# sergiud/SuiteSparse

Hardware: AMD Instinct MI355X
Metric: GFLOP/s supernodal Cholesky factor (Common->fl / t_factorize) (higher is better)
Workload: dtype f64; 1 GPU; poisson3d_200^3_geometricND_leaf4; n=8000000, nsuper=428821, parallelism=1 GPU

## Files before the change

### include/cholmod.h

```cpp
#ifndef CHOLMOD_AMD_H
#define CHOLMOD_AMD_H

#include <stddef.h>
#include <stdint.h>
#include <stdio.h>

#ifdef __cplusplus
extern "C" {
#endif

typedef int64_t SuiteSparse_long ;

#define CHOLMOD_MAIN_VERSION 3
#define CHOLMOD_SUB_VERSION 0
#define CHOLMOD_SUBSUB_VERSION 14

#ifndef TRUE
#define TRUE 1
#define FALSE 0
#endif

#define CHOLMOD_INT 0
#define CHOLMOD_INTLONG 1
#define CHOLMOD_LONG 2
// ... 206 lines not shown
double cholmod_l_norm_dense (cholmod_dense *X, int norm, cholmod_common *Common) ;
double cholmod_l_norm_sparse (cholmod_sparse *A, int norm, cholmod_common *Common) ;

cholmod_factor *cholmod_l_analyze (cholmod_sparse *A, cholmod_common *Common) ;
cholmod_factor *cholmod_l_analyze_p (cholmod_sparse *A, SuiteSparse_long *UserPerm,
    SuiteSparse_long *fset, size_t fsize, cholmod_common *Common) ;
cholmod_factor *cholmod_l_analyze_p2 (int for_whom, cholmod_sparse *A,
    SuiteSparse_long *UserPerm, SuiteSparse_long *fset, size_t fsize,
    cholmod_common *Common) ;
int cholmod_l_factorize (cholmod_sparse *A, cholmod_factor *L, cholmod_common *Common) ;
int cholmod_l_factorize_p (cholmod_sparse *A, double beta [2], SuiteSparse_long *fset,
    size_t fsize, cholmod_factor *L, cholmod_common *Common) ;
cholmod_dense *cholmod_l_solve (int sys, cholmod_factor *L, cholmod_dense *B,
    cholmod_common *Common) ;
int cholmod_l_solve2 (int sys, cholmod_factor *L, cholmod_dense *B, cholmod_sparse *Bset,
    cholmod_dense **X_Handle, cholmod_sparse **Xset_Handle, cholmod_dense **Y_Handle,
    cholmod_dense **E_Handle, cholmod_common *Common) ;
double cholmod_l_rcond (cholmod_factor *L, cholmod_common *Common) ;
int cholmod_l_change_factor (int to_xtype, int to_ll, int to_super, int to_packed, int to_monotonic,
    cholmod_factor *L, cholmod_common *Common) ;
int cholmod_l_etree (cholmod_sparse *A, SuiteSparse_long *Parent, cholmod_common *Common) ;
SuiteSparse_long cholmod_l_postorder (SuiteSparse_long *Parent, size_t n,
    SuiteSparse_long *Weight, SuiteSparse_long *Post, cholmod_common *Common) ;
int cholmod_l_rowcolcounts (cholmod_sparse *A, SuiteSparse_long *fset, size_t fsize,
    SuiteSparse_long *Parent, SuiteSparse_long *Post, SuiteSparse_long *RowCount,
    SuiteSparse_long *ColCount, SuiteSparse_long *First, SuiteSparse_long *Level,
    cholmod_common *Common) ;

int cholmod_l_super_symbolic (cholmod_sparse *A, cholmod_sparse *F,
    SuiteSparse_long *Parent, cholmod_factor *L, cholmod_common *Common) ;
int cholmod_l_super_symbolic2 (int for_whom, cholmod_sparse *A, cholmod_sparse *F,
    SuiteSparse_long *Parent, cholmod_factor *L, cholmod_common *Common) ;
int cholmod_l_super_numeric (cholmod_sparse *A, cholmod_sparse *F, double beta [2],
    cholmod_factor *L, cholmod_common *Common) ;
int cholmod_l_super_lsolve (cholmod_factor *L, cholmod_dense *X, cholmod_dense *E,
    cholmod_common *Common) ;
int cholmod_l_super_ltsolve (cholmod_factor *L, cholmod_dense *X, cholmod_dense *E,
    cholmod_common *Common) ;

int cholmod_l_gpu_memorysize (size_t *total_mem, size_t *available_mem,
    cholmod_common *Common) ;
int cholmod_l_gpu_probe (cholmod_common *Common) ;
int cholmod_l_gpu_deallocate (cholmod_common *Common) ;
void cholmod_l_gpu_end (cholmod_common *Common) ;
int cholmod_l_gpu_allocate (cholmod_common *Common) ;
int cholmod_gpu_memorysize (size_t *total_mem, size_t *available_mem, cholmod_common *Common) ;
int cholmod_gpu_probe (cholmod_common *Common) ;
int cholmod_gpu_deallocate (cholmod_common *Common) ;
void cholmod_gpu_end (cholmod_common *Common) ;
int cholmod_gpu_allocate (cholmod_common *Common) ;

int cholmod_l_factor_to_host (cholmod_factor *L, cholmod_common *Common) ;
int cholmod_l_hip_stats (cholmod_factor *L, double *stats, cholmod_common *Common) ;
int cholmod_l_hip_prepare (cholmod_factor *L, cholmod_common *Common) ;
int cholmod_l_gather_factor (cholmod_factor *L, cholmod_common *Common) ;
int cholmod_l_refactorize_resident (double beta [2], cholmod_factor *L,
    cholmod_common *Common) ;

#ifdef __cplusplus
}
#endif
#endif
```

### include/cholmod_hip.h

```cpp
#ifndef CHOLMOD_HIP_H
#define CHOLMOD_HIP_H

#include <stddef.h>
#include <stdint.h>

#ifdef __cplusplus
extern "C" {
#endif

#define CHOLMOD_HIP_OK            0
#define CHOLMOD_HIP_NOT_POSDEF    1
#define CHOLMOD_HIP_NO_DEVICE   (-1)
#define CHOLMOD_HIP_OUT_OF_MEMORY (-2)
#define CHOLMOD_HIP_TOO_LARGE   (-3)
#define CHOLMOD_HIP_INVALID     (-4)
#define CHOLMOD_HIP_GPU_PROBLEM (-5)

#define CHOLMOD_HIP_PLAN_DEFAULT   0
#define CHOLMOD_HIP_TILE128         4
#define CHOLMOD_HIP_NO_SMALL_FRONTS 16
#define CHOLMOD_HIP_NO_XCD_SWIZZLE 32
#define CHOLMOD_HIP_FIXED_OB       64
#define CHOLMOD_HIP_WIDE_OB       128
#define CHOLMOD_HIP_NO_CB_ASSIGN   2048
#define CHOLMOD_HIP_NO_FUSED_POTRF 512
#define CHOLMOD_HIP_NO_FUSED_TRSM 1024
#define CHOLMOD_HIP_NO_LEAF_PAIRS 4096
#define CHOLMOD_HIP_NO_EXCHANGE_LOOKAHEAD 256
#define CHOLMOD_HIP_CHAIN256     8192
#define CHOLMOD_HIP_PHI_TWIN    16384
#define CHOLMOD_HIP_CX_STORAGE   32768
#define CHOLMOD_HIP_PLAN_HOST_ONLY 2

typedef struct cholmod_hip_plan cholmod_hip_plan ;

int cholmod_hip_probe (void) ;

int cholmod_hip_memorysize (size_t *total_mem, size_t *available_mem) ;

int cholmod_hip_set_device (int device) ;
int cholmod_hip_device_count (int *count) ;

cholmod_hip_plan *cholmod_hip_plan_create (int64_t n, int64_t nsuper,
    const int64_t *super, const int64_t *pi, const int64_t *px,
    const int64_t *s, int flags, int *status) ;

void cholmod_hip_plan_destroy (cholmod_hip_plan *plan) ;

typedef int (*cholmod_hip_allreduce_fn) (void *dev_ptr, int64_t count_doubles,
    int group_first, int group_size, void *user) ;
cholmod_hip_plan *cholmod_hip_plan_create_dist (int64_t n, int64_t nsuper,
    const int64_t *super, const int64_t *pi, const int64_t *px,
    const int64_t *s, int flags, int rank, int world, int *status) ;
int cholmod_hip_set_allreduce (cholmod_hip_plan *plan,
    cholmod_hip_allreduce_fn fn, void *user) ;
int cholmod_hip_rccl_unique_id (void *id128) ;
int cholmod_hip_rccl_attach (cholmod_hip_plan *plan, const void *id128) ;
int cholmod_hip_rccl_detach (cholmod_hip_plan *plan) ;
int64_t cholmod_hip_debug_routing (cholmod_hip_plan *plan, int64_t cap, int64_t *pair_d, int64_t *pair_a,
    int64_t *cb_lo, int64_t *cb_hi) ;
int cholmod_hip_debug_schedule_hash (cholmod_hip_plan *plan, uint64_t *out16) ;
int cholmod_hip_progress_enable (cholmod_hip_plan *plan, int enable) ;
int cholmod_hip_progress (cholmod_hip_plan *plan, int64_t *out12) ;
int64_t cholmod_hip_get_batches (cholmod_hip_plan *plan, int64_t *batch_of, int64_t *global_arena) ;
int cholmod_hip_get_partition (cholmod_hip_plan *plan, int64_t *owner) ;
int cholmod_hip_get_groups (cholmod_hip_plan *plan, int64_t *first, int64_t *size) ;
int cholmod_hip_gather_factor (cholmod_hip_plan *plan) ;

int cholmod_hip_factorize (cholmod_hip_plan *plan, const int64_t *Sp,
    const int64_t *Si, const int64_t *Snz, const double *Sx, double beta,
    int quick_return_if_not_posdef, double *Lx_host, int64_t *minor) ;

int cholmod_hip_upload_matrix (cholmod_hip_plan *plan, const int64_t *Sp,
    const int64_t *Si, const int64_t *Snz, const double *Sx) ;
int cholmod_hip_factorize_resident (cholmod_hip_plan *plan, double beta,
    int quick_return_if_not_posdef, int64_t *minor) ;

int cholmod_hip_set_value_map (cholmod_hip_plan *plan, const int64_t *src, int64_t snz,
    int64_t nvalues) ;
int cholmod_hip_refresh_values (cholmod_hip_plan *plan, const double *values, int64_t nvalues) ;
int cholmod_hip_values_staging (cholmod_hip_plan *plan, double **host_buffer, int64_t *nvalues) ;
int cholmod_hip_values_push (cholmod_hip_plan *plan, int64_t offset, int64_t count) ;
int cholmod_hip_values_commit (cholmod_hip_plan *plan, int commit) ;
int cholmod_hip_values_gather_index (cholmod_hip_plan *plan, const int64_t **index, int64_t *chunk_len, int64_t *count) ;
int cholmod_hip_values_begin (cholmod_hip_plan *plan) ;
int cholmod_hip_values_push_chunk (cholmod_hip_plan *plan, int64_t chunk) ;

int cholmod_hip_download_factor (cholmod_hip_plan *plan, double *Lx_host) ;
int cholmod_hip_download_even_columns (cholmod_hip_plan *plan, double *out_host) ;
int cholmod_hip_upload_factor (cholmod_hip_plan *plan, const double *Lx_host) ;

int cholmod_hip_solve (cholmod_hip_plan *plan, int which, double *X,
    int64_t nrhs, int64_t ldx) ;

int cholmod_hip_get_maps (cholmod_hip_plan *plan, int64_t *sparent,
    int64_t *level, int64_t *relmap) ;

int cholmod_hip_diag_minmax (cholmod_hip_plan *plan, double *out3) ;
int cholmod_hip_factor_checks (cholmod_hip_plan *plan, double *out5) ;
int cholmod_hip_factor_checks_local (cholmod_hip_plan *plan, double *out5) ;

#define CHOLMOD_HIP_NSTATS 40
int cholmod_hip_get_stats (cholmod_hip_plan *plan, double *stats) ;
int cholmod_hip_set_profiling (cholmod_hip_plan *plan, int on) ;
int64_t cholmod_hip_get_launch_profile (cholmod_hip_plan *plan, int64_t cap, int32_t *kind,
    int32_t *grid, int32_t *aux, double *ms, double *flops, double *bytes) ;

int cholmod_hip_debug_thin_cycles (cholmod_hip_plan *plan, int64_t launch, long long *out10) ;
int64_t cholmod_hip_debug_launch_regions (cholmod_hip_plan *plan, int64_t launch, int64_t cap, int64_t *out) ;

int cholmod_hip_dense_partial_factor (double *F, int64_t nsrow, int64_t nscol,
    int flags, int64_t *info) ;

const char *cholmod_hip_version (void) ;

#ifdef __cplusplus
}
#endif
#endif
```

### suitesparse_amd/cholmod.py

```python
from __future__ import annotations

import ctypes as C
import os
import subprocess

import numpy as np

_HERE = os.path.dirname(os.path.abspath(__file__))
LIB_PATH = os.environ.get("CHOLMOD_AMD_LIB") or os.path.join(_HERE, "lib", "libcholmod_amd.so")
HOOKS_LIB_PATH = os.path.join(_HERE, "lib", "libcholmod_amd_testhooks.so")
CSRC = os.path.join(_HERE, "csrc")

CHOLMOD_MAXMETHODS = 9
CHOLMOD_HIP_NSTATS = 40

PATTERN, REAL, COMPLEX, ZOMPLEX = 0, 1, 2, 3
OK, NOT_INSTALLED, OUT_OF_MEMORY, TOO_LARGE, INVALID, GPU_PROBLEM = 0, -1, -2, -3, -4, -5
NOT_POSDEF = 1
NATURAL, GIVEN, POSTORDERED = 0, 1, 6
SIMPLICIAL, AUTO, SUPERNODAL = 0, 1, 2
SYS_A, SYS_LDLt, SYS_LD, SYS_DLt, SYS_L, SYS_Lt, SYS_D, SYS_P, SYS_Pt = range(9)
HIP_PLAN_HOST_ONLY = 2
HIP_WIDE_OB, HIP_NO_FUSED_POTRF, HIP_NO_FUSED_TRSM, HIP_PHI_TWIN = 128, 512, 1024, 16384
HIP_INVALID = -4


class Method(C.Structure):
    _fields_ = [("lnz", C.c_double), ("fl", C.c_double), ("ordering", C.c_int)]


ERRFUNC = C.CFUNCTYPE(None, C.c_int, C.c_char_p, C.c_int, C.c_char_p)
ALLREDUCE_FN = C.CFUNCTYPE(C.c_int, C.c_void_p, C.c_int64, C.c_int, C.c_int, C.c_void_p)


class Common(C.Structure):
    _fields_ = [
        ("supernodal", C.c_int), ("supernodal_switch", C.c_double),
        ("final_asis", C.c_int), ("final_super", C.c_int), ("final_ll", C.c_int),
        ("final_pack", C.c_int), ("final_monotonic", C.c_int), ("final_resymbol", C.c_int),
        ("zrelax", C.c_double * 3), ("nrelax", C.c_size_t * 3),
        ("prefer_upper", C.c_int), ("quick_return_if_not_posdef", C.c_int),
        ("print", C.c_int), ("nmethods", C.c_int), ("current", C.c_int), ("selected", C.c_int),
        ("method", Method * (CHOLMOD_MAXMETHODS + 1)),
        ("postorder", C.c_int), ("try_catch", C.c_int),
        ("error_handler", ERRFUNC),
        ("itype", C.c_int), ("dtype", C.c_int), ("status", C.c_int),
        ("fl", C.c_double), ("lnz", C.c_double), ("anz", C.c_double), ("modfl", C.c_double),
        ("malloc_count", C.c_size_t), ("memory_usage", C.c_size_t), ("memory_inuse", C.c_size_t),
        ("nrealloc_col", C.c_double), ("nrealloc_factor", C.c_double), ("ndbounds_hit", C.c_double),
        ("rowfacfl", C.c_double), ("aatfl", C.c_double),
        ("called_nd", C.c_int), ("blas_ok", C.c_int),
        ("useGPU", C.c_int), ("maxGpuMemBytes", C.c_size_t), ("maxGpuMemFraction", C.c_double),
        ("gpuMemorySize", C.c_size_t), ("gpuKernelTime", C.c_double), ("gpuFlops", C.c_int64),
        ("gpuNumKernelLaunches", C.c_int), ("devBuffSize", C.c_size_t), ("ibuffer", C.c_int),
        ("syrkStart", C.c_double),
        ("cholmod_cpu_gemm_time", C.c_double), ("cholmod_cpu_syrk_time", C.c_double),
        ("cholmod_cpu_trsm_time", C.c_double), ("cholmod_cpu_potrf_time", C.c_double),
        ("cholmod_gpu_gemm_time", C.c_double), ("cholmod_gpu_syrk_time", C.c_double),
        ("cholmod_gpu_trsm_time", C.c_double), ("cholmod_gpu_potrf_time", C.c_double),
        ("cholmod_assemble_time", C.c_double), ("cholmod_assemble_time2", C.c_double),
        ("cholmod_cpu_gemm_calls", C.c_size_t), ("cholmod_cpu_syrk_calls", C.c_size_t),
        ("cholmod_cpu_trsm_calls", C.c_size_t), ("cholmod_cpu_potrf_calls", C.c_size_t),
        ("cholmod_gpu_gemm_calls", C.c_size_t), ("cholmod_gpu_syrk_calls", C.c_size_t),
        ("cholmod_gpu_trsm_calls", C.c_size_t), ("cholmod_gpu_potrf_calls", C.c_size_t),
        ("hip_factor_on_device", C.c_int), ("hip_flags", C.c_int), ("hip_profile", C.c_int),
        ("hip_rank", C.c_int), ("hip_world", C.c_int),
        ("hip_allreduce", C.c_void_p), ("hip_allreduce_user", C.c_void_p),
# ... 10 lines not shown


class Triplet(C.Structure):
    _fields_ = [("nrow", C.c_size_t), ("ncol", C.c_size_t), ("nzmax", C.c_size_t), ("nnz", C.c_size_t),
                ("i", C.c_void_p), ("j", C.c_void_p), ("x", C.c_void_p), ("z", C.c_void_p),
                ("stype", C.c_int), ("itype", C.c_int), ("xtype", C.c_int), ("dtype", C.c_int)]


class Dense(C.Structure):
    _fields_ = [("nrow", C.c_size_t), ("ncol", C.c_size_t), ("nzmax", C.c_size_t),
                ("d", C.c_size_t), ("x", C.c_void_p), ("z", C.c_void_p),
                ("xtype", C.c_int), ("dtype", C.c_int)]


class Factor(C.Structure):
    _fields_ = [("n", C.c_size_t), ("minor", C.c_size_t),
                ("Perm", C.c_void_p), ("ColCount", C.c_void_p), ("IPerm", C.c_void_p),
                ("nzmax", C.c_size_t),
                ("p", C.c_void_p), ("i", C.c_void_p), ("x", C.c_void_p), ("z", C.c_void_p),
                ("nz", C.c_void_p), ("next", C.c_void_p), ("prev", C.c_void_p),
                ("nsuper", C.c_size_t), ("ssize", C.c_size_t), ("xsize", C.c_size_t),
                ("maxcsize", C.c_size_t), ("maxesize", C.c_size_t),
                ("super", C.c_void_p), ("pi", C.c_void_p), ("px", C.c_void_p), ("s", C.c_void_p),
                ("ordering", C.c_int), ("is_ll", C.c_int), ("is_super", C.c_int),
                ("is_monotonic", C.c_int), ("itype", C.c_int), ("xtype", C.c_int),
                ("dtype", C.c_int), ("useGPU", C.c_int),
                ("hip_plan", C.c_void_p), ("hip_on_device", C.c_int), ("hip_host_valid", C.c_int),
                ("cx_twin", C.c_void_p), ("hip_apat_hash", C.c_uint64), ("hip_apat_nnz", C.c_size_t),
                ("hip_apat_valid", C.c_int), ("hip_apat_hash2", C.c_uint64), ("hip_is_twin", C.c_int),
                ("bset_work", C.c_void_p), ("hip_plan_ahead", C.c_int)]


API_SYMBOLS = [
    "cholmod_l_start", "cholmod_l_finish", "cholmod_l_defaults", "cholmod_l_error",
    "cholmod_l_malloc", "cholmod_l_calloc", "cholmod_l_free",
    "cholmod_l_allocate_sparse", "cholmod_l_free_sparse", "cholmod_l_copy_sparse",
    "cholmod_l_nnz", "cholmod_l_ptranspose", "cholmod_l_transpose",
    "cholmod_l_allocate_triplet", "cholmod_l_free_triplet", "cholmod_l_triplet_to_sparse",
    "cholmod_l_allocate_dense", "cholmod_l_zeros", "cholmod_l_ones", "cholmod_l_copy_dense",
    "cholmod_l_free_dense", "cholmod_l_free_factor",
    "cholmod_l_read_sparse", "cholmod_l_read_triplet", "cholmod_l_read_dense", "cholmod_l_read_matrix", "cholmod_l_check_factor", "cholmod_l_check_sparse",
    "cholmod_gpu_memorysize", "cholmod_gpu_probe", "cholmod_gpu_deallocate", "cholmod_gpu_end", "cholmod_gpu_allocate",
    "cholmod_l_gpu_stats", "cholmod_l_sdmult", "cholmod_l_norm_dense", "cholmod_l_norm_sparse",
    "cholmod_l_analyze", "cholmod_l_analyze_p", "cholmod_l_analyze_p2",
    "cholmod_l_factorize", "cholmod_l_factorize_p", "cholmod_l_solve", "cholmod_l_solve2",
    "cholmod_l_rcond", "cholmod_l_change_factor", "cholmod_l_realloc",
    "SuiteSparse_start", "SuiteSparse_finish", "SuiteSparse_malloc", "SuiteSparse_calloc", "SuiteSparse_realloc", "SuiteSparse_free",
    "cholmod_l_etree", "cholmod_l_postorder", "cholmod_l_rowcolcounts",
    "cholmod_l_super_symbolic", "cholmod_l_super_symbolic2", "cholmod_l_super_numeric",
    "cholmod_l_super_lsolve", "cholmod_l_super_ltsolve",
    "cholmod_l_gpu_memorysize", "cholmod_l_gpu_probe", "cholmod_l_gpu_deallocate",
    "cholmod_l_gpu_end", "cholmod_l_gpu_allocate",
    "cholmod_l_factor_to_host", "cholmod_l_hip_stats", "cholmod_l_refactorize_resident",
    "cholmod_l_gather_factor", "cholmod_l_hip_prepare",
]
HIP_SYMBOLS = [
    "cholmod_hip_probe", "cholmod_hip_memorysize", "cholmod_hip_set_device", "cholmod_hip_device_count",
    "cholmod_hip_plan_create", "cholmod_hip_plan_destroy", "cholmod_hip_factorize",
    "cholmod_hip_plan_create_dist", "cholmod_hip_set_allreduce", "cholmod_hip_get_partition",
    "cholmod_hip_get_groups", "cholmod_hip_get_batches", "cholmod_hip_progress_enable", "cholmod_hip_progress", "cholmod_hip_debug_schedule_hash", "cholmod_hip_diag_minmax", "cholmod_hip_values_staging", "cholmod_hip_values_push", "cholmod_hip_values_commit", "cholmod_hip_values_gather_index", "cholmod_hip_values_begin", "cholmod_hip_values_push_chunk", "cholmod_hip_debug_routing",
    "cholmod_hip_gather_factor",
    "cholmod_hip_upload_matrix", "cholmod_hip_factorize_resident",
    "cholmod_hip_set_value_map", "cholmod_hip_refresh_values",
    "cholmod_hip_download_factor", "cholmod_hip_download_even_columns", "cholmod_hip_upload_factor", "cholmod_hip_solve",
    "cholmod_hip_get_maps", "cholmod_hip_get_stats", "cholmod_hip_set_profiling",
    
    
    "cholmod_hip_dense_partial_factor", "cholmod_hip_factor_checks", "cholmod_hip_factor_checks_local", "cholmod_hip_get_launch_profile", "cholmod_hip_debug_thin_cycles", "cholmod_hip_debug_launch_regions",
    "cholmod_hip_rccl_unique_id", "cholmod_hip_rccl_attach", "cholmod_hip_rccl_detach",
    "cholmod_hip_version",
]

PROBES_PATH = os.path.join(_HERE, "lib", "libcholmod_amd_probes.so")
PROBE_SYMBOLS = [
    "cholmod_hip_bench_update_kernel", "cholmod_hip_bench_update_pair", "cholmod_hip_bench_mfma_peak", "cholmod_hip_bench_mfma_peak2",
    "cholmod_hip_bench_mixed", "cholmod_hip_debug_potrf_cycles", "cholmod_hip_debug_panel_cycles",
    "cholmod_hip_debug_latency", "cholmod_hip_bench_mfma_ceiling", "cholmod_hip_probe_cu_mask", "cholmod_hip_probe_overlap", "cholmod_hip_debug_update_diff", "cholmod_hip_debug_diag_cycles", "cholmod_hip_bench_handoff",
]

_probes = None


def build(force: bool = False) -> str:
    if force:
        subprocess.check_call(["make", "-C", CSRC, "-s", "clean"])
    subprocess.check_call(["make", "-C", CSRC, "-s", "-j3"])
    return LIB_PATH


_libs = {}


def lib(hooks=None):
    if hooks is None:
        hooks = os.environ.get("SSAMD_TEST_HOOKS_LIB") == "1"
    path = HOOKS_LIB_PATH if hooks else LIB_PATH
    if path in _libs:
        return _libs[path]
    if not os.path.exists(path):
        raise RuntimeError(
            f"{path} is missing: build it with `python -c 'import __graft_entry__ as g; "
            "g.build()'` (hipcc --offload-arch=gfx950).  There is no fallback path.")
    L = C.CDLL(path)
    vp, i64, dbl, sz = C.c_void_p, C.c_int64, C.c_double, C.c_size_t
    cm = C.POINTER(Common)
    sp, dn, fc = C.POINTER(Sparse), C.POINTER(Dense), C.POINTER(Factor)

    def sig(name, res, args):
        f = getattr(L, name)
        f.restype = res
        f.argtypes = args

# ... 3 lines not shown
    sig("cholmod_l_allocate_sparse", sp, [sz, sz, sz, C.c_int, C.c_int, C.c_int, C.c_int, cm])
    sig("cholmod_l_free_sparse", C.c_int, [C.POINTER(sp), cm])
    sig("cholmod_l_copy_sparse", sp, [sp, cm])
    sig("cholmod_l_nnz", i64, [sp, cm])
    sig("cholmod_l_ptranspose", sp, [sp, C.c_int, vp, vp, sz, cm])
    sig("cholmod_l_transpose", sp, [sp, C.c_int, cm])
    sig("cholmod_l_allocate_dense", dn, [sz, sz, sz, C.c_int, cm])
    sig("cholmod_l_zeros", dn, [sz, sz, C.c_int, cm])
    sig("cholmod_l_ones", dn, [sz, sz, C.c_int, cm])
    sig("cholmod_l_copy_dense", dn, [dn, cm])
    sig("cholmod_l_free_dense", C.c_int, [C.POINTER(dn), cm])
    sig("cholmod_l_free_factor", C.c_int, [C.POINTER(fc), cm])
    sig("cholmod_l_check_factor", C.c_int, [fc, cm])
    sig("cholmod_l_check_sparse", C.c_int, [sp, cm])
    sig("cholmod_l_gpu_stats", C.c_int, [cm])
    sig("cholmod_l_sdmult", C.c_int, [sp, C.c_int, C.POINTER(dbl * 2), C.POINTER(dbl * 2), dn, dn, cm])
    sig("cholmod_l_norm_dense", dbl, [dn, C.c_int, cm])
    sig("cholmod_l_norm_sparse", dbl, [sp, C.c_int, cm])
    sig("cholmod_l_analyze", fc, [sp, cm])
    sig("cholmod_l_analyze_p", fc, [sp, vp, vp, sz, cm])
    sig("cholmod_l_analyze_p2", fc, [C.c_int, sp, vp, vp, sz, cm])
    sig("cholmod_l_factorize", C.c_int, [sp, fc, cm])
    sig("cholmod_l_factorize_p", C.c_int, [sp, C.POINTER(dbl * 2), vp, sz, fc, cm])
    sig("cholmod_l_solve", dn, [C.c_int, fc, dn, cm])
    sig("cholmod_l_solve2", C.c_int, [C.c_int, fc, dn, sp, C.POINTER(dn), C.POINTER(sp), C.POINTER(dn), C.POINTER(dn), cm])
    sig("cholmod_l_rcond", dbl, [fc, cm])
    sig("cholmod_l_change_factor", C.c_int, [C.c_int, C.c_int, C.c_int, C.c_int, C.c_int, fc, cm])
    sig("cholmod_l_etree", C.c_int, [sp, vp, cm])
    sig("cholmod_l_postorder", i64, [vp, sz, vp, vp, cm])
    sig("cholmod_l_rowcolcounts", C.c_int, [sp, vp, sz, vp, vp, vp, vp, vp, vp, cm])
    sig("cholmod_l_super_symbolic", C.c_int, [sp, sp, vp, fc, cm])
    sig("cholmod_l_super_numeric", C.c_int, [sp, sp, C.POINTER(dbl * 2), fc, cm])
    sig("cholmod_l_super_lsolve", C.c_int, [fc, dn, dn, cm])
    sig("cholmod_l_super_ltsolve", C.c_int, [fc, dn, dn, cm])
    sig("cholmod_l_gpu_memorysize", C.c_int, [C.POINTER(sz), C.POINTER(sz), cm])
    sig("cholmod_l_gpu_probe", C.c_int, [cm])
    sig("cholmod_l_gpu_allocate", C.c_int, [cm])
    sig("cholmod_l_gpu_deallocate", C.c_int, [cm])
    sig("cholmod_l_factor_to_host", C.c_int, [fc, cm])
    sig("cholmod_l_hip_stats", C.c_int, [fc, C.POINTER(dbl * CHOLMOD_HIP_NSTATS), cm])
    sig("cholmod_l_refactorize_resident", C.c_int, [C.POINTER(dbl * 2), fc, cm])
    sig("cholmod_l_read_sparse", sp, [vp, cm])
    sig("cholmod_l_read_dense", dn, [vp, cm])
    sig("cholmod_l_read_triplet", vp, [vp, cm])
    sig("cholmod_l_free_triplet", C.c_int, [C.POINTER(vp), cm])
    sig("cholmod_l_read_matrix", vp, [vp, C.c_int, C.POINTER(C.c_int), cm])
    sig("cholmod_hip_probe", C.c_int, [])
    sig("cholmod_hip_set_device", C.c_int, [C.c_int])
    sig("cholmod_hip_memorysize", C.c_int, [C.POINTER(sz), C.POINTER(sz)])
    sig("cholmod_hip_plan_create", vp, [i64, i64, vp, vp, vp, vp, C.c_int, C.POINTER(C.c_int)])
    sig("cholmod_hip_plan_destroy", None, [vp])
    sig("cholmod_hip_plan_create_dist", vp, [i64, i64, vp, vp, vp, vp, C.c_int, C.c_int, C.c_int,
                                             C.POINTER(C.c_int)])
    sig("cholmod_hip_set_allreduce", C.c_int, [vp, ALLREDUCE_FN, vp])
    sig("cholmod_hip_get_partition", C.c_int, [vp, vp])
    sig("cholmod_hip_get_groups", C.c_int, [vp, vp, vp])
    sig("cholmod_hip_get_batches", i64, [vp, vp, vp])
    sig("cholmod_hip_progress_enable", C.c_int, [vp, C.c_int])
    sig("cholmod_hip_progress", C.c_int, [vp, vp])
    sig("cholmod_hip_debug_schedule_hash", C.c_int, [vp, vp])
    sig("cholmod_hip_debug_routing", C.c_int64, [vp, C.c_int64, vp, vp, vp, vp])
    sig("cholmod_hip_gather_factor", C.c_int, [vp])
    sig("cholmod_l_gather_factor", C.c_int, [fc, cm])
    sig("cholmod_l_hip_prepare", C.c_int, [fc, cm])
    sig("cholmod_hip_factorize", C.c_int, [vp, vp, vp, vp, vp, dbl, C.c_int, vp, C.POINTER(i64)])
    sig("cholmod_hip_upload_matrix", C.c_int, [vp, vp, vp, vp, vp])
    sig("cholmod_hip_factorize_resident", C.c_int, [vp, dbl, C.c_int, C.POINTER(i64)])
    sig("cholmod_hip_download_factor", C.c_int, [vp, vp])
    sig("cholmod_hip_upload_factor", C.c_int, [vp, vp])
    sig("cholmod_hip_solve", C.c_int, [vp, C.c_int, vp, i64, i64])
    sig("cholmod_hip_get_maps", C.c_int, [vp, vp, vp, vp])
    sig("cholmod_hip_get_stats", C.c_int, [vp, vp])
    sig("cholmod_hip_set_profiling", C.c_int, [vp, C.c_int])
    sig("cholmod_hip_dense_partial_factor", C.c_int, [vp, i64, i64, C.c_int, C.POINTER(i64)])
    sig("cholmod_hip_factor_checks", C.c_int, [vp, vp])
    sig("cholmod_hip_factor_checks_local", C.c_int, [vp, vp])
    sig("cholmod_hip_get_launch_profile", i64, [vp, i64, vp, vp, vp, vp, vp, vp])
    sig("cholmod_hip_debug_thin_cycles", C.c_int, [vp, i64, vp])
    sig("cholmod_hip_debug_launch_regions", i64, [vp, i64, i64, vp])
    sig("cholmod_hip_rccl_unique_id", C.c_int, [vp])
    sig("cholmod_hip_rccl_attach", C.c_int, [vp, vp])
    sig("cholmod_hip_rccl_detach", C.c_int, [vp])
    sig("cholmod_hip_version", C.c_char_p, [])
    _libs[path] = L
    return L


def probes():
    global _probes
    if _probes is not None:
        return _probes
    if not os.path.exists(PROBES_PATH):
        raise RuntimeError(f"{PROBES_PATH} is missing: build it with __graft_entry__.build()")
    L = C.CDLL(PROBES_PATH)
    vp, i64, dbl = C.c_void_p, C.c_int64, C.c_double
    for name, res, args in (
            ("cholmod_hip_bench_update_kernel", dbl, [i64, i64, i64, C.c_int, C.c_int]),
            ("cholmod_hip_bench_update_pair", dbl, [i64, i64, i64, i64, i64, C.c_int, C.c_int]),
            ("cholmod_hip_bench_mfma_peak", dbl, [C.c_int, C.c_int]),
            ("cholmod_hip_bench_mfma_peak2", dbl, [C.c_int, C.c_int, C.c_int, C.c_int]),
            ("cholmod_hip_bench_mixed", dbl, [C.c_int, C.c_int, C.c_int]),
            ("cholmod_hip_bench_mfma_ceiling", dbl, [C.c_int, C.c_int, C.c_int, C.c_int, vp]),
            ("cholmod_hip_probe_cu_mask", dbl, [vp, C.c_int, C.c_int, C.c_int, vp]),
            ("cholmod_hip_probe_overlap", C.c_int, [vp, vp, C.c_int, i64, i64, C.c_int, C.c_int, C.c_int, vp]),
            ("cholmod_hip_debug_update_diff", dbl, [i64, i64, i64, C.c_int, C.c_int, C.c_int]),
            ("cholmod_hip_debug_diag_cycles", C.c_int, [vp, C.c_int, C.c_int]),
# ... 230 lines not shown
```

### suitesparse_amd/csrc/hip/descriptors.hip.h

```cpp
#pragma once
#include <hip/hip_runtime.h>
#include <stdint.h>

typedef long long i64;
typedef int i32;

namespace sship {


struct FrontD {
    i64 psx;
    i64 psi;
    i64 cb;
    i64 rel;
    i32 k1;
    i32 nscol, nsrow, ncb;
    i32 parent;
    i32 child_begin, child_end;
    i32 assemble;
    i32 cbp;
    i32 own_w, own_g, own_r;
    i32 cbd;
    i32 cb_lo, cb_hi;
};
__host__ __device__ __forceinline__ bool col_owned (const FrontD &f, int c) { return f.own_w == 0 || ((c / f.own_w) % f.own_g) == f.own_r ; }
__host__ __device__ __forceinline__ int col_local (const FrontD &f, int c) { return f.own_w == 0 ? c : ((c / f.own_w) / f.own_g) * f.own_w + c % f.own_w ; }
__host__ __device__ __forceinline__ int owned_before (const FrontD &f, int c)
{
    if (f.own_w == 0) return c ;
    const int t = c / f.own_w ;
    const int full = t > f.own_r ? (t - f.own_r + f.own_g - 1) / f.own_g : 0 ;
    return full * f.own_w + ((t % f.own_g) == f.own_r ? c % f.own_w : 0) ;
}

struct ChildD { i64 cb; i64 rel; i32 ncb; i32 cbp; };
struct EaGroup { i32 front; i32 blk_start; i32 c_lo; i32 c_hi;
                 i64 pbase; };
#define EA_NO_PBASE INT64_MIN
struct ZeroGroup { i64 off; i64 len; i32 blk_start; i32 pad; };
struct PfGroup { i64 off; i32 lda; i32 nb; i32 front; i32 col0; };
struct TrGroup { i64 l_off; i64 b_off; i32 lda; i32 m; i32 nb; i32 front;
                 i32 col0; i32 blk_start; };
struct DgGroup { i64 off; i32 lda; i32 w; i32 front; i32 col0; i32 slot; i32 pad; };
struct RsGroup { i64 l_off; i64 b_off; i32 lda; i32 m; i32 w; i32 front; i32 col0; i32 blk_start; i32 slot; i32 pad; };
struct GemmGroup {
    i64 a_off, b_off, c_off;
    i32 lda, ldc;
    i32 m, n, k;
    i32 tri;
    i32 c_in_cb;
    i32 tile_start;
    i32 mt, nt;
    i32 front;
    i32 tile_mul, tile_add;
    i32 ntiles;
    i32 nblk;
    i32 swz;
    i32 assign;
    i32 pf_next, pf_col0;
    i32 tile_cnt;
};

__host__ __device__ __forceinline__ int tri_col (int j, int m) { return j * m - ((j * (j + 1)) >> 1) ; }

struct RelPair { i32 d ; i32 a ; i64 off ; } ;
#define ZERO_CHUNK 8192
#define ZERO_COLS 8
#ifndef EA_TW
#define EA_TW 8
#endif
#define UPD3_LX_PAD 64
#define PF_NB 64
#define PF2_LD 64
#define TRM_ROWS 64
#define SM_MAX 136
#define TF_PW 16
struct XchgD {
    i64 slab ;
    i32 lda ;
    i32 w ;
    i32 mb ;
    i32 R ;
    i32 g, r ;
    i32 fo ;
    i32 mf ;
    i32 Rf ;
} ;
#define WIN_ROWS 8192
struct WinD { i64 store ; i64 win ; i32 ld ; i32 c0, c1 ; i32 r0 ; i32 nrows ; i32 own_w, own_g, own_r ; i32 mode ; i32 blk_start ; } ;
#define DG_W 256
#define RS_ROWS 64
struct CfGroup { i64 l_off ; i32 lda ; i32 w ; i32 front ; i32 col0 ; i32 m1 ; i32 slot ; i32 fslot ; i32 dstart ; i32 bstart ; i32 off2 ; i32 m2 ; i32 off3 ; i32 m3 ; i32 pad ; } ;
struct SolveTask { i32 front ; i32 c0, c1 ; i32 below ; } ;
#define SOLVE_IB 64
#define SOLVE_SB 256
#define SOLVE_BIG_COLS 256
struct InvTask { i32 front ; i32 jb ; i64 w_off ; } ;
struct SolveBlk { i32 front, jb, w, wg_start, inv, slot ; } ;
#define CHK_COLS 64
struct CheckTask { i32 front ; i32 c0 ; } ;

}
```

### suitesparse_amd/csrc/hip/engine.hip

```cpp
#include "kernels.hip.h"
#include "plan.hip.h"
#include <thread>

#include <dlfcn.h>
#include <unistd.h>

namespace sship {
RcclApi *rccl_api ()
{
    static RcclApi api ;
    static bool tried = false ;
    if (tried) return api.h ? &api : nullptr ;
    tried = true ;
    const char *over = getenv ("CHOLMOD_HIP_RCCL_LIBRARY") ;
    const char *names [] = {"librccl.so.1", "librccl.so", "/opt/rocm/lib/librccl.so.1", nullptr} ;
    void *h = nullptr ;
    if (over && *over)
    {
        h = dlopen (over, RTLD_NOW | RTLD_LOCAL) ;
        if (!h) fprintf (stderr, "cholmod_hip: CHOLMOD_HIP_RCCL_LIBRARY=%s: %s\n", over, dlerror ()) ;
    }
    else for (int q = 0 ; names [q] && !h ; q++) h = dlopen (names [q], RTLD_NOW | RTLD_LOCAL) ;
    if (!h) return nullptr ;
    api.GetUniqueId = (decltype (api.GetUniqueId)) dlsym (h, "ncclGetUniqueId") ;
    api.CommInitRank = (decltype (api.CommInitRank)) dlsym (h, "ncclCommInitRank") ;
    api.CommSplit = (decltype (api.CommSplit)) dlsym (h, "ncclCommSplit") ;
    api.AllReduce = (decltype (api.AllReduce)) dlsym (h, "ncclAllReduce") ;
    api.ReduceScatter = (decltype (api.ReduceScatter)) dlsym (h, "ncclReduceScatter") ;
    api.AllGather = (decltype (api.AllGather)) dlsym (h, "ncclAllGather") ;
    api.Broadcast = (decltype (api.Broadcast)) dlsym (h, "ncclBroadcast") ;
    api.CommDestroy = (decltype (api.CommDestroy)) dlsym (h, "ncclCommDestroy") ;
    api.GetErrorString = (decltype (api.GetErrorString)) dlsym (h, "ncclGetErrorString") ;
    if (!api.GetUniqueId || !api.CommInitRank || !api.CommSplit || !api.AllReduce || !api.ReduceScatter || !api.AllGather || !api.Broadcast || !api.CommDestroy) return nullptr ;
    api.h = h ;
    return &api ;
}
}
#define COMMA ,
#define CXS_LAUNCH(K, ...) do { if (cxs) hipLaunchKernelGGL (K<true>, __VA_ARGS__) ; else hipLaunchKernelGGL (K<false>, __VA_ARGS__) ; } while (0)
#define RCCLCHK(call) do { ncclResult_t r_ = (call) ; if (r_ != ncclSuccess) { \
    fprintf (stderr, "cholmod_hip: %s failed: %s (%s:%d)\n", #call, \
        (rccl_api () && rccl_api ()->GetErrorString) ? rccl_api ()->GetErrorString (r_) : "?", __FILE__, __LINE__) ; \
    return CHOLMOD_HIP_GPU_PROBLEM ; } } while (0)


namespace {

static void free_device (cholmod_hip_plan *P)
{
    if (P->prog_dev) { (void) hipHostFree (P->prog_dev) ; P->prog_dev = nullptr ; }
    if (P->h_vals) { (void) hipHostFree (P->h_vals) ; P->h_vals = nullptr ; }
    if (P->values_ev) { (void) hipEventDestroy (P->values_ev) ; P->values_ev = nullptr ; }
    for (auto e : P->chunk_ev) (void) hipEventDestroy (e) ;
    P->chunk_ev.clear () ;
    if (P->d_vorder) { (void) hipFree (P->d_vorder) ; P->d_vorder = nullptr ; }
    if (RcclApi *R = (P->nccl_world ? rccl_api () : nullptr))
    {
        for (auto &g : P->nccl_group) (void) R->CommDestroy (g.second) ;
        (void) R->CommDestroy (P->nccl_world) ;
        P->nccl_group.clear () ; P->nccl_world = nullptr ;
    }
    if (P->ar_done) (void) hipEventDestroy (P->ar_done) ;
    void *ptrs [] = {P->d_Ls, P->d_fr, P->d_supermap, P->d_child, P->d_relmap, P->d_info,
        P->d_lvl_list, P->d_Lx, P->d_cb, P->d_zg, P->d_eg, P->d_pg, P->d_tg, P->d_tu_cnt, P->d_cdesc, P->d_smd, P->d_sp01, P->d_gg, P->d_sm,
        P->d_Sp, P->d_Si, P->d_Snz, P->d_Sx, P->d_amap, P->d_X, P->d_Y, P->d_perm, P->d_xchg, P->d_stage, P->d_ag, P->d_agf, P->d_Lx_full, P->d_fr_full, P->d_dg, P->d_rg, P->d_wg, P->d_cg, P->d_cflags, P->d_crel, P->d_relpairs, P->d_dinv, P->d_sv,
        P->d_inv_tasks, P->d_winv, P->d_solved, P->d_sv_acc, P->d_ticket, P->d_chk, P->d_chk_out, P->d_thin_tim, P->d_sb_tasks, P->d_sb_commit, P->d_first_fail, P->d_vsrc, P->d_vals} ;
    for (void *p : ptrs) if (p) (void) hipFree (p) ;
    for (auto e : P->evpool) (void) hipEventDestroy (e) ;
    for (auto e : P->sync_ev) (void) hipEventDestroy (e) ;
    if (P->stream2) (void) hipStreamDestroy (P->stream2) ;
    if (P->ev0) (void) hipEventDestroy (P->ev0) ;
    if (P->ev1) (void) hipEventDestroy (P->ev1) ;
    if (P->stream) (void) hipStreamDestroy (P->stream) ;
}

static int upload_plan (cholmod_hip_plan *P)
{
    hipError_t e ;
    const bool ptiming = getenv ("CHOLMOD_HIP_PLAN_TIMING") != nullptr ;
    auto pnow = [] () { return std::chrono::duration<double> (std::chrono::steady_clock::now ().time_since_epoch ()).count () ; } ;
    double tu0 = pnow () ;
    HIPCHK (hipStreamCreate (&P->stream)) ;
    if (const char *e = TEST_ENV ("CHOLMOD_HIP_TEST_JITTER"))
    {
        unsigned long long seed = 0 ; int mx = 2000 ;
        if (sscanf (e, "%llu:%d", &seed, &mx) >= 1 && mx > 0)
        {
            P->jitter_us = mx ;
            P->jitter_state = seed * 0x9E3779B97F4A7C15ull + (unsigned long long) (P->rank + 1) * 0xD1B54A32D192ED03ull ;
        }
    }
    { const char *e = TEST_ENV ("CHOLMOD_HIP_TEST_DROP_WAITS") ; P->test_drop_waits = e ? std::max (atoi (e), 1) : 0 ; }
    if (const char *e = TEST_ENV ("CHOLMOD_HIP_TEST_HANG_EXCHANGE")) (void) sscanf (e, "%d:%ld:%ld", &P->test_hang_rank, &P->test_hang_xchg, &P->test_hang_fact) ;
    P->upd3_wg4 = P->world > 1 || P->force_shared ;
    {
        int least = 0, greatest = 0 ;
        if (hipDeviceGetStreamPriorityRange (&least, &greatest) == hipSuccess && greatest != least)
            HIPCHK (hipStreamCreateWithPriority (&P->stream2, hipStreamDefault, greatest)) ;
        else HIPCHK (hipStreamCreate (&P->stream2)) ;
    }
    for (int q = 0 ; q < P->sch.nevents ; q++)
    {
        hipEvent_t e ;
        HIPCHK (hipEventCreateWithFlags (&e, hipEventDisableTiming)) ;
        P->sync_ev.push_back (e) ;
    }
    HIPCHK (hipEventCreate (&P->ev0)) ;
    HIPCHK (hipEventCreate (&P->ev1)) ;
    size_t freeb = 0, totalb = 0 ;
    HIPCHK (hipMemGetInfo (&freeb, &totalb)) ;
    double need = 8.0 * P->lx_local + 8.0 * P->arena + 8.0 * P->ssize + 4.0 * P->relsize
        + sizeof (GemmGroup) * (double) P->sch.gg.size () + 64.0 * P->nsuper + (double) (64 << 20) ;
    if (need > (double) freeb)
    {
        fprintf (stderr, "cholmod_hip: factor needs %.2f GB of HBM, %.2f GB free\n",
            need / 1e9, freeb / 1e9) ;
        return CHOLMOD_HIP_OUT_OF_MEMORY ;
    }
    double tu1 = pnow () ;
    P->d_Ls = dupload (P->Ls, e) ; HIPCHK (e) ;
    P->d_fr = dupload (P->fr, e) ; HIPCHK (e) ;
    P->d_supermap = dupload (P->supermap, e) ; HIPCHK (e) ;
    P->d_child = dupload (P->child, e) ; HIPCHK (e) ;
    P->d_crel = dupload (P->crel, e) ; HIPCHK (e) ;
    P->d_relpairs = dupload (P->relpairs, e) ; HIPCHK (e) ;
    {
        std::vector<ChildD> cdv (P->child.size ()) ;
        for (size_t q = 0 ; q < P->child.size () ; q++)
        {
            if (P->child [q] < 0 || (size_t) P->child [q] >= P->fr.size ()) { cdv [q] = ChildD {0, 0, 0, 1} ; continue ; }
            const FrontD &cf = P->fr [P->child [q]] ;
            cdv [q] = ChildD {cf.cb, cf.rel, cf.ncb, cf.cbp} ;
        }
        P->d_cdesc = dupload (cdv, e) ; HIPCHK (e) ;
    }
    P->d_lvl_list = dupload (P->lvl_list, e) ; HIPCHK (e) ;
    P->d_zg = dupload (P->sch.zg, e) ; HIPCHK (e) ;
    P->d_eg = dupload (P->sch.eg, e) ; HIPCHK (e) ;
    P->d_pg = dupload (P->sch.pg, e) ; HIPCHK (e) ;
    P->d_tg = dupload (P->sch.tg, e) ; HIPCHK (e) ;
    HIPCHK (hipMalloc ((void **) &P->d_tu_cnt, std::max<size_t> (P->sch.tg.size (), 1) * sizeof (i32))) ;
    P->d_gg = dupload (P->sch.gg, e) ; HIPCHK (e) ;
    P->d_dg = dupload (P->sch.dg, e) ; HIPCHK (e) ;
    P->d_rg = dupload (P->sch.rg, e) ; HIPCHK (e) ;
    P->d_wg = dupload (P->sch.wg, e) ; HIPCHK (e) ;
    P->d_cg = dupload (P->sch.cg, e) ; HIPCHK (e) ;
    HIPCHK (hipMalloc ((void **) &P->d_cflags, (4 * (size_t) P->sch.ncflags + 4) * sizeof (int))) ;
    HIPCHK (hipMalloc ((void **) &P->d_dinv, (size_t) std::max (P->sch.max_dinv_slots, 1) * 4096 * sizeof (double))) ;
    P->d_sm = dupload (P->sch.sm, e) ; HIPCHK (e) ;
    {
        std::vector<FrontD> smd (P->sch.sm.size ()) ;
        for (size_t q = 0 ; q < smd.size () ; q++) smd [q] = P->fr [P->sch.sm [q]] ;
        P->d_smd = dupload (smd, e) ; HIPCHK (e) ;
        HIPCHK (hipMalloc ((void **) &P->d_sp01, std::max<size_t> (2 * smd.size (), 1) * sizeof (i64))) ;
    }
    P->d_sv = dupload (P->sv_tasks, e) ; HIPCHK (e) ;
    double tu2 = pnow () ;
    HIPCHK (hipMalloc ((void **) &P->d_relmap, std::max<i64> (std::max (P->relsize, P->relsize_all), 1) * sizeof (i32))) ;
    HIPCHK (hipMalloc ((void **) &P->d_info, std::max<i64> (P->nsuper, 1) * sizeof (i32))) ;
    HIPCHK (hipMalloc ((void **) &P->d_first_fail, sizeof (int))) ;
    if (TEST_ENV ("CHOLMOD_HIP_TEST_FAIL_ALLOC")) return CHOLMOD_HIP_OUT_OF_MEMORY ;
    HIPCHK (hipMalloc ((void **) &P->d_Lx, (std::max<i64> (P->lx_local, 1) + UPD3_LX_PAD) * sizeof (double))) ;
    HIPCHK (hipMalloc ((void **) &P->d_cb, std::max<i64> (P->arena, 1) * sizeof (double))) ;
    HIPCHK (hipMalloc ((void **) &P->d_xchg, 3 * (size_t) P->world * sizeof (double))) ;
    {
        i64 mx = 1, mxg = 1, mxf = 1 ;
        for (const Launch &L : P->sch.launches)
            if (L.kind == K_XCHG_RS || L.kind == K_XCHG_AG)
            {
                mx = std::max (mx, ((i64) L.xd.w * L.xd.w + ((i64) L.xd.R + L.xd.Rf) * L.xd.w) * L.xd.g) ;
                mxg = std::max (mxg, (i64) L.xd.R * L.xd.w * L.xd.g) ;
                mxf = std::max (mxf, (i64) L.xd.Rf * L.xd.w * L.xd.g) ;
            }
        HIPCHK (hipMalloc ((void **) &P->d_stage, (size_t) mx * sizeof (double))) ;
        HIPCHK (hipMalloc ((void **) &P->d_ag, (size_t) mxg * sizeof (double))) ;
        HIPCHK (hipMalloc ((void **) &P->d_agf, (size_t) mxf * sizeof (double))) ;
        P->agf_len = mxf ;
        P->stage_len = mx ; P->ag_len = mxg ;
    }
    double tu3 = pnow () ;
    if (getenv ("CHOLMOD_HIP_THIN_TIMING"))
    {
        HIPCHK (hipMalloc ((void **) &P->d_thin_tim, (P->sch.launches.size () + 1) * 10 * sizeof (long long))) ;
        HIPCHK (hipMemset (P->d_thin_tim, 0, (P->sch.launches.size () + 1) * 10 * sizeof (long long))) ;
    }
    if (P->nsuper > 0)
    {
        int grid = (int) ((P->nsuper * 64 + 255) / 256) ;
        hipLaunchKernelGGL (k_relmap, dim3 (grid), dim3 (256), 0, P->stream,
            (int) P->nsuper, P->d_fr, P->d_Ls, P->d_relmap) ;
        if (!P->relpairs.empty ())
            hipLaunchKernelGGL (k_relmap_pairs, dim3 ((unsigned) ((P->relpairs.size () * 64 + 255) / 256)), dim3 (256), 0, P->stream,
                (int) P->relpairs.size (), P->d_relpairs, P->d_fr, P->d_Ls, P->d_relmap) ;
        HIPCHK (hipGetLastError ()) ;
        HIPCHK (hipStreamSynchronize (P->stream)) ;
    }
    if (ptiming) fprintf (stderr, "cholmod_hip upload_plan: streams/events %.3f s, maps + schedule H2D %.3f s, hipMalloc (L %.1f GB, arena %.1f GB) %.3f s, relmap kernel %.3f s\n",
        tu1 - tu0, tu2 - tu1, 8e-9 * P->lx_local, 8e-9 * P->arena, tu3 - tu2, pnow () - tu3) ;
    return CHOLMOD_HIP_OK ;
// ... 182 lines not shown
        case K_EA:
            CX_LAUNCH (k_extend_add, dim3 (L.grid), dim3 (L.stream == 1 && !serial && narrow_xs () ? 64 : 256), 0, st,
                P->d_eg + L.goff, L.ng, P->d_fr, P->d_child, P->d_crel, P->d_relmap, P->d_Lx, P->d_cb, L.aux > 0 ? L.aux : EA_TW) ; break ;
        case K_POTRF:
            if (cx) hipLaunchKernelGGL ((k_potrf_mfma<false, true>), dim3 (L.grid), dim3 (256), 0, st,
                P->d_pg + L.goff, P->d_Lx, P->d_info, (long long *) nullptr) ;
            else hipLaunchKernelGGL ((k_potrf_mfma<false, false>), dim3 (L.grid), dim3 (256), 0, st,
                P->d_pg + L.goff, P->d_Lx, P->d_info, (long long *) nullptr) ;
            break ;
        case K_TRSM:
            { int rl = raise_lds_limits () ; if (rl != CHOLMOD_HIP_OK) return rl ; }
            if (cx) hipLaunchKernelGGL ((k_trsm_mfma<false, true>), dim3 (L.grid), dim3 (256), trsm_mfma_lds_bytes (L.aux), st,
                P->d_tg + L.goff, L.ng, P->d_Lx, P->d_info, L.aux, (long long *) nullptr) ;
            else hipLaunchKernelGGL ((k_trsm_mfma<false, false>), dim3 (L.grid), dim3 (256), trsm_mfma_lds_bytes (L.aux), st,
                P->d_tg + L.goff, L.ng, P->d_Lx, P->d_info, L.aux, (long long *) nullptr) ;
            break ;
        case K_TRSM_UPD:
            { int rl = raise_lds_limits () ; if (rl != CHOLMOD_HIP_OK) return rl ; }
            CX_LAUNCH (k_trsm_upd, dim3 (L.grid), dim3 (256), trsm_upd_lds_bytes (), st,
                P->d_tg + L.goff, L.ng, P->d_Lx, P->d_info, P->d_tu_cnt + L.goff) ;
            break ;
        case K_UPD_BIG:
            hipLaunchKernelGGL ((k_update2<BIG, BIG, BKK, 2, false>), dim3 (L.grid), dim3 (256), 0, st,
                P->d_gg + L.goff, L.ng, P->d_Lx, P->d_cb) ;
            break ;
        case K_UPD_SMALL:
            TW_LAUNCH (k_update2<SMALL COMMA SMALL COMMA BKK COMMA 2 COMMA false COMMA, >, dim3 (L.grid), dim3 (256), 0, st,
                P->d_gg + L.goff, L.ng, P->d_Lx, P->d_cb) ;
            break ;
        case K_DIAG:
            hipLaunchKernelGGL (k_diag<false>, dim3 (L.grid), dim3 (256), 0, st, P->d_dg + L.goff, P->d_Lx, P->d_info, P->d_dinv, (long long *) nullptr) ;
            break ;
        case K_ROWSOLVE:
            { int rl = raise_lds_limits () ; if (rl != CHOLMOD_HIP_OK) return rl ; }
            hipLaunchKernelGGL (k_rowsolve, dim3 (L.grid), dim3 (256), rowsolve_lds_bytes (), st,
                P->d_rg + L.goff, L.ng, P->d_Lx, P->d_info, P->d_dinv) ;
            break ;
        case K_UPD_W:
            if (P->upd3_wg4)
            {
                const unsigned g4 = (unsigned) (((L.grid + 31) / 32) * 8) ;
                if (L.aux >= 1024) TW_LAUNCH (k_update3<4 COMMA, COMMA 4>, dim3 (g4), dim3 (256), 0, st, P->d_gg + L.goff, L.ng, P->d_Lx, P->d_cb) ;
                else TW_LAUNCH (k_update3<2 COMMA, COMMA 4>, dim3 (g4), dim3 (256), 0, st, P->d_gg + L.goff, L.ng, P->d_Lx, P->d_cb) ;
            }
            else if (L.half)
            {
                const unsigned gh = 2u * (unsigned) ((L.grid + 7) / 8 * 8) ;
                if (L.aux >= 1024) TW_LAUNCH (k_update3<4 COMMA, COMMA 1 COMMA true>, dim3 (gh), dim3 (64), 0, st, P->d_gg + L.goff, L.ng, P->d_Lx, P->d_cb) ;
                else TW_LAUNCH (k_update3<2 COMMA, COMMA 1 COMMA true>, dim3 (gh), dim3 (64), 0, st, P->d_gg + L.goff, L.ng, P->d_Lx, P->d_cb) ;
            }
            else if (L.aux >= 1024) TW_LAUNCH (k_update3<4 COMMA, >, dim3 (L.grid), dim3 (64), 0, st, P->d_gg + L.goff, L.ng, P->d_Lx, P->d_cb) ;
            else TW_LAUNCH (k_update3<2 COMMA, >, dim3 (L.grid), dim3 (64), 0, st, P->d_gg + L.goff, L.ng, P->d_Lx, P->d_cb) ;
            break ;
        case K_UPD_PF:
            TW_LAUNCH (k_update2f<, >, dim3 (L.grid), dim3 (256), 0, st,
                P->d_gg + L.goff, L.ng, P->d_Lx, P->d_cb, P->d_info) ;
            break ;
    }
    if (!serial && L.rec_ev >= 0) HIPCHK (hipEventRecord (P->sync_ev [L.rec_ev], st)) ;
    return CHOLMOD_HIP_OK ;
}

static void exchange_volume (const cholmod_hip_plan *P, double *S)
{
    S [17] = S [18] = S [25] = S [39] = 0 ;
    const size_t nl = P->sch.launches.size () ;
    for (size_t q = 0 ; q < nl ; q++)
    {
        const Launch &L = P->sch.launches [q] ;
        if (L.kind != K_XCHG_RS && L.kind != K_XCHG_AG) continue ;
        S [17] += 1 ; S [18] += L.bytes ;
        if (L.kind != K_XCHG_AG) continue ;
        S [25] += L.bytes ;
        bool inl = L.stream == 0 ;
        for (size_t p = q + 1 ; !inl && p < nl ; p++)
        {
            const Launch &N = P->sch.launches [p] ;
            if (N.kind == K_JOIN) inl = true ;
            else if (!(N.kind == K_XCHG_AG && N.stream == 1)) break ;
        }
        if (inl) S [39] += L.bytes ;
    }
}

static int apply_value_chunks (cholmod_hip_plan *P, long need)
{
    while (P->chunks_applied < need)
    {
        const long c = P->chunks_applied ;
        for (long spin = 0 ; ; spin++)
        {
            const long have = P->chunks_pushed.load (std::memory_order_acquire) ;
            if (have < 0) return CHOLMOD_HIP_GPU_PROBLEM ;
            if (have > c) break ;
            if ((spin & 1023) == 1023) std::this_thread::yield () ;
        }
        HIPCHK (hipStreamWaitEvent (P->stream, P->chunk_ev [c], 0)) ;
        const i64 k0 = c * P->chunk_len, k1 = std::min<i64> (k0 + P->chunk_len, P->s_cur_nz) ;
        hipLaunchKernelGGL (k_values_chunk, dim3 ((unsigned) ((k1 - k0 + 255) / 256)), dim3 (256), 0, P->stream,
            k0, k1, P->d_vorder, P->d_vals, P->d_amap, P->d_Sx, P->d_Lx) ;
        P->chunks_applied = c + 1 ;
    }
    return CHOLMOD_HIP_OK ;
}

static int factorize_prologue (cholmod_hip_plan *P)
// ... 137 lines not shown
    (void) hipEventRecord (P->ev1, st) ;
    double th1 = now () ;
    float ms = 0 ;
    i64 sbad = -1, binfo = 0 ;
    if (poisoned == CHOLMOD_HIP_OK)
    {
        int first = (int) P->nsuper ;
        i32 inf = 0 ;
        bool ok = hipMemcpyAsync (P->d_first_fail, &first, sizeof (int), hipMemcpyHostToDevice, st) == hipSuccess ;
        if (ok && P->nsuper > 0)
            hipLaunchKernelGGL (k_first_fail, dim3 ((unsigned) ((P->nsuper + 255) / 256)), dim3 (256), 0, st,
                P->nsuper, P->d_info, P->d_first_fail) ;
        int chain_err = 0 ;
        if (P->sch.ncflags > 0)
            ok = ok && hipMemcpyAsync (&chain_err, P->d_cflags + 4 * (size_t) P->sch.ncflags, sizeof (int), hipMemcpyDeviceToHost, st) == hipSuccess ;
        ok = ok && hipMemcpyAsync (&first, P->d_first_fail, sizeof (int), hipMemcpyDeviceToHost, st) == hipSuccess
            && hipStreamSynchronize (st) == hipSuccess
            && hipEventElapsedTime (&ms, P->ev0, P->ev1) == hipSuccess ;
        if (ok && first < (int) P->nsuper)
        {
            ok = hipMemcpy (&inf, P->d_info + first, sizeof (i32), hipMemcpyDeviceToHost) == hipSuccess ;
            sbad = first ; binfo = inf ;
        }
        if (chain_err != 0)
        {
            fprintf (stderr, "cholmod_hip: k_chainf: a workgroup waited for a flag beyond its budget (hand-off between workgroups failed)\n") ;
            ok = false ;
        }
        if (!ok)
        {
            if (P->world == 1) return CHOLMOD_HIP_GPU_PROBLEM ;
            poisoned = CHOLMOD_HIP_GPU_PROBLEM ;
        }
        else if (building_map) P->amap_valid = true ;
    }
    double th2 = now () ;
    if (host_timing)
        fprintf (stderr, "cholmod_hip: host enqueue %.3f ms, wait+info copy %.3f ms, device %.3f ms, %zu launches\n",
            1e3 * (th1 - th0), 1e3 * (th2 - th1), (double) ms, nl) ;
    double *S = P->stats ;
    for (int q = 0 ; q < CHOLMOD_HIP_NSTATS ; q++) S [q] = 0 ;
    S [0] = ms * 1e-3 ;
    S [1] = P->exec_flops ;
    S [2] = (double) nl + 3 ;
    S [3] = P->nlevels ;
    S [4] = 8.0 * P->arena ;
    S [5] = 8.0 * P->xsize ;
    S [36] = 8.0 * P->lx_local ;
    exchange_volume (P, S) ;
    for (size_t q = 0 ; q < nl ; q++)
    {
        const Launch &L = P->sch.launches [q] ;
        if (L.kind == K_UPD_SMALL) { S [7] += 1 ; S [8] += L.flops ; S [16] += L.bytes ; }
        if (L.kind == K_UPD_W) { S [33] += 1 ; S [34] += L.flops ; S [35] += L.bytes ; }
        if (L.kind == K_UPD_PF) { S [26] += 1 ; S [28] += L.flops ; S [29] += L.bytes ; }
        if (L.kind == K_TRSM_UPD) S [31] += 1 ;
        if (L.kind == K_SMALL) { S [20] += L.bytes ; S [21] += L.ng ; }
        S [22] = P->nsplit ;
        if (L.kind == K_UPD_BIG) { S [15] += L.flops ; }
        if (L.kind == K_EA) S [10] += L.bytes ;
        if (L.kind == K_WIN)
            for (int w = 0 ; w < L.ng ; w++)
            {
                const WinD &Wd = P->sch.wg [L.goff + w] ;
                if (Wd.mode == 0) { S [37] += 1 ; if (Wd.win < 0) S [38] += 1 ; }
            }
    }
    if (prof && poisoned == CHOLMOD_HIP_OK)
    {
        float t = 0 ;
        HIPCHK (hipEventElapsedTime (&t, P->evpool [0], P->evpool [1])) ;
        S [13] = t * 1e-3 ;
        P->launch_ms.assign (nl, 0.0f) ;
        for (size_t q = 0 ; q < nl ; q++)
        {
            const Launch &L = P->sch.launches [q] ;
            HIPCHK (hipEventElapsedTime (&t, P->evpool [2 * (q + 1)], P->evpool [2 * (q + 1) + 1])) ;
            P->launch_ms [q] = t ;
            double sec = t * 1e-3 ;
            switch (L.kind)
            {
                case K_UPD_SMALL: S [6] += sec ; if (L.aux < MB) { S [23] += sec ; } break ;
                case K_UPD_PF: S [27] += sec ; break ;
                case K_UPD_W: S [32] += sec ; break ;
                case K_UPD_BIG: S [14] += sec ; break ;
                case K_EA: case K_ZERO: case K_WIN: S [9] += sec ; break ;
                case K_POTRF: case K_DIAG: case K_CHAINF: S [11] += sec ; break ;
                case K_ROWSOLVE: S [12] += sec ; break ;
                case K_SMALL: S [19] += sec ; break ;
                case K_TRSM: S [12] += sec ; break ;
                case K_TRSM_UPD: S [30] += sec ; break ;
            }
        }
    }
    if (P->world > 1 || P->force_shared)
    {
        if (!P->ar_fn && !P->nccl_world) return CHOLMOD_HIP_INVALID ;
        std::vector<double> x (3 * (size_t) P->world, 0.0) ;
        x [P->rank] = (double) (sbad >= 0 ? sbad : P->nsuper) ;
        x [P->world + P->rank] = (double) binfo ;
        x [2 * P->world + P->rank] = (poisoned != CHOLMOD_HIP_OK) ? 1.0 : 0.0 ;
        HIPCHK (hipMemcpy (P->d_xchg, x.data (), x.size () * sizeof (double), hipMemcpyHostToDevice)) ;
        if (P->nccl_world)
        {
            RCCLCHK (rccl_api ()->AllReduce (P->d_xchg, P->d_xchg, x.size (), ncclDouble, ncclSum, P->nccl_world, st)) ;
            HIPCHK (hipStreamSynchronize (st)) ;
        }
        else if (P->ar_fn (P->d_xchg, (i64) x.size (), 0, P->world, P->ar_user) != 0) return CHOLMOD_HIP_GPU_PROBLEM ;
        HIPCHK (hipMemcpy (x.data (), P->d_xchg, x.size () * sizeof (double), hipMemcpyDeviceToHost)) ;
        for (int r = 0 ; r < P->world ; r++)
            if (x [2 * P->world + r] != 0.0) return poisoned != CHOLMOD_HIP_OK ? poisoned : CHOLMOD_HIP_GPU_PROBLEM ;
        i64 best = P->nsuper ;
        for (int r = 0 ; r < P->world ; r++)
            if ((i64) x [r] < best) { best = (i64) x [r] ; binfo = (i64) x [P->world + r] ; }
        sbad = best < P->nsuper ? best : -1 ;
    }
    *minor = P->n ;
    if (sbad < 0) return CHOLMOD_HIP_OK ;
    const FrontD &f = P->fr [sbad] ;
    *minor = f.k1 + binfo - 1 ;
    i64 first_zero = sbad + ((binfo == 1 || quick) ? 0 : 1) ;
    i64 zero_from = P->lx_fronts ;
    for (i64 q = first_zero ; q < P->nsuper ; q++) if (P->lpx [q] >= 0) { zero_from = P->lpx [q] ; break ; }
    if (zero_from < P->lx_fronts)
        HIPCHK (hipMemsetAsync (P->d_Lx + zero_from, 0, (P->lx_fronts - zero_from) * sizeof (double), st)) ;
    HIPCHK (hipStreamSynchronize (st)) ;
    return CHOLMOD_HIP_NOT_POSDEF ;
}

}

static double *whole_factor (cholmod_hip_plan *P) { return P->world == 1 ? P->d_Lx : (P->full_valid ? P->d_Lx_full : nullptr) ; }
static const FrontD *whole_fronts (cholmod_hip_plan *P) { return P->world == 1 ? P->d_fr : P->d_fr_full ; }


extern "C" {

const char *cholmod_hip_version (void) { return "suitesparse_amd cholmod_hip 0.1 (gfx950)" ; }

int cholmod_hip_probe (void)
{
    int cnt = 0 ;
    if (hipGetDeviceCount (&cnt) != hipSuccess) return 0 ;
    return cnt > 0 ? 1 : 0 ;
}

int cholmod_hip_device_count (int *count)
{
    if (!count) return CHOLMOD_HIP_INVALID ;
    *count = 0 ;
    int cnt = 0 ;
    if (hipGetDeviceCount (&cnt) != hipSuccess) { (void) hipGetLastError () ; return CHOLMOD_HIP_NO_DEVICE ; }
    *count = cnt ;
    return CHOLMOD_HIP_OK ;
}

int cholmod_hip_memorysize (size_t *total_mem, size_t *available_mem)
{
    if (total_mem) *total_mem = 0 ;
    if (available_mem) *available_mem = 0 ;
    if (!cholmod_hip_probe ()) return 1 ;
    size_t f = 0, t = 0 ;
    if (hipMemGetInfo (&f, &t) != hipSuccess) return 1 ;
    if (total_mem) *total_mem = t ;
    if (available_mem) *available_mem = f ;
    return 0 ;
}

int cholmod_hip_set_device (int device)
{
    return hipSetDevice (device) == hipSuccess ? CHOLMOD_HIP_OK : CHOLMOD_HIP_NO_DEVICE ;
}

static cholmod_hip_plan *plan_create_impl (int64_t n, int64_t nsuper,
    const int64_t *super, const int64_t *pi, const int64_t *px, const int64_t *s,
    int flags, int rank, int world, int *status) ;

cholmod_hip_plan *cholmod_hip_plan_create_dist (int64_t n, int64_t nsuper,
    const int64_t *super, const int64_t *pi, const int64_t *px, const int64_t *s,
    int flags, int rank, int world, int *status)
{
    int st_local ;
    if (!status) status = &st_local ;
    try { return plan_create_impl (n, nsuper, super, pi, px, s, flags, rank, world, status) ; }
    catch (const std::bad_alloc &) { *status = CHOLMOD_HIP_OUT_OF_MEMORY ; return nullptr ; }
}

static cholmod_hip_plan *plan_create_impl (int64_t n, int64_t nsuper,
    const int64_t *super, const int64_t *pi, const int64_t *px, const int64_t *s,
    int flags, int rank, int world, int *status)
{
    *status = CHOLMOD_HIP_OK ;
    if (n < 0 || nsuper < 0 || !super || !pi || !px || !s || world < 1 || rank < 0 || rank >= world)
    { *status = CHOLMOD_HIP_INVALID ; return nullptr ; }
    if (n > INT32_MAX || nsuper > INT32_MAX) { *status = CHOLMOD_HIP_TOO_LARGE ; return nullptr ; }
    bool host_only = (flags & CHOLMOD_HIP_PLAN_HOST_ONLY) != 0 ;
    if (!host_only && !cholmod_hip_probe ()) { *status = CHOLMOD_HIP_NO_DEVICE ; return nullptr ; }
    const double tpc = std::chrono::duration<double> (std::chrono::steady_clock::now ().time_since_epoch ()).count () ;
    if (flags & CHOLMOD_HIP_CX_STORAGE)
    {
        if (world > 1) { if (status) *status = CHOLMOD_HIP_INVALID ; return nullptr ; }
        flags |= CHOLMOD_HIP_PHI_TWIN ;
        if (getenv ("CHOLMOD_HIP_CX_NO_THIN")) flags |= CHOLMOD_HIP_NO_SMALL_FRONTS ;
        flags &= ~(CHOLMOD_HIP_CHAIN256 | CHOLMOD_HIP_TILE128) ;
    }
    if (flags & CHOLMOD_HIP_PHI_TWIN)
    {
        bool ok = (n % 2 == 0) ;
        for (i64 q = 0 ; ok && q <= nsuper ; q++) ok = (super [q] % 2 == 0) && (pi [q] % 2 == 0) ;
        for (i64 q = 0 ; ok && q + 1 < pi [nsuper] ; q += 2) ok = (s [q] % 2 == 0) && (s [q + 1] == s [q] + 1) ;
        if (!ok) { if (status) *status = CHOLMOD_HIP_INVALID ; return nullptr ; }
    }
    cholmod_hip_plan *P = new (std::nothrow) cholmod_hip_plan ;
    if (!P) { *status = CHOLMOD_HIP_OUT_OF_MEMORY ; return nullptr ; }
    struct Guard { cholmod_hip_plan *P ; ~Guard () { if (P) { free_device (P) ; delete P ; } } } guard {P} ;
    P->n = n ; P->nsuper = nsuper ; P->flags = flags ; P->host_only = host_only ;
    P->rank = rank ; P->world = world ;
    P->super.assign (super, super + nsuper + 1) ;
    P->pi.assign (pi, pi + nsuper + 1) ;
    P->px.assign (px, px + nsuper + 1) ;
    P->ssize = pi [nsuper] ; P->xsize = px [nsuper] ;
    P->Ls.assign (s, s + std::max<i64> (P->ssize, 1)) ;
    {
        const char *e = getenv ("CHOLMOD_HIP_ARENA_BUDGET_MB") ;
        double fixed = 8.0 * P->xsize + 8.0 * P->ssize + 4.0 * (P->ssize - n) + 3e9 ;
        if (e && atof (e) > 0) P->arena_budget = (i64) (atof (e) * 1048576.0) ;
        else if (world > 1) P->arena_budget = -1 ;
        else if (!host_only)
        {
            size_t freeb = 0, totalb = 0 ;
            if (hipMemGetInfo (&freeb, &totalb) == hipSuccess)
                P->arena_budget = (i64) std::max (1e9, (double) freeb - fixed) ;
        }
    }
    const bool ptiming = getenv ("CHOLMOD_HIP_PLAN_TIMING") != nullptr ;
    auto pnow = [] () { return std::chrono::duration<double> (std::chrono::steady_clock::now ().time_since_epoch ()).count () ; } ;
    double tp0 = pnow () ;
    *status = build_host (P) ;
    double tp1 = pnow () ;
    if (*status == CHOLMOD_HIP_OK && !host_only) *status = upload_plan (P) ;
    if (ptiming) fprintf (stderr, "cholmod_hip_plan_create: copy maps %.3f s, build_host %.3f s, upload_plan %.3f s\n",
        tp0 - tpc, tp1 - tp0, pnow () - tp1) ;
    if (*status != CHOLMOD_HIP_OK) return nullptr ;
    guard.P = nullptr ;
    return P ;
}

cholmod_hip_plan *cholmod_hip_plan_create (int64_t n, int64_t nsuper,
    const int64_t *super, const int64_t *pi, const int64_t *px, const int64_t *s,
    int flags, int *status)
{
    return cholmod_hip_plan_create_dist (n, nsuper, super, pi, px, s, flags, 0, 1, status) ;
}

int cholmod_hip_set_allreduce (cholmod_hip_plan *P, cholmod_hip_allreduce_fn fn, void *user)
{
    if (!P) return CHOLMOD_HIP_INVALID ;
    P->ar_fn = fn ; P->ar_user = user ;
    return CHOLMOD_HIP_OK ;
}

int cholmod_hip_get_groups (cholmod_hip_plan *P, int64_t *first, int64_t *size)
{
    if (!P || !first || !size) return CHOLMOD_HIP_INVALID ;
    for (i64 q = 0 ; q < P->nsuper ; q++) { first [q] = P->grp0 [q] ; size [q] = P->grpn [q] ; }
    return CHOLMOD_HIP_OK ;
}

int64_t cholmod_hip_debug_routing (cholmod_hip_plan *P, int64_t cap, int64_t *pair_d, int64_t *pair_a, int64_t *cb_lo, int64_t *cb_hi)
{
    if (!P) return CHOLMOD_HIP_INVALID ;
    for (size_t q = 0 ; q < P->relpairs.size () && (i64) q < cap ; q++)
    {
        if (pair_d) pair_d [q] = P->relpairs [q].d ;
        if (pair_a) pair_a [q] = P->relpairs [q].a ;
// ... 812 lines not shown
    P->stats [2] = (double) P->sch.launches.size () + 3 ;
    P->stats [3] = P->nlevels ;
    P->stats [4] = 8.0 * P->arena ;
    P->stats [5] = 8.0 * P->xsize ;
    P->stats [36] = 8.0 * P->lx_local ;
    P->stats [22] = P->nsplit ;
    P->stats [24] = P->solve_seconds ;
    exchange_volume (P, P->stats) ;
    for (int q = 0 ; q < CHOLMOD_HIP_NSTATS ; q++) stats [q] = P->stats [q] ;
    return CHOLMOD_HIP_OK ;
}

int cholmod_hip_debug_thin_cycles (cholmod_hip_plan *P, int64_t launch, long long *out10)
{
    if (!P || !P->d_thin_tim || launch < 0 || launch >= (i64) P->sch.launches.size ()) return CHOLMOD_HIP_INVALID ;
    HIPCHK (hipMemcpy (out10, P->d_thin_tim + 10 * launch, 10 * sizeof (long long), hipMemcpyDeviceToHost)) ;
    return CHOLMOD_HIP_OK ;
}

int64_t cholmod_hip_get_launch_profile (cholmod_hip_plan *P, int64_t cap, int32_t *kind, int32_t *grid,
    int32_t *aux, double *ms, double *flops, double *bytes)
{
    if (!P) return CHOLMOD_HIP_INVALID ;
    i64 nl = (i64) P->sch.launches.size () ;
    for (i64 q = 0 ; q < nl && q < cap ; q++)
    {
        const Launch &L = P->sch.launches [q] ;
        if (kind) kind [q] = L.kind ;
        if (grid) grid [q] = L.grid ;
        if (aux) aux [q] = L.aux ;
        if (ms) ms [q] = q < (i64) P->launch_ms.size () ? P->launch_ms [q] : 0.0 ;
        if (flops) flops [q] = L.flops ;
        if (bytes) bytes [q] = L.bytes ;
    }
    return nl ;
}

int cholmod_hip_debug_schedule_hash (cholmod_hip_plan *P, uint64_t *out16)
{
    if (!P || !out16) return CHOLMOD_HIP_INVALID ;
    auto fnv = [] (uint64_t h, const void *p, size_t nbytes) -> uint64_t
    {
        const unsigned char *b = (const unsigned char *) p ;
        for (size_t q = 0 ; q < nbytes ; q++) { h ^= b [q] ; h *= 0x100000001b3ull ; }
        return h ;
    } ;
    const uint64_t H0 = 0xcbf29ce484222325ull ;
    auto hv = [&] (const auto &v) -> uint64_t
    {
        return v.empty () ? H0 : fnv (H0, v.data (), v.size () * sizeof (v [0])) ;
    } ;
    const Schedule &S = P->sch ;
    out16 [0] = hv (S.zg) ; out16 [1] = hv (S.eg) ; out16 [2] = hv (S.pg) ; out16 [3] = hv (S.tg) ;
    out16 [4] = hv (S.gg) ; out16 [5] = hv (S.dg) ; out16 [6] = hv (S.rg) ; out16 [7] = hv (S.wg) ;
    out16 [8] = hv (S.cg) ; out16 [9] = hv (S.sm) ;
    uint64_t h = H0 ;
    for (const Launch &L : S.launches)
    {
        const i64 v [] = {L.kind, L.grid, L.ng, (i64) L.goff, L.stream, L.wait_ev, L.rec_ev, L.ar_g0, L.ar_gn, L.aux, L.leaf_T, L.leaf_pw, L.ndiag, L.half,
            L.xd.slab, L.xd.lda, L.xd.w, L.xd.mb, L.xd.R, L.xd.g, L.xd.r, L.xd.fo, L.xd.mf, L.xd.Rf, L.far} ;
        h = fnv (h, v, sizeof (v)) ;
        const double d [] = {L.flops, L.bytes} ;
        h = fnv (h, d, sizeof (d)) ;
    }
    out16 [10] = h ;
    out16 [11] = hv (P->fr) ;
    out16 [12] = fnv (hv (P->child), P->crel.data (), P->crel.size () * sizeof (i64)) ;
    out16 [13] = P->relpairs.empty () ? H0 : fnv (H0, P->relpairs.data (), P->relpairs.size () * sizeof (RelPair)) ;
    const i64 w [] = {S.ncflags, S.max_dinv_slots, S.nevents, P->arena, P->lx_local, P->lx_fronts, P->nsplit, P->relsize_all, P->global_arena} ;
    out16 [14] = fnv (H0, w, sizeof (w)) ;
    out16 [15] = fnv (fnv (hv (P->lpx), P->win_off.data (), P->win_off.size () * sizeof (i64)), P->assign_cb.data (), P->assign_cb.size ()) ;
    return CHOLMOD_HIP_OK ;
}

int64_t cholmod_hip_debug_launch_regions (cholmod_hip_plan *P, int64_t launch, int64_t cap, int64_t *out)
{
    if (!P || launch < 0 || launch >= (i64) P->sch.launches.size ()) return CHOLMOD_HIP_INVALID ;
    const Launch &L = P->sch.launches [launch] ;
    if (L.kind != K_UPD_W && L.kind != K_UPD_SMALL && L.kind != K_UPD_BIG && L.kind != K_UPD_PF) return 0 ;
    for (i64 q = 0 ; q < L.ng && q < cap ; q++)
    {
        const GemmGroup &G = P->sch.gg [L.goff + q] ;
        const i64 v [12] = {G.m, G.n, G.k, G.tri, G.c_in_cb, G.lda, G.ldc, G.ntiles, G.nblk, G.front, G.assign, G.swz} ;
        for (int t = 0 ; t < 12 ; t++) out [12 * q + t] = v [t] ;
    }
    return L.ng ;
}

int cholmod_hip_set_profiling (cholmod_hip_plan *P, int on)
{
    if (!P) return CHOLMOD_HIP_INVALID ;
    P->profiling = on != 0 ;
    return CHOLMOD_HIP_OK ;
}

int cholmod_hip_dense_partial_factor (double *F, int64_t nsrow, int64_t nscol, int flags,
    int64_t *info_out)
{
    if (!F || nsrow <= 0 || nscol <= 0 || nscol > nsrow) return CHOLMOD_HIP_INVALID ;
    if (!cholmod_hip_probe ()) return CHOLMOD_HIP_NO_DEVICE ;
    FrontD f ;
    memset (&f, 0, sizeof (f)) ;
    f.nscol = (i32) nscol ; f.nsrow = (i32) nsrow ; f.ncb = (i32) (nsrow - nscol) ; f.parent = -1 ;
    std::vector<FrontD> fr (1, f) ;
    Schedule S ;
    i32 id = 0 ;
    double fl = 0 ;
// ... 56 lines not shown
```

### suitesparse_amd/csrc/hip/kernels.hip.h

```cpp
#pragma once
#include <hip/hip_runtime.h>
#include <stdint.h>
#include <type_traits>

#include "descriptors.hip.h"

namespace sship {

typedef double d4 __attribute__((ext_vector_type(4))) ;
typedef double d2u __attribute__((ext_vector_type(2), aligned(8))) ;

template <bool CX>
__device__ __forceinline__ double ldcx (const double *base, int r, int c, i64 ld)
{
    if constexpr (!CX) return base [r + (i64) c * ld] ;
    else
    {
        const double v = base [(r ^ (c & 1)) + (i64) (c >> 1) * ld] ;
        return ((c & 1) && !(r & 1)) ? -v : v ;
    }
}
template <bool CX>
__device__ __forceinline__ void stcx (double *base, int r, int c, i64 ld, double v)
{
// ... 1429 lines not shown
                const int i = wm * WM + 2 * (lane & 15) ;
                const int j = wn * WN + 2 * ((lane >> 4) + 4 * r) + b ;
                if (i >= mrem || j >= nrem) continue ;
                const bool both = !G.tri || row0 + i >= col0 + j ;
                const bool second = G.tri && row0 + i + 1 == col0 + j ;
                double *Cj = C + i + colx<TW == 2> (j, G.ldc) ;
                if (both)
                {
                    d2u v ;
                    if (G.assign) { v.x = -acc [0][b][r] ; v.y = -acc [1][b][r] ; }
                    else { v = *(const d2u *) Cj ; v.x -= acc [0][b][r] ; v.y -= acc [1][b][r] ; }
                    *(d2u *) Cj = v ;
                }
                else if (second)
                {
                    if (G.assign) Cj [1] = -acc [1][b][r] ; else Cj [1] -= acc [1][b][r] ;
                }
            }
        return ;
    }
#pragma unroll
    for (int a = 0 ; a < TI ; a++)
#pragma unroll
        for (int b = 0 ; b < TJ ; b++)
#pragma unroll
            for (int r = 0 ; r < 4 ; r++)
            {
                int i = wm * WM + a * 16 + (lane & 15) ;
                int j = wn * WN + b * 16 + (lane >> 4) + 4 * r ;
                if (i < mrem && j < nrem && (!G.tri || row0 + i >= col0 + j))
                {
                    if (G.assign) C [i + (i64) j * G.ldc] = -acc [a][b][r] ;
                    else C [i + (i64) j * G.ldc] -= acc [a][b][r] ;
                }
            }
}

template <int BM, int BN, int BK, int MINW, bool DB, int TW = 0>
__global__ void __launch_bounds__(256, MINW) k_update2 (const GemmGroup *g, int ng,
    double *Lx, double *CB)
{
    __shared__ double sm [(DB ? 2 : 1) * BK * (BM + 16 + BN + 16)] ;
    int gi = find_group (g, ng, (int) blockIdx.x, &GemmGroup::tile_start) ;
    GemmGroup G = g [gi] ;
    int I, J ;
    if ((int) blockIdx.x - G.tile_start >= G.nblk) return ;
    if (!decode_tile (G, (int) blockIdx.x - G.tile_start, I, J)) return ;
    update_tile<BM, BN, BK, DB, false, TW> (G, I, J, Lx, CB, sm) ;
}

#ifndef UPD3_CLAMP_LOADS
#define UPD3_CLAMP_LOADS 0
#endif
template <int DEPTH, bool EDGE, int TW = 0, int NQ = 2>
__device__ __forceinline__ void update_tile_w (const GemmGroup &G, int I, int J, double *Lx, double *CB, int cofs = 0)
{
    const int lane = threadIdx.x & 63, lr = lane & 15, lk = lane >> 4 ;
    const int row0 = I * 64, col0 = J * 64 + cofs ;
    const int mrem = G.m - row0, nrem = G.n - col0 ;
    const i64 lda = G.lda ;
    const int K = G.k ;
    const double *pa [2], *pb [2] ;
    int ra [2][2], rb [2][2] ;
#pragma unroll
    for (int q = 0 ; q < 2 ; q++)
    {
        ra [q][0] = 32 * q + 2 * lr ; ra [q][1] = ra [q][0] + 1 ;
        rb [q][0] = 32 * q + 2 * lr ; rb [q][1] = rb [q][0] + 1 ;
        if constexpr (EDGE && UPD3_CLAMP_LOADS)
        {
#pragma unroll
            for (int h = 0 ; h < 2 ; h++)
            {
                if (ra [q][h] > mrem - 1) ra [q][h] = mrem - 1 ;
                if (rb [q][h] > nrem - 1) rb [q][h] = nrem - 1 ;
            }
        }
        pa [q] = Lx + G.a_off + row0 + (i64) lk * lda ;
        pb [q] = Lx + G.b_off + col0 + (i64) lk * lda ;
    }
    struct Frag { double a [4], b [2 * NQ] ; } ;
    auto load = [&] (Frag &F, int kk)
    {
        const i64 ko = (i64) kk * lda ;
#pragma unroll
        for (int q = 0 ; q < 2 ; q++)
        {
            if constexpr (EDGE && UPD3_CLAMP_LOADS)
            {
                F.a [2 * q] = pa [q][ko + ra [q][0]] ; F.a [2 * q + 1] = pa [q][ko + ra [q][1]] ;
                if (q < NQ) { F.b [2 * q] = pb [q][ko + rb [q][0]] ; F.b [2 * q + 1] = pb [q][ko + rb [q][1]] ; }
            }
            else
            {
                d2u va = *(const d2u *) (pa [q] + ko + ra [q][0]) ;
                F.a [2 * q] = va.x ; F.a [2 * q + 1] = va.y ;
                if (q < NQ)
                {
                    d2u vb = *(const d2u *) (pb [q] + ko + rb [q][0]) ;
                    F.b [2 * q] = vb.x ; F.b [2 * q + 1] = vb.y ;
                }
            }
        }
    } ;
    auto load_tail = [&] (Frag &F, int kk)
    {
        const bool live = kk + lk < K ;
        const i64 ko = (i64) kk * lda - (live ? 0 : (i64) (kk + lk - (K - 1)) * lda) ;
#pragma unroll
        for (int q = 0 ; q < 2 ; q++)
        {
            double a0, a1, b0 = 0, b1 = 0 ;
            if constexpr (EDGE && UPD3_CLAMP_LOADS)
            {
                a0 = pa [q][ko + ra [q][0]] ; a1 = pa [q][ko + ra [q][1]] ;
                if (q < NQ) { b0 = pb [q][ko + rb [q][0]] ; b1 = pb [q][ko + rb [q][1]] ; }
            }
            else
            {
                d2u va = *(const d2u *) (pa [q] + ko + ra [q][0]) ;
                a0 = va.x ; a1 = va.y ;
                if (q < NQ) { d2u vb = *(const d2u *) (pb [q] + ko + rb [q][0]) ; b0 = vb.x ; b1 = vb.y ; }
            }
            F.a [2 * q] = live ? a0 : 0.0 ; F.a [2 * q + 1] = live ? a1 : 0.0 ;
            if (q < NQ) { F.b [2 * q] = live ? b0 : 0.0 ; F.b [2 * q + 1] = live ? b1 : 0.0 ; }
        }
    } ;
    d4 acc [4][2 * NQ] ;
#pragma unroll
    for (int a = 0 ; a < 4 ; a++)
#pragma unroll
        for (int b = 0 ; b < 2 * NQ ; b++) acc [a][b] = (d4) {0.0, 0.0, 0.0, 0.0} ;
    auto compute = [&] (const Frag &F)
    {
#pragma unroll
        for (int a = 0 ; a < 4 ; a++)
#pragma unroll
            for (int b = 0 ; b < 2 * NQ ; b++)
                acc [a][b] = __builtin_amdgcn_mfma_f64_16x16x4f64 (F.b [b], F.a [a], acc [a][b], 0, 0, 0) ;
    } ;
    const int nfull = K >> 2, nsteps = (K + 3) >> 2 ;
    auto load_any = [&] (Frag &F, int step) { if (step < nfull) load (F, 4 * step) ; else load_tail (F, 4 * step) ; } ;
    Frag f [DEPTH] ;
#pragma unroll
    for (int d = 0 ; d < DEPTH - 1 ; d++) if (d < nsteps) load_any (f [d], d) ;
    __builtin_amdgcn_s_waitcnt (0x0F70) ;
    int s = 0 ;
    for ( ; s + 2 * DEPTH - 1 <= nfull ; s += DEPTH)
    {
        load (f [DEPTH - 1], 4 * (s + DEPTH - 1)) ;
#pragma unroll
        for (int d = 0 ; d < DEPTH ; d++)
        {
            compute (f [d]) ;
            if (d < DEPTH - 1) load (f [d], 4 * (s + DEPTH + d)) ;
        }
    }
    for ( ; s < nsteps ; s += DEPTH)
    {
        if (s + DEPTH - 1 < nsteps) load_any (f [DEPTH - 1], s + DEPTH - 1) ;
#pragma unroll
        for (int d = 0 ; d < DEPTH ; d++)
        {
            if (s + d < nsteps) compute (f [d]) ;
            if (d < DEPTH - 1 && s + DEPTH + d < nsteps) load_any (f [d], s + DEPTH + d) ;
        }
    }
    if constexpr (TW)
    {
#pragma unroll
        for (int q = 0 ; q < 2 ; q++)
#pragma unroll
            for (int p = 0 ; p < NQ ; p++)
#pragma unroll
                for (int r = 0 ; r < 4 ; r++)
                {
                    const double ee = acc [2 * q][2 * p][r] + acc [2 * q + 1][2 * p + 1][r] ;
                    const double oe = acc [2 * q + 1][2 * p][r] - acc [2 * q][2 * p + 1][r] ;
                    acc [2 * q][2 * p][r] = ee ; acc [2 * q + 1][2 * p + 1][r] = ee ;
                    acc [2 * q + 1][2 * p][r] = oe ; acc [2 * q][2 * p + 1][r] = -oe ;
                }
    }
    double *C = (G.c_in_cb ? CB : Lx) + G.c_off + row0 + colx<TW == 2> (col0, G.ldc) ;
    const bool diag = G.tri && I == J ;
#pragma unroll
    for (int b = 0 ; b < 2 * NQ ; b++)
#pragma unroll
        for (int r = 0 ; r < 4 ; r++)
        {
            if (TW == 2 && (b & 1)) continue ;
            const int j = 32 * (b >> 1) + 2 * (lk + 4 * r) + (b & 1) ;
            const int jd = j + cofs ;
            double *Cj = C + colx<TW == 2> (j, G.ldc) ;
#pragma unroll
            for (int q = 0 ; q < 2 ; q++)
            {
                const int i = 32 * q + 2 * lr ;
                auto store_pair = [&] ()
                {
                    if (diag && i + 1 < jd) return ;
                    d2u v ;
                    if (G.assign) { v.x = -acc [2 * q][b][r] ; v.y = -acc [2 * q + 1][b][r] ; }
                    else
                    {
                        v = *(const d2u *) (Cj + i) ;
                        v.x -= acc [2 * q][b][r] ; v.y -= acc [2 * q + 1][b][r] ;
                    }
                    if (diag && i < jd) Cj [i + 1] = v.y ;
                    else *(d2u *) (Cj + i) = v ;
                } ;
                if constexpr (EDGE)
                {
                    if (j < nrem)
                    {
                        if (i + 1 < mrem) store_pair () ;
                        else if (i < mrem && (!diag || i >= jd))
                        {
                            if (G.assign) Cj [i] = -acc [2 * q][b][r] ;
                            else Cj [i] -= acc [2 * q][b][r] ;
                        }
                    }
                }
                else store_pair () ;
            }
        }
}

template <int DEPTH, int TW = 0, int WPB = 1, bool HALF = false>
__global__ void __launch_bounds__(64 * WPB, 2) k_update3 (const GemmGroup *g, int ng, double *Lx, double *CB)
{
    int vb = (int) blockIdx.x ;
    int cofs = 0 ;
    if constexpr (WPB > 1) vb = ((vb >> 3) * WPB + (int) (threadIdx.x >> 6)) * 8 + (vb & 7) ;
    if constexpr (HALF) { cofs = ((vb >> 3) & 1) * 32 ; vb = ((vb >> 4) << 3) | (vb & 7) ; }
    int gi = find_group (g, ng, vb, &GemmGroup::tile_start) ;
    GemmGroup G = g [gi] ;
    int I, J ;
    if (vb - G.tile_start >= G.nblk) return ;
    if (!decode_tile (G, vb - G.tile_start, I, J)) return ;
    if constexpr (HALF)
    {
        if (G.n - J * 64 - cofs <= 0) return ;
        if (G.m - I * 64 >= 64 && G.n - J * 64 - cofs >= 32) update_tile_w<DEPTH, false, TW, 1> (G, I, J, Lx, CB, cofs) ;
        else update_tile_w<DEPTH, true, TW, 1> (G, I, J, Lx, CB, cofs) ;
    }
    else
    {
        if (G.m - I * 64 >= 64 && G.n - J * 64 >= 64) update_tile_w<DEPTH, false, TW> (G, I, J, Lx, CB) ;
        else update_tile_w<DEPTH, true, TW> (G, I, J, Lx, CB) ;
    }
}

template <int TW>
__global__ void __launch_bounds__(256, 2) k_update2f (const GemmGroup *g, int ng,
    double *Lx, double *CB, i32 *info)
{
    __shared__ __attribute__((aligned(16))) double sm [PF_NB * PF2_LD] ;
    __shared__ int s_fail ;
    static_assert (PF_NB == 64 && PF2_LD == 64 && 16 * (64 + 16 + 64 + 16) <= PF_NB * PF2_LD, "slabs fit") ;
    int gi = find_group (g, ng, (int) blockIdx.x, &GemmGroup::tile_start) ;
    GemmGroup G = g [gi] ;
    int I, J ;
    if ((int) blockIdx.x - G.tile_start >= G.nblk) return ;
    if (!decode_tile (G, (int) blockIdx.x - G.tile_start, I, J)) return ;
    if (!(G.pf_next && I == 0 && J == 0))
    {
        update_tile<64, 64, 16, false, false, TW> (G, I, J, Lx, CB, sm) ;
        return ;
    }
    __builtin_amdgcn_s_setprio (3) ;
    update_tile<64, 64, 16, false, true, TW> (G, 0, 0, Lx, CB, sm) ;
    const int tid = threadIdx.x, lane = tid & 63, wave = tid >> 6 ;
    if (tid == 0) s_fail = -1 ;
    __syncthreads () ;
    double *A = Lx + G.c_off ;
    const i64 lda = G.ldc ;
    if (info [G.front] != 0)
    {
        for (int k = wave ; k < PF_NB ; k += 4)
            if (lane >= k) stcx<TW == 2> (A, lane, k, lda, 0.0) ;
        return ;
    }
    auto tick = [] (int) {} ;
    pf_eliminate<TW == 2> (sm, PF_NB / 16, &s_fail, tid, tick) ;
    const int fail = s_fail ;
    if (fail >= 0 && tid == 0) info [G.front] = G.pf_col0 + fail + 1 ;
    pf_store<TW == 2> (A, lda, sm, PF_NB, fail, lane, wave) ;
}

#define TU_LDX 80
__host__ __device__ inline size_t trsm_upd_lds_bytes ()
{
    return (size_t) (64 * 64 + 4 * 256 + 64 * TU_LDX) * sizeof (double) ;
}
template <bool CX>
__global__ void __launch_bounds__(256) k_trsm_upd (const TrGroup *g, int ng, double *Lx, i32 *info, i32 *cnt)
{
    extern __shared__ __attribute__((aligned(16))) double tu_lds [] ;
    double *Ls = tu_lds ;
    double *Wd = Ls + 64 * 64 ;
    double *X0s = Wd + 4 * 256 ;
    __shared__ int s_fail, s_last ;
// ... 1357 lines not shown
```

### suitesparse_amd/csrc/hip/plan.hip.h

```cpp
#pragma once
#include "descriptors.hip.h"
#include "../../../include/cholmod_hip.h"

#include <rccl/rccl.h>

#include <algorithm>
#include <atomic>
#include <cmath>
#include <cstdio>
#include <cstdlib>
#include <cstring>
#include <map>
#include <functional>
#include <memory>
#include <new>
#include <queue>
#include <vector>
#include <atomic>
#include <chrono>

#ifdef CHOLMOD_HIP_TEST_HOOKS
#define TEST_ENV(name) getenv (name)
#else
#define TEST_ENV(name) ((const char *) nullptr)
#endif

namespace sship {

constexpr int NB = PF_NB ;
constexpr int MB = 512 ;
struct ObThresholds { int t1, t2, t3 ; } ;
static inline ObThresholds outer_block_thresholds ()
{
    const char *e1 = getenv ("CHOLMOD_HIP_OB1024_ROWS"), *e2 = getenv ("CHOLMOD_HIP_OB2048_ROWS") ;
    const char *e3 = getenv ("CHOLMOD_HIP_OB4096_ROWS") ;
    return ObThresholds {e1 ? atoi (e1) : 4000, e2 ? atoi (e2) : 8000, e3 ? atoi (e3) : 24000} ;
}
static inline int outer_block (int maxrows, const ObThresholds &t)
{
    return maxrows >= t.t3 ? 4096 : maxrows >= t.t2 ? 2048 : maxrows >= t.t1 ? 1024 : MB ;
}
constexpr int BIG = 128, SMALL = 64, BKK = 16 ;
static inline int own_width ()
{
    const char *e = getenv ("CHOLMOD_HIP_OWN_W") ;
    int w = e ? atoi (e) : 128 ;
    return (w == 64 || w == 128 || w == 256 || w == 512) ? w : 128 ;
}
static inline int front_ob (const FrontD &f, int flags, const ObThresholds &t)
{
    return (flags & CHOLMOD_HIP_FIXED_OB) ? MB : (flags & CHOLMOD_HIP_WIDE_OB) ? 2048 : outer_block (f.nsrow, t) ;
}
static inline i64 window_len (const FrontD &f, int ob) { return (i64) f.nsrow * std::min (ob, (int) f.nscol) ; }
static inline int window_count (const FrontD &f, int ob) { return f.nscol > ob ? 2 : 1 ; }

enum Kind { K_ZERO = 0, K_EA, K_POTRF, K_TRSM, K_UPD_BIG, K_UPD_SMALL, K_JOIN, K_XCHG_RS, K_SMALL, K_UPD_PF, K_TRSM_UPD, K_XCHG_AG, K_UPD_W, K_DIAG, K_ROWSOLVE, K_WIN, K_CHAINF, K_NKIND } ;

struct Launch {
    int kind ;
    int grid ;
    int ng ;
    size_t goff ;
    double flops ;
    double bytes ;
    int stream = 0 ;
    int wait_ev = -1 ;
    int rec_ev = -1 ;
    XchgD xd = {0, 0, 0, 0, 0, 1, 0, 0, 0, 0} ;
    int far = 0 ;
    int ar_g0 = 0, ar_gn = 1 ;
    int aux = 0 ;
    int leaf_T = 0 ;
    int leaf_pw = 0 ;
    int ndiag = 0 ;
    int half = 0 ;
} ;

#define HIPCHK(call) do { hipError_t e_ = (call) ; if (e_ != hipSuccess) { \
    fprintf (stderr, "cholmod_hip: %s failed: %s (%s:%d)\n", #call, \
        hipGetErrorString (e_), __FILE__, __LINE__) ; return CHOLMOD_HIP_GPU_PROBLEM ; } } while (0)

struct Arena {
    std::map<i64, i64> free_by_off ;
    std::multimap<i64, i64> free_by_len ;
    i64 top = 0 ;
    void erase_len (i64 len, i64 off)
    {
        auto r = free_by_len.equal_range (len) ;
        for (auto it = r.first ; it != r.second ; ++it)
            if (it->second == off) { free_by_len.erase (it) ; return ; }
    }
    i64 alloc (i64 len)
    {
        if (len == 0) return 0 ;
        auto it = free_by_len.lower_bound (len) ;
        if (it != free_by_len.end ())
        {
            i64 blen = it->first, off = it->second ;
            free_by_len.erase (it) ;
            free_by_off.erase (off) ;
            if (blen > len)
            {
                free_by_off [off + len] = blen - len ;
                free_by_len.insert ({blen - len, off + len}) ;
            }
            return off ;
        }
        i64 off = top ;
        if (!free_by_off.empty ())
        {
            auto last = std::prev (free_by_off.end ()) ;
            if (last->first + last->second == top)
            {
                off = last->first ;
                erase_len (last->second, last->first) ;
                free_by_off.erase (last) ;
            }
        }
        top = off + len ;
        return off ;
    }
    void release (i64 off, i64 len)
    {
        if (len == 0) return ;
        auto nx = free_by_off.lower_bound (off) ;
        if (nx != free_by_off.end () && off + len == nx->first)
        {
            len += nx->second ;
            erase_len (nx->second, nx->first) ;
            nx = free_by_off.erase (nx) ;
        }
        if (nx != free_by_off.begin ())
        {
            auto pv = std::prev (nx) ;
            if (pv->first + pv->second == off)
            {
                off = pv->first ;
                len += pv->second ;
                erase_len (pv->second, pv->first) ;
                free_by_off.erase (pv) ;
            }
        }
        free_by_off [off] = len ;
        free_by_len.insert ({len, off}) ;
    }
} ;

struct Schedule {
    std::vector<ZeroGroup> zg ;
    std::vector<EaGroup> eg ;
    std::vector<PfGroup> pg ;
    std::vector<TrGroup> tg ;
    std::vector<GemmGroup> gg ;
    std::vector<DgGroup> dg ;
    std::vector<RsGroup> rg ;
    std::vector<WinD> wg ;
    std::vector<CfGroup> cg ;
    int ncflags = 0 ;
    int max_dinv_slots = 0 ;
    std::vector<i32> sm ;
    std::vector<Launch> launches ;
    int nevents = 0 ;
} ;

template <typename T> static T *dupload (const std::vector<T> &v, hipError_t &err)
{
    T *d = nullptr ;
    size_t bytes = std::max<size_t> (v.size (), 1) * sizeof (T) ;
    err = hipMalloc ((void **) &d, bytes) ;
    if (err != hipSuccess) return nullptr ;
    if (!v.empty ()) err = hipMemcpy (d, v.data (), v.size () * sizeof (T), hipMemcpyHostToDevice) ;
    return d ;
}

struct RcclApi {
    void *h = nullptr ;
    ncclResult_t (*GetUniqueId) (ncclUniqueId *) = nullptr ;
    ncclResult_t (*CommInitRank) (ncclComm_t *, int, ncclUniqueId, int) = nullptr ;
    ncclResult_t (*CommSplit) (ncclComm_t, int, int, ncclComm_t *, ncclConfig_t *) = nullptr ;
    ncclResult_t (*AllReduce) (const void *, void *, size_t, ncclDataType_t, ncclRedOp_t, ncclComm_t, hipStream_t) = nullptr ;
    ncclResult_t (*ReduceScatter) (const void *, void *, size_t, ncclDataType_t, ncclRedOp_t, ncclComm_t, hipStream_t) = nullptr ;
    ncclResult_t (*AllGather) (const void *, void *, size_t, ncclDataType_t, ncclComm_t, hipStream_t) = nullptr ;
    ncclResult_t (*Broadcast) (const void *, void *, size_t, ncclDataType_t, int, ncclComm_t, hipStream_t) = nullptr ;
    ncclResult_t (*CommDestroy) (ncclComm_t) = nullptr ;
    const char *(*GetErrorString) (ncclResult_t) = nullptr ;
} ;
RcclApi *rccl_api () ;

}

using namespace sship ;

struct cholmod_hip_plan {
    i64 n = 0, nsuper = 0, ssize = 0, xsize = 0 ;
    int flags = 0 ;
    bool host_only = false ;
    std::vector<i64> super, pi, px, Ls ;
    std::vector<FrontD> fr ;
    std::vector<i32> level, child, supermap ;
    std::vector<i32> lvl_ptr, lvl_list ;
    i64 relsize = 0, arena = 0 ;
    i64 arena_budget = 0 ;
    i64 global_arena = 0 ;
    std::vector<i32> batch_of ;
    int nsplit = 1 ;
    int nlevels = 0 ;
    int rank = 0, world = 1 ;
    bool force_shared = false ;
    std::vector<i32> owner ;
    std::vector<i32> grp0, grpn ;
    std::vector<char> assign_cb ;
    std::vector<i32> my_lvl_ptr, my_lvl_list ;
    cholmod_hip_allreduce_fn ar_fn = nullptr ;
    void *ar_user = nullptr ;
    int jitter_us = 0 ; unsigned long long jitter_state = 0 ;
    int test_drop_waits = 0 ;
    int test_hang_rank = -1 ; long test_hang_xchg = -1, test_hang_fact = 2 ;
    bool upd3_wg4 = false ;
    ncclComm_t nccl_world = nullptr ;
    std::map<i64, ncclComm_t> nccl_group ;
    hipEvent_t ar_done = nullptr ;
    double *d_xchg = nullptr ;
    double *d_stage = nullptr ;
    double *d_ag = nullptr ;
    double *d_agf = nullptr ;
    i64 stage_len = 0, ag_len = 0, agf_len = 0 ;
    std::vector<SolveTask> sv_tasks ;
    std::vector<i32> sv_ptr ;
    std::vector<std::vector<i32>> sv_big ;
    SolveTask *d_sv = nullptr ;
    std::vector<InvTask> inv_tasks ;
    std::vector<i64> inv_first ;
    InvTask *d_inv_tasks = nullptr ;
    double *d_winv = nullptr ;
    bool winv_valid = false ;
    double *d_solved = nullptr ; i64 solved_cap = 0 ;
    double *d_sv_acc = nullptr ; i64 sv_acc_cap = 0 ;
    unsigned int *d_ticket = nullptr ;
    struct SbLaunch { i32 level, first, ntasks, grid ; } ;
    std::vector<SolveBlk> sb_tasks, sb_commit ;
    std::vector<SbLaunch> sb_launch, sb_commit_launch ;
    std::vector<i32> sb_lvl_ptr ;
    SolveBlk *d_sb_tasks = nullptr, *d_sb_commit = nullptr ;
    int sb_max_tasks = 0 ;
    long long *d_thin_tim = nullptr ;
    CheckTask *d_chk = nullptr ; i64 nchk = 0 ;
    double *d_chk_out = nullptr ;
    Schedule sch ;
    double exec_flops = 0 ;
    hipStream_t stream = nullptr ;
    hipStream_t stream2 = nullptr ;
    std::vector<hipEvent_t> sync_ev ;
    i64 *d_Ls = nullptr ;
    FrontD *d_fr = nullptr ;
    i32 *d_supermap = nullptr, *d_child = nullptr, *d_relmap = nullptr, *d_info = nullptr ;
    i32 *d_lvl_list = nullptr ;
    double *d_Lx = nullptr, *d_cb = nullptr ;
    ZeroGroup *d_zg = nullptr ; EaGroup *d_eg = nullptr ; PfGroup *d_pg = nullptr ;
    TrGroup *d_tg = nullptr ; GemmGroup *d_gg = nullptr ; i32 *d_sm = nullptr ;
    DgGroup *d_dg = nullptr ; RsGroup *d_rg = nullptr ; double *d_dinv = nullptr ;
    std::vector<i64> lpx ;
    i64 lx_local = 0 ;
    std::vector<i64> win_off ;
    i64 lx_fronts = 0 ;
    std::vector<i64> crel ;
    std::vector<RelPair> relpairs ;
    i64 relsize_all = 0 ;
    bool passthru = false ;
    i64 *d_crel = nullptr ; RelPair *d_relpairs = nullptr ;
    WinD *d_wg = nullptr ;
    CfGroup *d_cg = nullptr ; int *d_cflags = nullptr ;
    double *d_Lx_full = nullptr ; FrontD *d_fr_full = nullptr ;
    bool full_valid = false ;
    FrontD *d_smd = nullptr ; i64 *d_sp01 = nullptr ;
    ChildD *d_cdesc = nullptr ;
    i32 *d_tu_cnt = nullptr ;
    double cur_beta = 0 ;
    i64 *d_Sp = nullptr, *d_Si = nullptr, *d_Snz = nullptr ; double *d_Sx = nullptr ;
    i64 s_nz = 0 ; bool s_unpacked = false ;
    int *d_first_fail = nullptr ;
    i64 *d_vsrc = nullptr ; double *d_vals = nullptr ;
    i64 vsrc_nz = 0, vals_n = 0, s_cur_nz = 0 ;
    double *h_vals = nullptr ; i64 h_vals_n = 0 ;
    hipEvent_t values_ev = nullptr ; bool values_pending = false ;
    std::vector<i64> h_Sp ;
    std::vector<int64_t> h_vgather ;
    i64 *d_vorder = nullptr ;
    std::vector<i64> batch_entries_end ;
    std::vector<size_t> batch_launch0 ;
    std::vector<i32> launch_need_chunks ;
    std::vector<hipEvent_t> chunk_ev ;
    i64 chunk_len = (i64) 1 << 20 ;
    long nchunks = 0, chunks_applied = 0 ;
    std::atomic<long> chunks_pushed {0} ;
    bool values_chunked = false, prologue_done = false ;
    int cur_mapped = 0 ;
    i64 *d_amap = nullptr ; bool amap_valid = false ;
    double *d_X = nullptr, *d_Y = nullptr ; i64 x_cap = 0 ;
    i64 *d_perm = nullptr ;
    volatile long long prog_fact = 0, prog_launch = 0, prog_xchg_enq = 0 ;
    long long *prog_dev = nullptr ;
    bool profiling = false ;
    double stats [CHOLMOD_HIP_NSTATS] = {0} ;
    double solve_seconds = 0 ;
    std::vector<float> launch_ms ;
    hipEvent_t ev0 = nullptr, ev1 = nullptr ;
    std::vector<hipEvent_t> evpool ;
} ;

namespace sship {

int build_host (cholmod_hip_plan *P) ;
void schedule_dense (const std::vector<FrontD> &fr, const i32 *ids, int nf,
    Schedule &S, int flags, const i32 *owner, const i32 *grp0, const i32 *grpn, int rank, int world,
    const char *assign_cb = nullptr, const i64 *win = nullptr, const i32 *child = nullptr, bool allow_half = false) ;

}
```

### suitesparse_amd/csrc/hip/plan_build.hip

```cpp
#include "plan.hip.h"

namespace sship {
namespace {

struct PlanBuilder
{
    cholmod_hip_plan *P ;
    const i64 n, nsuper ;
    int nlev = 0 ;
    std::vector<i32> cptr, call ;
    std::vector<double> wsub ;
    std::vector<i32> st_stack ;
    bool distribute = false, passthru = false, cx_storage = false ;
    int ownw = 128 ;
    std::vector<i64> cb_len_all ;
    std::vector<std::vector<i32>> rel_list ;
    std::vector<std::vector<i32>> batches ;

    explicit PlanBuilder (cholmod_hip_plan *P_) : P (P_), n (P_->n), nsuper (P_->nsuper) {}

    bool mine (i64 s) const { return P->rank >= P->grp0 [s] && P->rank < P->grp0 [s] + P->grpn [s] ; }
    template <typename F> void for_subtree (i32 root, F &&fn)
    {
        st_stack.clear () ;
// ... 579 lines not shown
        Lz.ng = (int) (S.zg.size () - Lz.goff) ; Lz.grid = blocks ;
        if (Lz.ng) S.launches.push_back (Lz) ;
    }
    void schedule_extend_add (const i32 *ids, int nf, int phase)
    {
        Schedule &S = P->sch ;
        Launch Le {K_EA, 0, 0, S.eg.size (), 0, 0} ;
        int blocks = 0 ;
        int tw = EA_TW ;
        for (int q = 0 ; q < nf ; q++)
            if (P->fr [ids [q]].child_end != P->fr [ids [q]].child_begin && P->fr [ids [q]].nsrow >= 2048) tw = 4 ;
        Le.aux = tw ;
        for (int q = 0 ; q < nf ; q++)
        {
            const FrontD &f = P->fr [ids [q]] ;
            if (f.child_end == f.child_begin) continue ;
            bool asg = P->assign_cb [ids [q]] != 0 ;
            if (f.cbd) continue ;
            int lo = (phase == 0 && !f.own_w) ? 0 : f.nscol ;
            int hi = phase == 0 ? (asg ? f.nscol : f.nsrow) : f.nsrow ;
            if (phase == 1 && !asg) continue ;
            if (hi <= lo) continue ;
            S.eg.push_back (EaGroup {ids [q], blocks, lo, hi, EA_NO_PBASE}) ;
            blocks += (hi - lo + tw - 1) / tw ;
            if (phase == 0)
                for (int c = f.child_begin ; c < f.child_end ; c++)
                {
                    double r = P->fr [P->child [c]].ncb ;
                    Le.bytes += (r * (r + 1) / 2) * 24.0 + 4.0 * r ;
                }
        }
        Le.ng = (int) (S.eg.size () - Le.goff) ; Le.grid = blocks ;
        if (Le.ng) S.launches.push_back (Le) ;
    }
    void schedule_batches ()
    {
        Schedule &S = P->sch ;
        std::vector<i32> mine_ids, gen ;
        P->batch_launch0.clear () ;
        for (const auto &bt : batches)
        {
            P->batch_launch0.push_back (S.launches.size ()) ;
            mine_ids.clear () ; gen.clear () ;
            for (i32 sf : bt) if (mine (sf)) mine_ids.push_back (sf) ;
            if (mine_ids.empty ()) continue ;
            schedule_thin (mine_ids, gen) ;
            const i32 *ids = gen.data () ;
            const int nf = (int) gen.size () ;
            if (nf == 0) continue ;
            schedule_zero (ids, nf) ;
            schedule_extend_add (ids, nf, 0) ;
            schedule_dense (P->fr, ids, nf, S, P->flags, P->owner.data (), P->grp0.data (), P->grpn.data (),
                P->rank, P->world, P->assign_cb.data (), P->win_off.data (), P->child.data (),
                P->world == 1 && !P->force_shared) ;
            schedule_extend_add (ids, nf, 1) ;
        }
    }

    int run ()
    {
        int rc = init_fronts () ;
        if (rc != CHOLMOD_HIP_OK) return rc ;
        rc = build_etree () ;
        if (rc != CHOLMOD_HIP_OK) return rc ;
        assign_ownership () ;
        layout_local_factor () ;
        build_child_lists () ;
        choose_batches () ;
        build_solve_tasks () ;
        layout_windows () ;
        schedule_batches () ;
        return CHOLMOD_HIP_OK ;
    }
} ;

}

int build_host (cholmod_hip_plan *P)
{
    PlanBuilder B (P) ;
    return B.run () ;
}

}
```

### suitesparse_amd/csrc/hip/schedule_dense.hip

```cpp
#include "plan.hip.h"

namespace sship {
namespace {

struct Upd { int q, kc, kk, t0, t1 ; bool cb, wide ; } ;

struct DenseScheduler
{
    const std::vector<FrontD> &fr ;
    const i32 *ids ; const int nf ;
    Schedule &S ;
    const int flags ;
    const i32 *owner, *grp0, *grpn ;
    const int rank, world ;
    const char *assign_cb ;
    const i64 *win ;
    const i32 *child ;
    const bool allow_half ;
    bool cx, twin, use_big ;
    ObThresholds obt ;
    int maxnscol = 0, maxrows = 0 ;
    i64 w_min_tiles ;
    i64 w_half_min, w_half_max ;
    int w_min_k ;
    i64 unfuse_tiles ;
    bool by_launch ;
    bool one_region ;
    bool swz16 ;
    bool xla ;
    bool chain256 = false ;
    bool fused256 = true ;
    bool fuse_potrf = false, fuse_trsm = false ;
    bool balance_cb ;
    std::vector<GemmGroup> big, small ;
    std::vector<GemmGroup> pfv ;
    std::vector<GemmGroup> wav ;
    std::vector<int> early ;
    std::vector<int> early_open ;
    std::vector<int> pf_done ;
    std::vector<Upd> step ;

    DenseScheduler (const std::vector<FrontD> &fr_, const i32 *ids_, int nf_, Schedule &S_, int flags_, const i32 *owner_,
        const i32 *grp0_, const i32 *grpn_, int rank_, int world_, const char *assign_cb_, const i64 *win_, const i32 *child_,
        bool allow_half_)
        : fr (fr_), ids (ids_), nf (nf_), S (S_), flags (flags_), owner (owner_), grp0 (grp0_), grpn (grpn_), rank (rank_),
          world (world_), assign_cb (assign_cb_), win (win_), child (child_), allow_half (allow_half_)
    {
        cx = (flags & CHOLMOD_HIP_CX_STORAGE) != 0 ;
        twin = (flags & CHOLMOD_HIP_PHI_TWIN) != 0 || cx ;
        use_big = (flags & CHOLMOD_HIP_TILE128) != 0 && !twin ;
        obt = outer_block_thresholds () ;
        for (int q = 0 ; q < nf ; q++)
        {
            maxnscol = std::max (maxnscol, fr [ids [q]].nscol) ;
            maxrows = std::max (maxrows, fr [ids [q]].nsrow) ;
        }
        { const char *e = getenv ("CHOLMOD_HIP_UPD3_MIN_TILES") ; w_min_tiles = e ? (i64) atoll (e) : (i64) 2048 ; }
        by_launch = true ;
        { const char *e = getenv ("CHOLMOD_HIP_UPD3_HALF_MAX") ; w_half_max = e ? (i64) atoll (e) : (i64) 10240 ; }
        w_half_min = 512 ; w_min_k = 256 ; unfuse_tiles = w_min_tiles ;
        if (!allow_half || w_min_tiles <= 0) w_half_max = 0 ;
        if (w_half_max <= 0 || w_half_min > w_min_tiles) w_half_min = w_min_tiles ;
        one_region = false ;
        swz16 = false ;
        xla = !(flags & CHOLMOD_HIP_NO_EXCHANGE_LOOKAHEAD) ;
        balance_cb = !use_big && !getenv ("CHOLMOD_HIP_NO_CB_BALANCE") ;
        early.assign (nf, -1) ; early_open.assign (nf, -1) ; pf_done.assign (nf, -1) ;
        choose_chain () ;
    }

    i64 co (int c, i64 ld) const { return cx ? (i64) (c >> 1) * ld : (i64) c * ld ; }
    void twin_operands (GemmGroup &G, int origin, int kc) const
    {
        if ((origin | kc | G.k | G.m | G.n | G.lda | G.ldc) & 1) { fprintf (stderr, "cholmod_hip: twin plan with an odd region\n") ; abort () ; }
        if (!cx) G.lda *= 2 ;
        G.k /= 2 ;
    }
    int ob_of (const FrontD &f) const { return front_ob (f, flags, obt) ; }
    bool is_shared (int fid) const { return owner && owner [fid] < 0 ; }
    bool windowed (int fid) const { return win && win [fid] >= 0 ; }
    i64 psx_at (int fid, int col) const
    {
        const FrontD &f = fr [fid] ;
        if (!windowed (fid)) return f.psx ;
        int OBq = ob_of (f), ob = col / OBq ;
        return win [fid] + (i64) (ob & 1) * window_len (f, OBq) - (i64) ob * OBq * f.nsrow ;
    }
    static i64 region_tiles (const GemmGroup &G)
    {
        i64 mt = (G.m + SMALL - 1) / SMALL, nt = (G.n + SMALL - 1) / SMALL ;
        return G.tri ? nt * (nt + 1) / 2 + (mt - nt) * nt : mt * nt ;
    }
    static i64 tri_tiles (int rows, int cols)
    {
        i64 mt = (rows + SMALL - 1) / SMALL, nt = (cols + SMALL - 1) / SMALL ;
        return nt * (nt + 1) / 2 + (mt - nt) * nt ;
    }
    XchgD xchg_of (int q, int c0) const
    {
        const FrontD &f = fr [ids [q]] ;
        int c1 = std::min (c0 + MB, f.nscol) ;
        int g = grpn [ids [q]], r = rank - grp0 [ids [q]] ;
        if (world == 1) { g = 1 ; r = 0 ; }
        const int OBq = ob_of (f), o1 = std::min ((c0 / OBq) * OBq + OBq, (int) f.nscol) ;
        auto chunk = [g] (int rows) { return rows > 0 ? (((rows + g - 1) / g) + 15) / 16 * 16 : 0 ; } ;
        const int mb = o1 - c1, mf = f.nsrow - o1 ;
        return XchgD {psx_at (ids [q], c0) + c0 + (i64) c0 * f.nsrow, f.nsrow, c1 - c0, mb, chunk (mb), g, r, o1 - c0, mf, chunk (mf)} ;
    }
    void chunk_rows (int q, int i0, int b1, int lo [3], int hi [3]) const
    {
        const FrontD &f = fr [ids [q]] ;
        lo [0] = b1 ; hi [0] = f.nsrow ; lo [1] = hi [1] = lo [2] = hi [2] = 0 ;
        if (!is_shared (ids [q])) return ;
        const int b0 = (i0 / MB) * MB ;
        XchgD X = xchg_of (q, b0) ;
        hi [0] = b0 + X.w ;
        lo [1] = b0 + X.w + X.r * X.R ; hi [1] = std::min (lo [1] + X.R, b0 + X.w + X.mb) ;
        lo [2] = b0 + X.fo + X.r * X.Rf ; hi [2] = std::min (lo [2] + X.Rf, (int) f.nsrow) ;
        for (int p = 1 ; p < 3 ; p++) if (hi [p] < lo [p]) hi [p] = lo [p] ;
    }
    int record_last ()
    {
        if (S.launches.size () == 0) return -1 ;
        if (S.launches.back ().rec_ev < 0) S.launches.back ().rec_ev = S.nevents++ ;
        return S.launches.back ().rec_ev ;
    }

    GemmGroup blank_region (int fid) const
    {
        GemmGroup G ;
        memset (&G, 0, sizeof (G)) ;
// ... 141 lines not shown
    }
    void flush_kind (std::vector<GemmGroup> &v, int kind)
    {
        if (v.empty ()) return ;
        const int T = kind == K_UPD_BIG ? BIG : SMALL ;
        Launch L {kind, 0, (int) v.size (), S.gg.size (), 0, 0} ;
        i64 tiles = 0 ;
        auto close_launch = [&] ()
        {
            L.ng = (int) (S.gg.size () - L.goff) ;
            L.grid = (int) tiles ;
            L.half = (kind == K_UPD_W && tiles < w_half_max) ? 1 : 0 ;
            if (L.ng) S.launches.push_back (L) ;
            L = Launch {L.kind, 0, 0, S.gg.size (), 0, 0} ;
            tiles = 0 ;
        } ;
        for (auto &G : v)
        {
            if (one_region && kind == K_UPD_W && S.gg.size () > L.goff) close_launch () ;
            const i64 mine = place_region (G, T, kind == K_UPD_W, tiles) ;
            if (mine == 0) continue ;
            const i64 cnt = G.ntiles ;
            G.nblk = (i32) mine ;
            G.tile_start = (i32) tiles ;
            tiles += mine ;
            double elems = G.tri ? (double) G.n * (G.n + 1) / 2 + (double) (G.m - G.n) * G.n : (double) G.m * G.n ;
            double share = (G.tile_mul == 1 && !G.tile_cnt) ? 1.0 : std::min (1.0, (double) mine / (double) cnt) ;
            L.flops += 2.0 * elems * G.k * share ;
            L.aux = std::max (L.aux, (int) G.k) ;
            L.bytes += ((G.assign ? 8.0 : 16.0) * elems + 8.0 * ((double) G.m + G.n) * G.k) * share ;
            S.gg.push_back (G) ;
        }
        close_launch () ;
        v.clear () ;
    }
    void flush_updates ()
    {
        if (w_min_tiles > 0 && !use_big)
        {
            i64 pooled = 0 ;
            if (by_launch) for (auto &G : small) if (G.k >= w_min_k || region_tiles (G) >= w_min_tiles) pooled += region_tiles (G) ;
            std::vector<GemmGroup> keep ;
            for (auto &G : small)
            {
                const bool w = region_tiles (G) >= w_min_tiles || (by_launch && pooled >= w_half_min && G.k >= w_min_k) ;
                if (w) wav.push_back (G) ; else keep.push_back (G) ;
            }
            small.swap (keep) ;
        }
        flush_kind (big, K_UPD_BIG) ;
        flush_kind (small, K_UPD_SMALL) ;
        flush_kind (pfv, K_UPD_PF) ;
        flush_kind (wav, K_UPD_W) ;
    }

    void emit_rs (int q, int c0, int wait_ev)
    {
        Launch La {K_XCHG_RS, 0, 0, 0, 0, 0} ;
        La.xd = xchg_of (q, c0) ;
        La.bytes = 8.0 * ((double) La.xd.w * La.xd.w + ((double) La.xd.R + La.xd.Rf) * La.xd.w) * La.xd.g ;
        La.ar_g0 = grp0 [ids [q]] ; La.ar_gn = grpn [ids [q]] ;
        La.wait_ev = wait_ev ;
        S.launches.push_back (La) ;
    }
    struct FarGather { int q, c0, ev ; } ;
    std::vector<FarGather> pending ;
    int far_ev = -1 ;
    Launch ag_launch (int q, int c0, int far) const
    {
        Launch La {K_XCHG_AG, 0, 0, 0, 0, 0} ;
        La.xd = xchg_of (q, c0) ;
        La.far = far ;
        La.bytes = 8.0 * (double) (far ? La.xd.Rf : La.xd.R) * La.xd.w * La.xd.g ;
        La.ar_g0 = grp0 [ids [q]] ; La.ar_gn = grpn [ids [q]] ;
        return La ;
    }
    void emit_ag (int q, int c0)
    {
        Launch Ln = ag_launch (q, c0, 0), Lf = ag_launch (q, c0, 1) ;
        if (Ln.xd.R > 0) S.launches.push_back (Ln) ;
        if (Lf.xd.Rf == 0) return ;
        if (xla) pending.push_back (FarGather {q, c0, -1}) ;
        else S.launches.push_back (Lf) ;
    }
    void issue_far_gathers ()
    {
        for (const FarGather &p : pending)
        {
            Launch Lf = ag_launch (p.q, p.c0, 1) ;
            Lf.stream = 1 ; Lf.wait_ev = p.ev ;
            S.launches.push_back (Lf) ;
            far_ev = -2 ;
        }
        if (far_ev == -2) far_ev = record_last () ;
        pending.clear () ;
    }
    void join_far_gathers ()
    {
        issue_far_gathers () ;
        if (far_ev < 0) return ;
        Launch Lj {K_JOIN, 0, 0, 0, 0, 0} ;
        Lj.wait_ev = far_ev ;
        S.launches.push_back (Lj) ;
        far_ev = -1 ;
    }
    void emit_win (int q, int mode, int ca, int cb, int stream, int wait_ev)
// ... 73 lines not shown

    int emit_next_columns_first ()
    {
        bool any_next = false ;
        if (xla)
            for (const Upd &x : step)
            {
                if (!x.wide || !is_shared (ids [x.q]) || x.t1 <= x.t0) continue ;
                const FrontD &f = fr [ids [x.q]] ;
                int tn = std::min (x.t0 + MB, x.t1) ;
                if (x.cb && windowed (ids [x.q])) add_outer_slabs (f, ids [x.q], x.kc, x.kk, x.t0, tn) ;
                else if (x.cb) add_update (f, ids [x.q], x.t0, x.kc, x.kk, f.nsrow - x.t0, tn - x.t0, false, true) ;
                else add_wide_shared (x, x.t0, tn) ;
                any_next = true ;
            }
        if (!any_next) return -2 ;
        flush_updates () ;
        return record_last () ;
    }
    bool unfuse_wide_k () const
    {
        i64 pooled = 0 ;
        if (by_launch && fuse_potrf && w_min_tiles > 0 && !use_big)
            for (const Upd &x : step)
            {
                const FrontD &f = fr [ids [x.q]] ;
                if (is_shared (ids [x.q]) || x.cb || x.kk < 512 || f.nscol - x.t0 < NB || x.t1 - x.t0 < NB) continue ;
                pooled += tri_tiles (f.nsrow - x.t0, x.t1 - x.t0) ;
            }
        return pooled >= 2 * unfuse_tiles ;
    }
    void emit_step ()
    {
        for (const Upd &x : step) if (x.cb && is_shared (ids [x.q])) { join_far_gathers () ; break ; }
        const int ev_next = emit_next_columns_first () ;
        const bool any_next = ev_next != -2 ;
        const bool ff_unfuse_wide_k = unfuse_wide_k () ;
        for (const Upd &x : step)
        {
            const FrontD &f = fr [ids [x.q]] ;
            const int fid = ids [x.q] ;
            int c0 = x.t0 ;
            bool ahead = any_next && x.wide && is_shared (fid) && x.t1 > x.t0 ;
            if (ahead) c0 = std::min (x.t0 + MB, x.t1) ;
            bool ff = fuse_potrf && !(x.wide && is_shared (fid)) && !x.cb && c0 == x.t0 && f.nscol - x.t0 >= NB && x.t1 - c0 >= NB ;
            if (ff && w_min_tiles > 0 && !use_big && !is_shared (fid))
            {
                if (tri_tiles (f.nsrow - c0, x.t1 - c0) >= unfuse_tiles) ff = false ;
                if (ff_unfuse_wide_k && x.kk >= 512) ff = false ;
            }
            if (ff) pf_done [x.q] = x.t0 ;
            if (!x.wide && is_shared (fid) && x.t1 > c0) { add_chunk_update (x, c0, ff) ; continue ; }
            if (x.wide && is_shared (fid) && !x.cb) { if (x.t1 > c0) add_wide_shared (x, c0, x.t1) ; continue ; }
            if (x.cb && windowed (fid)) { if (x.t1 > c0) add_outer_slabs (f, fid, x.kc, x.kk, c0, x.t1) ; }
            else if (x.t1 > c0) add_update (f, fid, c0, x.kc, x.kk, f.nsrow - c0, x.t1 - c0, false, x.wide, ff) ;
            if (x.cb && f.cbd) add_distributed_cb (x) ;
            else if (x.cb)
            {
                size_t nsm = small.size () ;
                add_update (f, fid, f.nscol, x.kc, x.kk, f.ncb, f.ncb, true, x.wide) ;
                if (windowed (fid) && f.own_g > 1 && balance_cb && small.size () > nsm) balance_cb_tiles (x) ;
            }
        }
        flush_updates () ;
        if (any_next)
            for (const Upd &x : step)
            {
                if (!x.wide || !is_shared (ids [x.q]) || x.t1 <= x.t0) continue ;
                if (x.cb && windowed (ids [x.q]))
                {
                    emit_win (x.q, 0, x.t0, std::min (x.t0 + MB, x.t1), 1, ev_next) ;
                    early_open [x.q] = x.t0 ;
                }
                emit_rs (x.q, x.t0, ev_next) ;
                early [x.q] = x.t0 ;
            }
        issue_far_gathers () ;
        step.clear () ;
    }
    void push_doubling_steps (int i0, int W, const std::vector<char> *skip)
    {
        for (int q = 0 ; q < nf ; q++)
        {
            const FrontD &f = fr [ids [q]] ;
            if (f.nscol <= i0 || (skip && (*skip) [q])) continue ;
            int OBq = ob_of (f) ;
            int o0 = (i0 / OBq) * OBq ;
            int o1 = std::min (o0 + OBq, (int) f.nscol) ;
            if (i0 + W >= o1)
            {
                step.push_back (Upd {q, o0, o1 - o0, o1, f.nscol, true, true}) ;
                continue ;
            }
            int e = (i0 - o0) / W + 1 ;
            int p = e & -e ;
            int t0 = o0 + e * W ;
            int t1 = std::min (o0 + (e + p) * W, o1) ;
            int kc = o0 + (e - p) * W ;
            step.push_back (Upd {q, kc, t0 - kc, t0, t1, false, p * W >= MB}) ;
        }
        emit_step () ;
    }

    void choose_chain ()
    {
        chain256 = (flags & CHOLMOD_HIP_CHAIN256) != 0 && !cx ;
        if (!chain256 && !cx && !twin && getenv ("CHOLMOD_HIP_CHAINF_AUTO") && atoi (getenv ("CHOLMOD_HIP_CHAINF_AUTO")) != 0 && !(flags & CHOLMOD_HIP_NO_FUSED_POTRF))
        {
            bool any_shared = false ;
            for (int q = 0 ; q < nf ; q++) if (is_shared (ids [q])) any_shared = true ;
            chain256 = !any_shared && maxnscol >= 192 && maxrows <= 16384 ;
        }
        bool any_win = false ;
        for (int q = 0 ; q < nf ; q++) if (windowed (ids [q])) any_win = true ;
        if (any_win)
        {
            const bool c64 = getenv ("CHOLMOD_HIP_SHARED_CHAIN64") || getenv ("CHOLMOD_HIP_NO_CHAINF") || cx || (flags & CHOLMOD_HIP_NO_FUSED_POTRF) ;
            chain256 = !c64 ;
        }
        fused256 = !getenv ("CHOLMOD_HIP_NO_CHAINF") ;
        fuse_potrf = !(flags & CHOLMOD_HIP_NO_FUSED_POTRF) && !chain256 ;
        fuse_trsm = fuse_potrf && !(flags & CHOLMOD_HIP_NO_FUSED_TRSM) ;
    }

    void emit_chainf (int i0)
    {
        const int SB = DG_W ;
        Launch Lc {K_CHAINF, 0, 0, S.cg.size (), 0, 0} ;
        int dblocks = 0, bblocks = 0, wmax = 0 ;
        for (int q = 0 ; q < nf ; q++)
        {
            const FrontD &f = fr [ids [q]] ;
            if (f.nscol <= i0) continue ;
            int OBq = ob_of (f) ;
            int o0 = (i0 / OBq) * OBq ;
            int o1 = std::min (o0 + OBq, (int) f.nscol) ;
            int b1 = std::min (i0 + SB, o1) ;
            int w = b1 - i0 ;
            int slot = (int) (S.cg.size () - Lc.goff) ;
            int lo [3], hi [3] ;
            chunk_rows (q, i0, b1, lo, hi) ;
            const int m1 = hi [0] - b1, m2 = hi [1] - lo [1], m3 = hi [2] - lo [2] ;
            S.cg.push_back (CfGroup {psx_at (ids [q], i0) + i0 + (i64) i0 * f.nsrow, f.nsrow, w, ids [q], i0, m1, slot, S.ncflags++, dblocks, bblocks,
                m2 ? lo [1] - i0 : 0, m2, m3 ? lo [2] - i0 : 0, m3, 0}) ;
            dblocks += (w + 63) / 64 ;
            bblocks += (m1 + 63) / 64 + (m2 + 63) / 64 + (m3 + 63) / 64 ;
            wmax = std::max (wmax, w) ;
            Lc.flops += (double) w * w * w / 3.0 + (double) (m1 + m2 + m3) * w * w ;
            Lc.bytes += 16.0 * (m1 + m2 + m3) * w ;
        }
        Lc.ng = (int) (S.cg.size () - Lc.goff) ; Lc.grid = dblocks + bblocks ; Lc.ndiag = dblocks ; Lc.aux = wmax ;
        S.max_dinv_slots = std::max (S.max_dinv_slots, Lc.ng) ;
        if (Lc.ng) S.launches.push_back (Lc) ;
    }
    void emit_diag_rowsolve (int i0)
    {
        const int SB = DG_W ;
        Launch Ld {K_DIAG, 0, 0, S.dg.size (), 0, 0} ;
        Launch Lr {K_ROWSOLVE, 0, 0, S.rg.size (), 0, 0} ;
        int rblocks = 0 ;
        for (int q = 0 ; q < nf ; q++)
        {
            const FrontD &f = fr [ids [q]] ;
            if (f.nscol <= i0) continue ;
            int OBq = ob_of (f) ;
            int o0 = (i0 / OBq) * OBq ;
            int o1 = std::min (o0 + OBq, (int) f.nscol) ;
            int b1 = std::min (i0 + SB, o1) ;
            int w = b1 - i0 ;
            int slot = (int) (S.dg.size () - Ld.goff) ;
            S.dg.push_back (DgGroup {psx_at (ids [q], i0) + i0 + (i64) i0 * f.nsrow, f.nsrow, w, ids [q], i0, slot, 0}) ;
            Ld.flops += (double) w * w * w / 3.0 ;
            int lo [3], hi [3] ;
            chunk_rows (q, i0, b1, lo, hi) ;
            for (int part = 0 ; part < 3 ; part++)
            {
                int m = hi [part] - lo [part] ;
                if (m <= 0) continue ;
                S.rg.push_back (RsGroup {psx_at (ids [q], i0) + i0 + (i64) i0 * f.nsrow, psx_at (ids [q], i0) + lo [part] + (i64) i0 * f.nsrow,
                    f.nsrow, m, w, ids [q], i0, rblocks, slot, 0}) ;
                rblocks += (m + RS_ROWS - 1) / RS_ROWS ;
                Lr.flops += (double) m * w * w ;
                Lr.bytes += 16.0 * m * w ;
            }
        }
        Ld.ng = Ld.grid = (int) (S.dg.size () - Ld.goff) ;
        S.max_dinv_slots = std::max (S.max_dinv_slots, Ld.ng) ;
        if (Ld.ng) S.launches.push_back (Ld) ;
        Lr.ng = (int) (S.rg.size () - Lr.goff) ; Lr.grid = rblocks ;
        if (Lr.ng) S.launches.push_back (Lr) ;
    }
    void run_chain256 ()
    {
        for (int i0 = 0 ; i0 < maxnscol ; i0 += DG_W)
        {
            enter_block_column (i0) ;
            if (fused256) emit_chainf (i0) ; else emit_diag_rowsolve (i0) ;
            leave_sub_block (i0, DG_W) ;
            push_doubling_steps (i0, DG_W, nullptr) ;
        }
    }

    void emit_potrf (int i0)
    {
        Launch Lp {K_POTRF, 0, 0, S.pg.size (), 0, 0} ;
        for (int q = 0 ; q < nf ; q++)
        {
            const FrontD &f = fr [ids [q]] ;
            if (f.nscol <= i0) continue ;
            if (pf_done [q] == i0) continue ;
            int nb = std::min (NB, f.nscol - i0) ;
            PfGroup G {psx_at (ids [q], i0) + i0 + co (i0, f.nsrow), f.nsrow, nb, ids [q], i0} ;
            S.pg.push_back (G) ;
            Lp.flops += (double) nb * nb * nb / 3.0 ;
        }
        Lp.ng = Lp.grid = (int) (S.pg.size () - Lp.goff) ;
        if (Lp.ng) S.launches.push_back (Lp) ;
    }
    void emit_trsm_upd (int i0, std::vector<char> &fused)
    {
        if (!fuse_trsm) return ;
        Launch Lf_ {K_TRSM_UPD, 0, 0, S.tg.size (), 0, 0} ;
        int fblocks = 0 ;
        for (int q = 0 ; q < nf ; q++)
        {
            const FrontD &f = fr [ids [q]] ;
            if (f.nscol < i0 + 2 * NB || is_shared (ids [q])) continue ;
            int OBq = ob_of (f) ;
            int o0 = (i0 / OBq) * OBq ;
            int o1 = std::min (o0 + OBq, (int) f.nscol) ;
            if (i0 + 2 * NB > o1) continue ;
            int e = (i0 - o0) / NB + 1 ;
            if ((e & -e) != 1) continue ;
            int m = f.nsrow - (i0 + NB) ;
            TrGroup G {f.psx + i0 + co (i0, f.nsrow),
                       f.psx + (i0 + NB) + co (i0, f.nsrow), f.nsrow, m, NB,
                       ids [q], i0, fblocks} ;
            fblocks += (m + TRM_ROWS - 1) / TRM_ROWS ;
            S.tg.push_back (G) ;
            Lf_.flops += (double) m * NB * NB + 2.0 * ((double) m * NB - (double) NB * (NB - 1) / 2) * NB + (double) NB * NB * NB / 3.0 ;
            Lf_.bytes += 8.0 * (3.0 * m * NB) ;
            fused [q] = 1 ;
            pf_done [q] = i0 + NB ;
        }
        Lf_.ng = (int) (S.tg.size () - Lf_.goff) ; Lf_.grid = fblocks ; Lf_.aux = NB ;
        if (Lf_.ng) S.launches.push_back (Lf_) ;
    }
    void emit_trsm (int i0, const std::vector<char> &fused)
    {
        Launch Lt {K_TRSM, 0, 0, S.tg.size (), 0, 0} ;
        int blocks = 0 ;
        for (int q = 0 ; q < nf ; q++)
        {
            const FrontD &f = fr [ids [q]] ;
            if (f.nscol <= i0 || fused [q]) continue ;
            int nb = std::min (NB, f.nscol - i0) ;
            int lo [3], hi [3] ;
            chunk_rows (q, i0, i0 + nb, lo, hi) ;
            for (int part = 0 ; part < 3 ; part++)
            {
                int m = hi [part] - lo [part] ;
                if (m <= 0) continue ;
                TrGroup G {psx_at (ids [q], i0) + i0 + co (i0, f.nsrow),
                           psx_at (ids [q], i0) + lo [part] + co (i0, f.nsrow), f.nsrow, m, nb,
                           ids [q], i0, blocks} ;
                blocks += (m + TRM_ROWS - 1) / TRM_ROWS ;
                S.tg.push_back (G) ;
                Lt.flops += (double) m * nb * nb ;
                Lt.aux = std::max (Lt.aux, (nb + 15) / 16 * 16) ;
            }
        }
        Lt.ng = (int) (S.tg.size () - Lt.goff) ; Lt.grid = blocks ;
        if (Lt.ng) S.launches.push_back (Lt) ;
    }
    void run_chain64 ()
    {
        for (int i0 = 0 ; i0 < maxnscol ; i0 += NB)
        {
            enter_block_column (i0) ;
            emit_potrf (i0) ;
            std::vector<char> fused (nf, 0) ;
            emit_trsm_upd (i0, fused) ;
            emit_trsm (i0, fused) ;
            leave_sub_block (i0, NB) ;
            push_doubling_steps (i0, NB, &fused) ;
        }
    }

    void run ()
    {
        if (chain256) run_chain256 () ; else run_chain64 () ;
        join_far_gathers () ;
    }
} ;

}

void schedule_dense (const std::vector<FrontD> &fr, const i32 *ids, int nf,
    Schedule &S, int flags, const i32 *owner, const i32 *grp0, const i32 *grpn, int rank, int world,
    const char *assign_cb, const i64 *win, const i32 *child, bool allow_half)
{
    DenseScheduler D (fr, ids, nf, S, flags, owner, grp0, grpn, rank, world, assign_cb, win, child, allow_half) ;
    D.run () ;
}

}
```

### suitesparse_amd/csrc/host/analyze.c

```c
#include "host_internal.h"
#include <time.h>
#include <stdio.h>
#include <stdlib.h>
#ifdef _OPENMP
#include <omp.h>
#endif


int ssamd_etree_upper (Int n, const Int *Up, const Int *Ui, Int *Parent)
{
    Int *anc = SuiteSparse_malloc ((size_t) (n > 0 ? n : 1), sizeof (Int)) ;
    if (!anc) return FALSE ;
    for (Int j = 0 ; j < n ; j++) { Parent [j] = EMPTY ; anc [j] = EMPTY ; }
    for (Int j = 0 ; j < n ; j++)
    {
        for (Int p = Up [j] ; p < Up [j+1] ; p++)
        {
            Int i = Ui [p] ;
            while (i < j)
            {
                Int up = anc [i] ;
                anc [i] = j ;
                if (up == EMPTY) { Parent [i] = j ; break ; }
                if (up == j) break ;
// ... 629 lines not shown
        ok = ok && ssamd_postorder (n, Parent, NULL, Post, work) == n ;
        double t3c = ssamd_now () ;
        if (ok) ssamd_colcounts (n, Lw->p, Lw->i, Parent, Post, ColCount, work) ;
        if (timing) fprintf (stderr, "cholmod_l_analyze:   etree %.3f s, postorder %.3f s, colcounts %.3f s\n",
            t3b - t3a, t3c - t3b, ssamd_now () - t3c) ;
        if (ok)
        {
            double fl = 0, lnz = 0 ;
            for (Int j = 0 ; j < n ; j++) { double c = (double) ColCount [j] ; fl += c * c ; lnz += c ; }
            Common->fl = fl ; Common->lnz = lnz ;
            Common->anz = (double) ((Int *) U->p) [n] ;
            Common->method [0].fl = fl ; Common->method [0].lnz = lnz ;
            Common->selected = 0 ;
            if (Common->nmethods == 0 && L->ordering != CHOLMOD_POSTORDERED) Common->method [0].ordering = L->ordering ;
        }
        if (ok && Common->postorder)
        {
            double t4a = ssamd_now () ;
            const Int npost = ssamd_postorder (n, Parent, ColCount, Post, work) ;
            if (npost == EMPTY) ok = FALSE ;
            else if (npost == n)
            {
                double t4b = ssamd_now () ;
                Int *tmp = work, *inv = work + n ;
                for (Int k = 0 ; k < n ; k++) tmp [k] = Perm [Post [k]] ;
                for (Int k = 0 ; k < n ; k++) Perm [k] = tmp [k] ;
                for (Int k = 0 ; k < n ; k++) tmp [k] = ColCount [Post [k]] ;
                for (Int k = 0 ; k < n ; k++) ColCount [k] = tmp [k] ;
                for (Int k = 0 ; k < n ; k++) inv [Post [k]] = k ;
                for (Int c = 0 ; c < n ; c++)
                {
                    Int op = Parent [Post [c]] ;
                    tmp [c] = (op == EMPTY) ? EMPTY : inv [op] ;
                }
                for (Int k = 0 ; k < n ; k++) Parent [k] = tmp [k] ;
                if (L->ordering == CHOLMOD_NATURAL) L->ordering = CHOLMOD_POSTORDERED ;
                cholmod_l_free_sparse (&U, Common) ;
                cholmod_l_free_sparse (&Lw, Common) ;
                if (A->stype < 0) U = cholmod_l_ptranspose (A, 0, Perm, NULL, 0, Common) ;
                else
                {
                    Lw = cholmod_l_ptranspose (A, 0, Perm, NULL, 0, Common) ;
                    if (Lw) U = cholmod_l_ptranspose (Lw, 0, NULL, NULL, 0, Common) ;
                }
                ok = (U != NULL) ;
                if (timing) fprintf (stderr, "cholmod_l_analyze:   weighted postorder %.3f s, compose + permuted pattern %.3f s\n",
                    t4b - t4a, ssamd_now () - t4b) ;
            }
        }
    }
    tt [3] = ssamd_now () ;
    if (ok) ok = cholmod_l_super_symbolic2 (for_whom, U, NULL, Parent, L, Common) ;
    tt [4] = ssamd_now () ;
    if (timing)
        fprintf (stderr, "cholmod_l_analyze: ordering %.3f s, permute %.3f s, etree+colcounts+postorder(+re-permute) %.3f s, super_symbolic %.3f s\n",
            tt [1] - tt [0], tt [2] - tt [1], tt [3] - tt [2], tt [4] - tt [3]) ;
    cholmod_l_free_sparse (&U, Common) ;
    cholmod_l_free_sparse (&Lw, Common) ;
    if (Parent) cholmod_l_free (n + 1, sizeof (Int), Parent, Common) ;
    if (Post) cholmod_l_free (n + 1, sizeof (Int), Post, Common) ;
    if (work) cholmod_l_free (5 * (size_t) n + 1, sizeof (Int), work, Common) ;
    if (Apk) cholmod_l_free_sparse (&Apk, Common) ;
    if (!ok)
    {
        if (Common->status == CHOLMOD_OK) ERROR (CHOLMOD_OUT_OF_MEMORY, "analyze failed") ;
        cholmod_l_free_factor (&L, Common) ;
        return NULL ;
    }
    if (for_whom == CHOLMOD_ANALYZE_FOR_CHOLESKY && A->xtype == CHOLMOD_REAL && !Common->hip_lazy_plan)
    {
        double tp = ssamd_now () ;
        ssamd_plan_ahead (L, Common) ;
        if (timing) fprintf (stderr, "cholmod_l_analyze: engine plan (schedule, maps, HBM reservation) %.3f s%s\n", ssamd_now () - tp,
            L->hip_plan ? "" : " -- none built") ;
    }
    return L ;
}

cholmod_factor *cholmod_l_analyze_p (cholmod_sparse *A, SuiteSparse_long *UserPerm,
    SuiteSparse_long *fset, size_t fsize, cholmod_common *Common)
{
    return cholmod_l_analyze_p2 (CHOLMOD_ANALYZE_FOR_CHOLESKY, A, UserPerm, fset, fsize, Common) ;
}

cholmod_factor *cholmod_l_analyze (cholmod_sparse *A, cholmod_common *Common)
{
    return cholmod_l_analyze_p2 (CHOLMOD_ANALYZE_FOR_CHOLESKY, A, NULL, NULL, 0, Common) ;
}
```

### suitesparse_amd/csrc/host/host_internal.h

```cpp
#ifndef SSAMD_HOST_INTERNAL_H
#define SSAMD_HOST_INTERNAL_H

#include <limits.h>
#include <math.h>
#include <stdint.h>
#include <stdio.h>
#include <stdlib.h>
#include <string.h>

#include "../../../include/SuiteSparse_config.h"
#include "../../../include/cholmod.h"
#include "../../../include/cholmod_hip.h"

typedef SuiteSparse_long Int ;
#define EMPTY (-1)

#define SSAMD_XENT(xtype) ((size_t) ((xtype) == CHOLMOD_COMPLEX ? 2 : 1))

#define ERROR(status, msg) cholmod_l_error (status, __FILE__, __LINE__, msg, Common)

#define RETURN_IF_NULL_COMMON(result) \
    do { if (Common == NULL) return (result) ; \
         if (Common->itype != CHOLMOD_LONG || Common->dtype != CHOLMOD_DOUBLE) \
         { Common->status = CHOLMOD_INVALID ; return (result) ; } } while (0)

#define RETURN_IF_NULL(A, result) \
    do { if ((A) == NULL) { \
             if (Common->status != CHOLMOD_OUT_OF_MEMORY) { ERROR (CHOLMOD_INVALID, "argument missing") ; } \
             return (result) ; } } while (0)

int ssamd_host_threads (void) ;
int ssamd_host_threads_uncapped (void) ;
cholmod_sparse *ssamd_aat (cholmod_sparse *A, cholmod_sparse *F, int values, int lower, cholmod_common *Common) ;
cholmod_sparse *ssamd_column_subset (cholmod_sparse *A, const SuiteSparse_long *fset, size_t fsize, int values, cholmod_common *Common) ;
cholmod_sparse *ssamd_sym_permute (cholmod_sparse *A, int values, SuiteSparse_long *Perm, int upper_out,
    cholmod_common *Common) ;
cholmod_sparse *ssamd_sym_permute_src (cholmod_sparse *A, int values, SuiteSparse_long *Perm, int upper_out,
    SuiteSparse_long **src_out, cholmod_common *Common) ;

int ssamd_etree_upper (Int n, const Int *Up, const Int *Ui, Int *Parent) ;
Int ssamd_postorder (Int n, const Int *Parent, const Int *Weight, Int *Post, Int *work3n) ;
void ssamd_colcounts (Int n, const Int *Lp, const Int *Li, const Int *Parent, const Int *Post,
    Int *ColCount, Int *work5n) ;

int ssamd_nested_dissection (Int n, const Int *Ap, const Int *Ai, Int *Perm, cholmod_common *Common) ;
int ssamd_resolve_use_gpu (cholmod_common *Common) ;
int ssamd_ensure_plan (cholmod_factor *L, cholmod_common *Common) ;
void ssamd_plan_ahead (cholmod_factor *L, cholmod_common *Common) ;

int ssamd_complex_super_numeric (cholmod_sparse *A, double beta, cholmod_factor *L, cholmod_common *Common) ;
int ssamd_complex_sync_host (cholmod_factor *L, cholmod_common *Common) ;
cholmod_factor *ssamd_complex_twin (cholmod_factor *L, cholmod_common *Common) ;

int ssamd_cpu_super_numeric (cholmod_sparse *A, double beta, cholmod_factor *L, cholmod_common *Common) ;
void ssamd_cpu_super_solve (int which, const cholmod_factor *L, double *X, Int nrhs, Int ldx) ;
const char *ssamd_cpu_blas_name (void) ;
int ssamd_cpu_max_threads (void) ;
int ssamd_cpu_quota (void) ;
int ssamd_factor_has_cholesky_sizes (const cholmod_factor *L) ;
int ssamd_solve_subset (int sys, cholmod_factor *L, cholmod_dense *B, cholmod_sparse *Bset, cholmod_dense *X,
    cholmod_sparse **Xset_Handle, cholmod_dense **Y_Handle, cholmod_common *Common) ;

#endif
```

### suitesparse_amd/csrc/host/numeric.c

```c
#include "host_internal.h"
#ifdef _OPENMP
#include <omp.h>
#else
static int omp_get_thread_num (void) { return 0 ; }
#endif
#include <time.h>


int cholmod_l_gpu_memorysize (size_t *total_mem, size_t *available_mem, cholmod_common *Common)
{
    if (total_mem) *total_mem = 0 ;
    if (available_mem) *available_mem = 0 ;
    if (!Common) return 1 ;
    return cholmod_hip_memorysize (total_mem, available_mem) ;
}

int cholmod_l_gpu_probe (cholmod_common *Common)
{
    if (!Common) return 0 ;
    if (!cholmod_hip_probe ()) return 0 ;
    size_t t = 0, a = 0 ;
    if (cholmod_hip_memorysize (&t, &a) == 0) Common->gpuMemorySize = a ;
    return 1 ;
}
// ... 15 lines not shown
    if (!Common) return 1 ;
    return cholmod_hip_probe () ? 0 : 1 ;
}

int cholmod_l_gpu_deallocate (cholmod_common *Common)
{
    if (!Common) return 1 ;
    return 0 ;
}

void cholmod_l_gpu_end (cholmod_common *Common)
{
    (void) Common ;
}


static int map_hip_status (int rc, cholmod_common *Common, const char *what)
{
    switch (rc)
    {
        case CHOLMOD_HIP_OK: return TRUE ;
        case CHOLMOD_HIP_NOT_POSDEF: return TRUE ;
        case CHOLMOD_HIP_OUT_OF_MEMORY: ERROR (CHOLMOD_OUT_OF_MEMORY, what) ; return FALSE ;
        case CHOLMOD_HIP_INVALID: ERROR (CHOLMOD_INVALID, what) ; return FALSE ;
        case CHOLMOD_HIP_TOO_LARGE: ERROR (CHOLMOD_TOO_LARGE, "problem too large for the HIP engine (32-bit maps)") ; return FALSE ;
        case CHOLMOD_HIP_NO_DEVICE:
            ERROR (CHOLMOD_GPU_PROBLEM, "no usable HIP device: the numeric factorization of this "
                "library runs only on the GPU engine") ;
            return FALSE ;
        default: ERROR (CHOLMOD_GPU_PROBLEM, what) ; return FALSE ;
    }
}

int ssamd_factor_has_cholesky_sizes (const cholmod_factor *L)
{
    if (!L || !L->is_super || !L->px || !L->super || !L->pi) return FALSE ;
    const Int *px = L->px ;
    if (L->nsuper > 0 && px [0] == 123456) return FALSE ;
    return (size_t) px [L->nsuper] <= L->xsize ;
}

static int plan_flags_of (const cholmod_factor *L, const cholmod_common *Common)
{
    int flags = Common->hip_flags ;
    if (L->hip_is_twin == 2) flags |= CHOLMOD_HIP_CX_STORAGE ;
    else if (L->hip_is_twin)
    {
        const char *e = getenv ("CHOLMOD_HIP_TWIN_FULL_K") ;
        if (!(e && atoi (e) != 0)) flags |= CHOLMOD_HIP_PHI_TWIN ;
    }
    return flags ;
}

int ssamd_ensure_plan (cholmod_factor *L, cholmod_common *Common)
{
    if (!ssamd_factor_has_cholesky_sizes (L))
    { ERROR (CHOLMOD_INVALID, "L was analysed for SPQR (no Cholesky sizes)") ; return FALSE ; }
    int st = 0 ;
    int world = Common->hip_world > 1 ? Common->hip_world : 1 ;
    const int flags = plan_flags_of (L, Common) ;
    if (L->hip_plan && L->hip_plan_ahead && !L->hip_on_device && (L->hip_plan_ahead - 1 != flags || world > 1))
    {
        cholmod_hip_plan_destroy ((cholmod_hip_plan *) L->hip_plan) ;
        L->hip_plan = NULL ;
    }
    L->hip_plan_ahead = 0 ;
    if (L->hip_plan) return TRUE ;
    const double t_plan = omp_get_wtime () ;
    cholmod_hip_plan *P = cholmod_hip_plan_create_dist ((int64_t) L->n, (int64_t) L->nsuper,
        L->super, L->pi, L->px, L->s, flags, world > 1 ? Common->hip_rank : 0, world, &st) ;
    Common->hip_plan_seconds = omp_get_wtime () - t_plan ;
    if (!P) return map_hip_status (st ? st : CHOLMOD_HIP_GPU_PROBLEM, Common, "HIP plan creation failed") ;
    if (Common->hip_allreduce)
        cholmod_hip_set_allreduce (P, Common->hip_allreduce, Common->hip_allreduce_user) ;
    L->hip_plan = P ;
    return TRUE ;
}

void ssamd_plan_ahead (cholmod_factor *L, cholmod_common *Common)
{
    if (!L || !L->is_super || !L->useGPU || L->hip_plan || Common->useGPU != 1) return ;
    if (Common->hip_world > 1 || Common->hip_allreduce) return ;
    if (!ssamd_factor_has_cholesky_sizes (L) || !cholmod_hip_probe ()) return ;
    const int st = Common->status, tc = Common->try_catch ;
    Common->try_catch = TRUE ;
    if (ssamd_ensure_plan (L, Common)) L->hip_plan_ahead = plan_flags_of (L, Common) + 1 ;
    Common->try_catch = tc ; Common->status = st ;
}

static void absorb_stats (cholmod_factor *L, cholmod_common *Common)
{
    double s [CHOLMOD_HIP_NSTATS] ;
    if (cholmod_hip_get_stats ((cholmod_hip_plan *) L->hip_plan, s) != CHOLMOD_HIP_OK) return ;
    Common->gpuKernelTime = s [0] ;
    Common->gpuFlops = (SuiteSparse_long) s [1] ;
    Common->gpuNumKernelLaunches = (int) s [2] ;
    Common->cholmod_gpu_syrk_time = s [6] + s [14] + s [27] + s [32] ;
    Common->cholmod_gpu_syrk_calls = (size_t) (s [7] + s [26] + s [33]) ;
    Common->cholmod_gpu_gemm_time = 0 ; Common->cholmod_gpu_gemm_calls = 0 ;
    Common->cholmod_gpu_potrf_time = s [11] ;
    Common->cholmod_gpu_trsm_time = s [12] ;
    Common->cholmod_assemble_time = s [13] ;
    Common->cholmod_assemble_time2 = s [9] ;
    Common->cholmod_cpu_gemm_time = Common->cholmod_cpu_syrk_time = 0 ;
    Common->cholmod_cpu_trsm_time = Common->cholmod_cpu_potrf_time = 0 ;
    Common->cholmod_cpu_gemm_calls = Common->cholmod_cpu_syrk_calls = 0 ;
    Common->cholmod_cpu_trsm_calls = Common->cholmod_cpu_potrf_calls = 0 ;
}


static int back_to_symbolic (cholmod_factor *L)
{
    L->xtype = CHOLMOD_PATTERN ; L->minor = L->n ;
    L->hip_on_device = FALSE ; L->hip_host_valid = FALSE ;
    return FALSE ;
}

static int finish_numeric (int rc, int64_t minor, cholmod_factor *L, cholmod_common *Common)
{
    const int was_symbolic = (L->xtype == CHOLMOD_PATTERN && !L->x) ;
    if (rc < 0)
    {
        if (was_symbolic || !(L->x && L->hip_host_valid)) back_to_symbolic (L) ;
        else L->hip_on_device = FALSE ;
        return map_hip_status (rc, Common, "HIP factorization failed") ;
    }
    L->xtype = CHOLMOD_REAL ;
    L->dtype = CHOLMOD_DOUBLE ;
    L->is_ll = TRUE ;
    L->minor = (size_t) minor ;
    L->hip_on_device = TRUE ;
    L->hip_host_valid = FALSE ;
    if (!Common->hip_factor_on_device)
    {
        if (Common->hip_world > 1)
        {
            int rg = cholmod_hip_gather_factor ((cholmod_hip_plan *) L->hip_plan) ;
            if (rg != CHOLMOD_HIP_OK) { if (was_symbolic) back_to_symbolic (L) ; return map_hip_status (rg, Common, "factor gather failed") ; }
        }
// ... 797 lines not shown
```

Measured before the change: 61250 GFLOP/s.

## Skip structurally zero rows in large-front updates via row reach gathering

Computes, at analysis time, the first column at which each row of a wide supernode (at least 512 columns) becomes nonzero, and passes this to the plan. A new gathered update kernel (k_update3g) uses a row map so the update GEMMs touch only rows that are nonzero at the current panel, skipping structurally zero work inside large fronts. The cost is extra index indirection in loads and stores, extra symbolic work during analysis, and more schedule state to carry.

```diff
diff --git a/include/cholmod.h b/include/cholmod.h
--- a/include/cholmod.h
+++ b/include/cholmod.h
@@ -282,6 +282,8 @@
 
 int cholmod_l_factor_to_host (cholmod_factor *L, cholmod_common *Common) ;
 int cholmod_l_hip_stats (cholmod_factor *L, double *stats, cholmod_common *Common) ;
+int64_t cholmod_l_hip_front_reach (cholmod_sparse *A, cholmod_factor *L, int64_t *reach_p, int32_t *reach_first,
+    cholmod_common *Common) ;
 int cholmod_l_hip_prepare (cholmod_factor *L, cholmod_common *Common) ;
 int cholmod_l_gather_factor (cholmod_factor *L, cholmod_common *Common) ;
 int cholmod_l_refactorize_resident (double beta [2], cholmod_factor *L,
diff --git a/include/cholmod_hip.h b/include/cholmod_hip.h
--- a/include/cholmod_hip.h
+++ b/include/cholmod_hip.h
@@ -46,6 +46,10 @@
     const int64_t *s, int flags, int *status) ;
 
 void cholmod_hip_plan_destroy (cholmod_hip_plan *plan) ;
+
+cholmod_hip_plan *cholmod_hip_plan_create_reach (int64_t n, int64_t nsuper,
+    const int64_t *super, const int64_t *pi, const int64_t *px,
+    const int64_t *s, int flags, const int64_t *reach_p, const int32_t *reach_first, int *status) ;
 
 typedef int (*cholmod_hip_allreduce_fn) (void *dev_ptr, int64_t count_doubles,
     int group_first, int group_size, void *user) ;
@@ -100,7 +104,7 @@
 int cholmod_hip_factor_checks (cholmod_hip_plan *plan, double *out5) ;
 int cholmod_hip_factor_checks_local (cholmod_hip_plan *plan, double *out5) ;
 
-#define CHOLMOD_HIP_NSTATS 40
+#define CHOLMOD_HIP_NSTATS 41
 int cholmod_hip_get_stats (cholmod_hip_plan *plan, double *stats) ;
 int cholmod_hip_set_profiling (cholmod_hip_plan *plan, int on) ;
 int64_t cholmod_hip_get_launch_profile (cholmod_hip_plan *plan, int64_t cap, int32_t *kind,
diff --git a/suitesparse_amd/cholmod.py b/suitesparse_amd/cholmod.py
--- a/suitesparse_amd/cholmod.py
+++ b/suitesparse_amd/cholmod.py
@@ -12,7 +12,7 @@
 CSRC = os.path.join(_HERE, "csrc")
 
 CHOLMOD_MAXMETHODS = 9
-CHOLMOD_HIP_NSTATS = 40
+CHOLMOD_HIP_NSTATS = 41
 
 PATTERN, REAL, COMPLEX, ZOMPLEX = 0, 1, 2, 3
 OK, NOT_INSTALLED, OUT_OF_MEMORY, TOO_LARGE, INVALID, GPU_PROBLEM = 0, -1, -2, -3, -4, -5
@@ -129,12 +129,12 @@
     "cholmod_l_gpu_memorysize", "cholmod_l_gpu_probe", "cholmod_l_gpu_deallocate",
     "cholmod_l_gpu_end", "cholmod_l_gpu_allocate",
     "cholmod_l_factor_to_host", "cholmod_l_hip_stats", "cholmod_l_refactorize_resident",
-    "cholmod_l_gather_factor", "cholmod_l_hip_prepare",
+    "cholmod_l_gather_factor", "cholmod_l_hip_prepare", "cholmod_l_hip_front_reach",
 ]
 HIP_SYMBOLS = [
     "cholmod_hip_probe", "cholmod_hip_memorysize", "cholmod_hip_set_device", "cholmod_hip_device_count",
     "cholmod_hip_plan_create", "cholmod_hip_plan_destroy", "cholmod_hip_factorize",
-    "cholmod_hip_plan_create_dist", "cholmod_hip_set_allreduce", "cholmod_hip_get_partition",
+    "cholmod_hip_plan_create_dist", "cholmod_hip_plan_create_reach", "cholmod_hip_set_allreduce", "cholmod_hip_get_partition",
     "cholmod_hip_get_groups", "cholmod_hip_get_batches", "cholmod_hip_progress_enable", "cholmod_hip_progress", "cholmod_hip_debug_schedule_hash", "cholmod_hip_diag_minmax", "cholmod_hip_values_staging", "cholmod_hip_values_push", "cholmod_hip_values_commit", "cholmod_hip_values_gather_index", "cholmod_hip_values_begin", "cholmod_hip_values_push_chunk", "cholmod_hip_debug_routing",
     "cholmod_hip_gather_factor",
     "cholmod_hip_upload_matrix", "cholmod_hip_factorize_resident",
@@ -244,6 +244,8 @@
     sig("cholmod_hip_plan_destroy", None, [vp])
     sig("cholmod_hip_plan_create_dist", vp, [i64, i64, vp, vp, vp, vp, C.c_int, C.c_int, C.c_int,
                                              C.POINTER(C.c_int)])
+    sig("cholmod_hip_plan_create_reach", vp, [i64, i64, vp, vp, vp, vp, C.c_int, vp, vp, C.POINTER(C.c_int)])
+    sig("cholmod_l_hip_front_reach", i64, [sp, fc, vp, vp, cm])
     sig("cholmod_hip_set_allreduce", C.c_int, [vp, ALLREDUCE_FN, vp])
     sig("cholmod_hip_get_partition", C.c_int, [vp, vp])
     sig("cholmod_hip_get_groups", C.c_int, [vp, vp, vp])
diff --git a/suitesparse_amd/csrc/hip/descriptors.hip.h b/suitesparse_amd/csrc/hip/descriptors.hip.h
--- a/suitesparse_amd/csrc/hip/descriptors.hip.h
+++ b/suitesparse_amd/csrc/hip/descriptors.hip.h
@@ -61,6 +61,8 @@
     i32 tile_cnt;
 };
 
+struct GatherGroup { GemmGroup g; i64 map; i32 tile_start; i32 pad; };
+
 __host__ __device__ __forceinline__ int tri_col (int j, int m) { return j * m - ((j * (j + 1)) >> 1) ; }
 
 struct RelPair { i32 d ; i32 a ; i64 off ; } ;
diff --git a/suitesparse_amd/csrc/hip/engine.hip b/suitesparse_amd/csrc/hip/engine.hip
--- a/suitesparse_amd/csrc/hip/engine.hip
+++ b/suitesparse_amd/csrc/hip/engine.hip
@@ -64,7 +64,8 @@
     void *ptrs [] = {P->d_Ls, P->d_fr, P->d_supermap, P->d_child, P->d_relmap, P->d_info,
         P->d_lvl_list, P->d_Lx, P->d_cb, P->d_zg, P->d_eg, P->d_pg, P->d_tg, P->d_tu_cnt, P->d_cdesc, P->d_smd, P->d_sp01, P->d_gg, P->d_sm,
         P->d_Sp, P->d_Si, P->d_Snz, P->d_Sx, P->d_amap, P->d_X, P->d_Y, P->d_perm, P->d_xchg, P->d_stage, P->d_ag, P->d_agf, P->d_Lx_full, P->d_fr_full, P->d_dg, P->d_rg, P->d_wg, P->d_cg, P->d_cflags, P->d_crel, P->d_relpairs, P->d_dinv, P->d_sv,
-        P->d_inv_tasks, P->d_winv, P->d_solved, P->d_sv_acc, P->d_ticket, P->d_chk, P->d_chk_out, P->d_thin_tim, P->d_sb_tasks, P->d_sb_commit, P->d_first_fail, P->d_vsrc, P->d_vals} ;
+        P->d_inv_tasks, P->d_winv, P->d_solved, P->d_sv_acc, P->d_ticket, P->d_chk, P->d_chk_out, P->d_thin_tim, P->d_sb_tasks, P->d_sb_commit, P->d_first_fail, P->d_vsrc, P->d_vals,
+        P->d_xg, P->d_gmap} ;
     for (void *p : ptrs) if (p) (void) hipFree (p) ;
     for (auto e : P->evpool) (void) hipEventDestroy (e) ;
     for (auto e : P->sync_ev) (void) hipEventDestroy (e) ;
@@ -145,6 +146,8 @@
     P->d_rg = dupload (P->sch.rg, e) ; HIPCHK (e) ;
     P->d_wg = dupload (P->sch.wg, e) ; HIPCHK (e) ;
     P->d_cg = dupload (P->sch.cg, e) ; HIPCHK (e) ;
+    P->d_xg = dupload (P->sch.xg, e) ; HIPCHK (e) ;
+    P->d_gmap = dupload (P->sch.gmap, e) ; HIPCHK (e) ;
     HIPCHK (hipMalloc ((void **) &P->d_cflags, (4 * (size_t) P->sch.ncflags + 4) * sizeof (int))) ;
     HIPCHK (hipMalloc ((void **) &P->d_dinv, (size_t) std::max (P->sch.max_dinv_slots, 1) * 4096 * sizeof (double))) ;
     P->d_sm = dupload (P->sch.sm, e) ; HIPCHK (e) ;
@@ -433,6 +436,16 @@
             else if (L.aux >= 1024) TW_LAUNCH (k_update3<4 COMMA, >, dim3 (L.grid), dim3 (64), 0, st, P->d_gg + L.goff, L.ng, P->d_Lx, P->d_cb) ;
             else TW_LAUNCH (k_update3<2 COMMA, >, dim3 (L.grid), dim3 (64), 0, st, P->d_gg + L.goff, L.ng, P->d_Lx, P->d_cb) ;
             break ;
+        case K_UPD_G:
+            if (L.half)
+            {
+                const unsigned gh = 2u * (unsigned) ((L.grid + 7) / 8 * 8) ;
+                if (L.aux >= 1024) hipLaunchKernelGGL ((k_update3g<4, true>), dim3 (gh), dim3 (64), 0, st, P->d_xg + L.goff, L.ng, P->d_gmap, P->d_Lx, P->d_cb) ;
+                else hipLaunchKernelGGL ((k_update3g<2, true>), dim3 (gh), dim3 (64), 0, st, P->d_xg + L.goff, L.ng, P->d_gmap, P->d_Lx, P->d_cb) ;
+            }
+            else if (L.aux >= 1024) hipLaunchKernelGGL ((k_update3g<4, false>), dim3 (L.grid), dim3 (64), 0, st, P->d_xg + L.goff, L.ng, P->d_gmap, P->d_Lx, P->d_cb) ;
+            else hipLaunchKernelGGL ((k_update3g<2, false>), dim3 (L.grid), dim3 (64), 0, st, P->d_xg + L.goff, L.ng, P->d_gmap, P->d_Lx, P->d_cb) ;
+            break ;
         case K_UPD_PF:
             TW_LAUNCH (k_update2f<, >, dim3 (L.grid), dim3 (256), 0, st,
                 P->d_gg + L.goff, L.ng, P->d_Lx, P->d_cb, P->d_info) ;
@@ -676,7 +689,8 @@
     {
         const Launch &L = P->sch.launches [q] ;
         if (L.kind == K_UPD_SMALL) { S [7] += 1 ; S [8] += L.flops ; S [16] += L.bytes ; }
-        if (L.kind == K_UPD_W) { S [33] += 1 ; S [34] += L.flops ; S [35] += L.bytes ; }
+        if (L.kind == K_UPD_W || L.kind == K_UPD_G) { S [33] += 1 ; S [34] += L.flops ; S [35] += L.bytes ; }
+        if (L.kind == K_UPD_G) S [40] += L.skipped ;
         if (L.kind == K_UPD_PF) { S [26] += 1 ; S [28] += L.flops ; S [29] += L.bytes ; }
         if (L.kind == K_TRSM_UPD) S [31] += 1 ;
         if (L.kind == K_SMALL) { S [20] += L.bytes ; S [21] += L.ng ; }
@@ -706,7 +720,7 @@
             {
                 case K_UPD_SMALL: S [6] += sec ; if (L.aux < MB) { S [23] += sec ; } break ;
                 case K_UPD_PF: S [27] += sec ; break ;
-                case K_UPD_W: S [32] += sec ; break ;
+                case K_UPD_W: case K_UPD_G: S [32] += sec ; break ;
                 case K_UPD_BIG: S [14] += sec ; break ;
                 case K_EA: case K_ZERO: case K_WIN: S [9] += sec ; break ;
                 case K_POTRF: case K_DIAG: case K_CHAINF: S [11] += sec ; break ;
@@ -798,7 +812,7 @@
 
 static cholmod_hip_plan *plan_create_impl (int64_t n, int64_t nsuper,
     const int64_t *super, const int64_t *pi, const int64_t *px, const int64_t *s,
-    int flags, int rank, int world, int *status) ;
+    int flags, int rank, int world, int *status, const int64_t *reach_p = nullptr, const int32_t *reach_first = nullptr) ;
 
 cholmod_hip_plan *cholmod_hip_plan_create_dist (int64_t n, int64_t nsuper,
     const int64_t *super, const int64_t *pi, const int64_t *px, const int64_t *s,
@@ -810,9 +824,19 @@
     catch (const std::bad_alloc &) { *status = CHOLMOD_HIP_OUT_OF_MEMORY ; return nullptr ; }
 }
 
+cholmod_hip_plan *cholmod_hip_plan_create_reach (int64_t n, int64_t nsuper,
+    const int64_t *super, const int64_t *pi, const int64_t *px, const int64_t *s,
+    int flags, const int64_t *reach_p, const int32_t *reach_first, int *status)
+{
+    int st_local ;
+    if (!status) status = &st_local ;
+    try { return plan_create_impl (n, nsuper, super, pi, px, s, flags, 0, 1, status, reach_p, reach_first) ; }
+    catch (const std::bad_alloc &) { *status = CHOLMOD_HIP_OUT_OF_MEMORY ; return nullptr ; }
+}
+
 static cholmod_hip_plan *plan_create_impl (int64_t n, int64_t nsuper,
     const int64_t *super, const int64_t *pi, const int64_t *px, const int64_t *s,
-    int flags, int rank, int world, int *status)
+    int flags, int rank, int world, int *status, const int64_t *reach_p, const int32_t *reach_first)
 {
     *status = CHOLMOD_HIP_OK ;
     if (n < 0 || nsuper < 0 || !super || !pi || !px || !s || world < 1 || rank < 0 || rank >= world)
@@ -845,6 +869,17 @@
     P->px.assign (px, px + nsuper + 1) ;
     P->ssize = pi [nsuper] ; P->xsize = px [nsuper] ;
     P->Ls.assign (s, s + std::max<i64> (P->ssize, 1)) ;
+    if (reach_p && reach_first)
+    {
+        for (i64 q = 0 ; q < nsuper ; q++)
+        {
+            const i64 len = reach_p [q + 1] - reach_p [q] ;
+            if (len < 0 || (len != 0 && len != pi [q + 1] - pi [q])) { *status = CHOLMOD_HIP_INVALID ; return nullptr ; }
+        }
+        P->reach_p.assign (reach_p, reach_p + nsuper + 1) ;
+        P->reach_first.assign (reach_first + reach_p [0], reach_first + reach_p [nsuper]) ;
+        for (i64 &v : P->reach_p) v -= reach_p [0] ;
+    }
     {
         const char *e = getenv ("CHOLMOD_HIP_ARENA_BUDGET_MB") ;
         double fixed = 8.0 * P->xsize + 8.0 * P->ssize + 4.0 * (P->ssize - n) + 3e9 ;
@@ -1763,7 +1798,9 @@
     } ;
     const Schedule &S = P->sch ;
     out16 [0] = hv (S.zg) ; out16 [1] = hv (S.eg) ; out16 [2] = hv (S.pg) ; out16 [3] = hv (S.tg) ;
-    out16 [4] = hv (S.gg) ; out16 [5] = hv (S.dg) ; out16 [6] = hv (S.rg) ; out16 [7] = hv (S.wg) ;
+    out16 [4] = hv (S.gg) ;
+    if (!S.xg.empty ()) out16 [4] = fnv (fnv (out16 [4], S.xg.data (), S.xg.size () * sizeof (GatherGroup)), S.gmap.data (), S.gmap.size () * sizeof (i32)) ;
+    out16 [5] = hv (S.dg) ; out16 [6] = hv (S.rg) ; out16 [7] = hv (S.wg) ;
     out16 [8] = hv (S.cg) ; out16 [9] = hv (S.sm) ;
     uint64_t h = H0 ;
     for (const Launch &L : S.launches)
diff --git a/suitesparse_amd/csrc/hip/kernels.hip.h b/suitesparse_amd/csrc/hip/kernels.hip.h
--- a/suitesparse_amd/csrc/hip/kernels.hip.h
+++ b/suitesparse_amd/csrc/hip/kernels.hip.h
@@ -1505,9 +1505,11 @@
 #ifndef UPD3_CLAMP_LOADS
 #define UPD3_CLAMP_LOADS 0
 #endif
-template <int DEPTH, bool EDGE, int TW = 0, int NQ = 2>
-__device__ __forceinline__ void update_tile_w (const GemmGroup &G, int I, int J, double *Lx, double *CB, int cofs = 0)
-{
+template <int DEPTH, bool EDGE, int TW = 0, int NQ = 2, bool GATHER = false>
+__device__ __forceinline__ void update_tile_w (const GemmGroup &G, int I, int J, double *Lx, double *CB, int cofs = 0,
+    const i32 *rmap = nullptr)
+{
+    static_assert (!GATHER || (TW == 0 && !UPD3_CLAMP_LOADS), "a gathered tile is real and loads row pairs") ;
     const int lane = threadIdx.x & 63, lr = lane & 15, lk = lane >> 4 ;
     const int row0 = I * 64, col0 = J * 64 + cofs ;
     const int mrem = G.m - row0, nrem = G.n - col0 ;
@@ -1529,8 +1531,18 @@
                 if (rb [q][h] > nrem - 1) rb [q][h] = nrem - 1 ;
             }
         }
-        pa [q] = Lx + G.a_off + row0 + (i64) lk * lda ;
-        pb [q] = Lx + G.b_off + col0 + (i64) lk * lda ;
+        if constexpr (GATHER)
+        {
+            const int ia = min (row0 + ra [q][0], G.m - 1), ib = min (col0 + rb [q][0], G.n - 1) ;
+            pa [q] = Lx + G.a_off + rmap [ia] + (i64) lk * lda ;
+            pb [q] = Lx + G.b_off + rmap [ib] + (i64) lk * lda ;
+            ra [q][0] = rb [q][0] = 0 ; ra [q][1] = rb [q][1] = 1 ;
+        }
+        else
+        {
+            pa [q] = Lx + G.a_off + row0 + (i64) lk * lda ;
+            pb [q] = Lx + G.b_off + col0 + (i64) lk * lda ;
+        }
     }
     struct Frag { double a [4], b [2 * NQ] ; } ;
     auto load = [&] (Frag &F, int kk)
@@ -1635,6 +1647,13 @@
                 }
     }
     double *C = (G.c_in_cb ? CB : Lx) + G.c_off + row0 + colx<TW == 2> (col0, G.ldc) ;
+    double *Cg = GATHER ? (G.c_in_cb ? CB : Lx) + G.c_off : nullptr ;
+    int rg [2] = {0, 0} ;
+    if constexpr (GATHER)
+    {
+#pragma unroll
+        for (int q = 0 ; q < 2 ; q++) rg [q] = rmap [min (row0 + 32 * q + 2 * lr, G.m - 1)] ;
+    }
     const bool diag = G.tri && I == J ;
 #pragma unroll
     for (int b = 0 ; b < 2 * NQ ; b++)
@@ -1644,11 +1663,12 @@
             if (TW == 2 && (b & 1)) continue ;
             const int j = 32 * (b >> 1) + 2 * (lk + 4 * r) + (b & 1) ;
             const int jd = j + cofs ;
-            double *Cj = C + colx<TW == 2> (j, G.ldc) ;
+            double *Cj = GATHER ? Cg + (i64) rmap [min (col0 + j, G.n - 1)] * G.ldc : C + colx<TW == 2> (j, G.ldc) ;
 #pragma unroll
             for (int q = 0 ; q < 2 ; q++)
             {
                 const int i = 32 * q + 2 * lr ;
+                const int io = GATHER ? rg [q] : i ;
                 auto store_pair = [&] ()
                 {
                     if (diag && i + 1 < jd) return ;
@@ -1656,11 +1676,11 @@
                     if (G.assign) { v.x = -acc [2 * q][b][r] ; v.y = -acc [2 * q + 1][b][r] ; }
                     else
                     {
-                        v = *(const d2u *) (Cj + i) ;
+                        v = *(const d2u *) (Cj + io) ;
                         v.x -= acc [2 * q][b][r] ; v.y -= acc [2 * q + 1][b][r] ;
                     }
-                    if (diag && i < jd) Cj [i + 1] = v.y ;
-                    else *(d2u *) (Cj + i) = v ;
+                    if (diag && i < jd) Cj [io + 1] = v.y ;
+                    else *(d2u *) (Cj + io) = v ;
                 } ;
                 if constexpr (EDGE)
                 {
@@ -1669,8 +1689,8 @@
                         if (i + 1 < mrem) store_pair () ;
                         else if (i < mrem && (!diag || i >= jd))
                         {
-                            if (G.assign) Cj [i] = -acc [2 * q][b][r] ;
-                            else Cj [i] -= acc [2 * q][b][r] ;
+                            if (G.assign) Cj [io] = -acc [2 * q][b][r] ;
+                            else Cj [io] -= acc [2 * q][b][r] ;
                         }
                     }
                 }
@@ -1701,6 +1721,31 @@
     {
         if (G.m - I * 64 >= 64 && G.n - J * 64 >= 64) update_tile_w<DEPTH, false, TW> (G, I, J, Lx, CB) ;
         else update_tile_w<DEPTH, true, TW> (G, I, J, Lx, CB) ;
+    }
+}
+
+template <int DEPTH, bool HALF = false>
+__global__ void __launch_bounds__(64, 2) k_update3g (const GatherGroup *g, int ng, const i32 *rmap, double *Lx, double *CB)
+{
+    int vb = (int) blockIdx.x ;
+    int cofs = 0 ;
+    if constexpr (HALF) { cofs = ((vb >> 3) & 1) * 32 ; vb = ((vb >> 4) << 3) | (vb & 7) ; }
+    const int gi = find_group (g, ng, vb, &GatherGroup::tile_start) ;
+    const GemmGroup G = g [gi].g ;
+    const i32 *map = rmap + g [gi].map ;
+    int I, J ;
+    if (vb - G.tile_start >= G.nblk) return ;
+    if (!decode_tile (G, vb - G.tile_start, I, J)) return ;
+    if constexpr (HALF)
+    {
+        if (G.n - J * 64 - cofs <= 0) return ;
+        if (G.m - I * 64 >= 64 && G.n - J * 64 - cofs >= 32) update_tile_w<DEPTH, false, 0, 1, true> (G, I, J, Lx, CB, cofs, map) ;
+        else update_tile_w<DEPTH, true, 0, 1, true> (G, I, J, Lx, CB, cofs, map) ;
+    }
+    else
+    {
+        if (G.m - I * 64 >= 64 && G.n - J * 64 >= 64) update_tile_w<DEPTH, false, 0, 2, true> (G, I, J, Lx, CB, 0, map) ;
+        else update_tile_w<DEPTH, true, 0, 2, true> (G, I, J, Lx, CB, 0, map) ;
     }
 }
 
diff --git a/suitesparse_amd/csrc/hip/plan.hip.h b/suitesparse_amd/csrc/hip/plan.hip.h
--- a/suitesparse_amd/csrc/hip/plan.hip.h
+++ b/suitesparse_amd/csrc/hip/plan.hip.h
@@ -54,7 +54,7 @@
 static inline i64 window_len (const FrontD &f, int ob) { return (i64) f.nsrow * std::min (ob, (int) f.nscol) ; }
 static inline int window_count (const FrontD &f, int ob) { return f.nscol > ob ? 2 : 1 ; }
 
-enum Kind { K_ZERO = 0, K_EA, K_POTRF, K_TRSM, K_UPD_BIG, K_UPD_SMALL, K_JOIN, K_XCHG_RS, K_SMALL, K_UPD_PF, K_TRSM_UPD, K_XCHG_AG, K_UPD_W, K_DIAG, K_ROWSOLVE, K_WIN, K_CHAINF, K_NKIND } ;
+enum Kind { K_ZERO = 0, K_EA, K_POTRF, K_TRSM, K_UPD_BIG, K_UPD_SMALL, K_JOIN, K_XCHG_RS, K_SMALL, K_UPD_PF, K_TRSM_UPD, K_XCHG_AG, K_UPD_W, K_DIAG, K_ROWSOLVE, K_WIN, K_CHAINF, K_UPD_G, K_NKIND } ;
 
 struct Launch {
     int kind ;
@@ -74,6 +74,7 @@
     int leaf_pw = 0 ;
     int ndiag = 0 ;
     int half = 0 ;
+    double skipped = 0 ;
 } ;
 
 #define HIPCHK(call) do { hipError_t e_ = (call) ; if (e_ != hipSuccess) { \
@@ -156,6 +157,8 @@
     std::vector<RsGroup> rg ;
     std::vector<WinD> wg ;
     std::vector<CfGroup> cg ;
+    std::vector<GatherGroup> xg ;
+    std::vector<i32> gmap ;
     int ncflags = 0 ;
     int max_dinv_slots = 0 ;
     std::vector<i32> sm ;
@@ -248,6 +251,10 @@
     double *d_chk_out = nullptr ;
     Schedule sch ;
     double exec_flops = 0 ;
+    std::vector<i64> reach_p ;
+    std::vector<i32> reach_first, head ;
+    bool head_gather = true ;
+    GatherGroup *d_xg = nullptr ; i32 *d_gmap = nullptr ;
     hipStream_t stream = nullptr ;
     hipStream_t stream2 = nullptr ;
     std::vector<hipEvent_t> sync_ev ;
@@ -310,9 +317,12 @@
 
 namespace sship {
 
+struct HeadInfo { const i32 *head ; const i64 *reach_p ; const i32 *first ; bool gather ; } ;
+
 int build_host (cholmod_hip_plan *P) ;
 void schedule_dense (const std::vector<FrontD> &fr, const i32 *ids, int nf,
     Schedule &S, int flags, const i32 *owner, const i32 *grp0, const i32 *grpn, int rank, int world,
-    const char *assign_cb = nullptr, const i64 *win = nullptr, const i32 *child = nullptr, bool allow_half = false) ;
-
-}
+    const char *assign_cb = nullptr, const i64 *win = nullptr, const i32 *child = nullptr, bool allow_half = false,
+    const HeadInfo *heads = nullptr) ;
+
+}
diff --git a/suitesparse_amd/csrc/hip/plan_build.hip b/suitesparse_amd/csrc/hip/plan_build.hip
--- a/suitesparse_amd/csrc/hip/plan_build.hip
+++ b/suitesparse_amd/csrc/hip/plan_build.hip
@@ -655,9 +655,45 @@
             schedule_extend_add (ids, nf, 0) ;
             schedule_dense (P->fr, ids, nf, S, P->flags, P->owner.data (), P->grp0.data (), P->grpn.data (),
                 P->rank, P->world, P->assign_cb.data (), P->win_off.data (), P->child.data (),
-                P->world == 1 && !P->force_shared) ;
+                P->world == 1 && !P->force_shared,
+                P->head.empty () ? nullptr : &heads) ;
             schedule_extend_add (ids, nf, 1) ;
         }
+    }
+
+    HeadInfo heads {nullptr, nullptr, nullptr, true} ;
+    void choose_heads ()
+    {
+        P->head.clear () ;
+        if (P->reach_p.empty () || P->world != 1 || P->force_shared || getenv ("CHOLMOD_HIP_NO_HEADS")) return ;
+        if (P->flags & (CHOLMOD_HIP_PHI_TWIN | CHOLMOD_HIP_CX_STORAGE | CHOLMOD_HIP_TILE128)) return ;
+        const ObThresholds obt = outer_block_thresholds () ;
+        const bool all = getenv ("CHOLMOD_HIP_HEAD_ALL") && atoi (getenv ("CHOLMOD_HIP_HEAD_ALL")) != 0 ;
+        auto rate = [] (int K) { return 1e12 * (K < 512 ? 60.0 : K < 1024 ? 70.0 : K < 2048 ? 74.5 : 75.0) ; } ;
+        auto tri = [] (double m) { return m * (m + 1) / 2 ; } ;
+        std::vector<i32> head (P->nsuper, 0) ;
+        bool any = false ;
+        for (i64 s = 0 ; s < P->nsuper ; s++)
+        {
+            const FrontD &f = P->fr [s] ;
+            if (P->reach_p [s + 1] - P->reach_p [s] != f.nsrow || P->owner [s] < 0) continue ;
+            const i32 *first = P->reach_first.data () + P->reach_p [s] ;
+            const int OB = front_ob (f, P->flags, obt) ;
+            double best = all ? 0.0 : 0.25e-3 ;
+            for (int H = 256 ; H < std::min (OB, (int) f.nscol) ; H += 256)
+            {
+                i64 R = 0 ;
+                for (int p = H ; p < f.nsrow ; p++) R += first [p] < H ;
+                const double N = f.nsrow - H ;
+                const double gain = all ? 2.0 * H * (tri (N) - tri ((double) R))
+                    : 2.0 * H * tri (N) / rate (OB) - 2.0 * H * tri ((double) R) / rate (H) - 16.0 * tri (N) / 4e12 ;
+                if (gain > best) { best = gain ; head [s] = H ; any = true ; }
+            }
+        }
+        if (!any) return ;
+        P->head.swap (head) ;
+        P->head_gather = !getenv ("CHOLMOD_HIP_HEAD_NO_GATHER") ;
+        heads = HeadInfo {P->head.data (), P->reach_p.data (), P->reach_first.data (), P->head_gather} ;
     }
 
     int run ()
@@ -667,12 +703,14 @@
         rc = build_etree () ;
         if (rc != CHOLMOD_HIP_OK) return rc ;
         assign_ownership () ;
+        choose_heads () ;
         layout_local_factor () ;
         build_child_lists () ;
         choose_batches () ;
         build_solve_tasks () ;
         layout_windows () ;
         schedule_batches () ;
+        for (const Launch &L : P->sch.launches) P->stats [40] += L.skipped ;
         return CHOLMOD_HIP_OK ;
     }
 } ;
diff --git a/suitesparse_amd/csrc/hip/schedule_dense.hip b/suitesparse_amd/csrc/hip/schedule_dense.hip
--- a/suitesparse_amd/csrc/hip/schedule_dense.hip
+++ b/suitesparse_amd/csrc/hip/schedule_dense.hip
@@ -17,6 +17,7 @@
     const i64 *win ;
     const i32 *child ;
     const bool allow_half ;
+    const HeadInfo *heads ;
     bool cx, twin, use_big ;
     ObThresholds obt ;
     int maxnscol = 0, maxrows = 0 ;
@@ -35,6 +36,8 @@
     std::vector<GemmGroup> big, small ;
     std::vector<GemmGroup> pfv ;
     std::vector<GemmGroup> wav ;
+    std::vector<GatherGroup> gav ;
+    double gav_skipped = 0 ;
     std::vector<int> early ;
     std::vector<int> early_open ;
     std::vector<int> pf_done ;
@@ -42,9 +45,9 @@
 
     DenseScheduler (const std::vector<FrontD> &fr_, const i32 *ids_, int nf_, Schedule &S_, int flags_, const i32 *owner_,
         const i32 *grp0_, const i32 *grpn_, int rank_, int world_, const char *assign_cb_, const i64 *win_, const i32 *child_,
-        bool allow_half_)
+        bool allow_half_, const HeadInfo *heads_)
         : fr (fr_), ids (ids_), nf (nf_), S (S_), flags (flags_), owner (owner_), grp0 (grp0_), grpn (grpn_), rank (rank_),
-          world (world_), assign_cb (assign_cb_), win (win_), child (child_), allow_half (allow_half_)
+          world (world_), assign_cb (assign_cb_), win (win_), child (child_), allow_half (allow_half_), heads (heads_)
     {
         cx = (flags & CHOLMOD_HIP_CX_STORAGE) != 0 ;
         twin = (flags & CHOLMOD_HIP_PHI_TWIN) != 0 || cx ;
@@ -77,6 +80,16 @@
         G.k /= 2 ;
     }
     int ob_of (const FrontD &f) const { return front_ob (f, flags, obt) ; }
+    int head_of (int fid) const { return heads && heads->head ? heads->head [fid] : 0 ; }
+    void ob_bounds (int q, int i0, int &o0, int &o1) const
+    {
+        const FrontD &f = fr [ids [q]] ;
+        const int OBq = ob_of (f), H = head_of (ids [q]) ;
+        if (H > 0 && i0 < H) o0 = 0 ;
+        else if (H > 0) o0 = H + ((i0 - H) / OBq) * OBq ;
+        else o0 = (i0 / OBq) * OBq ;
+        o1 = std::min (o0 + (H > 0 && i0 < H ? H : OBq), (int) f.nscol) ;
+    }
     bool is_shared (int fid) const { return owner && owner [fid] < 0 ; }
     bool windowed (int fid) const { return win && win [fid] >= 0 ; }
     i64 psx_at (int fid, int col) const
@@ -324,6 +337,79 @@
         flush_kind (small, K_UPD_SMALL) ;
         flush_kind (pfv, K_UPD_PF) ;
         flush_kind (wav, K_UPD_W) ;
+        flush_gathered () ;
+    }
+    void add_head_gathered (const Upd &x)
+    {
+        const int fid = ids [x.q], H = x.kk ;
+        const FrontD &f = fr [fid] ;
+        const i32 *first = heads->first + heads->reach_p [fid] ;
+        auto tri_elems = [] (double m, double n) { return n * (n + 1) / 2 + (m - n) * n ; } ;
+        double full = tri_elems (f.nsrow - H, f.nscol - H) + tri_elems (f.ncb, f.ncb), done = 0 ;
+        auto gathered = [&] (int from, int ncols, bool to_cb)
+        {
+            const size_t m0 = S.gmap.size () ;
+            int n = 0 ;
+            for (int p = from ; p < f.nsrow ; p += 2)
+            {
+                if (first [p] >= H && (p + 1 >= f.nsrow || first [p + 1] >= H)) continue ;
+                S.gmap.push_back (p) ; n += p < from + ncols ;
+                if (p + 1 < f.nsrow) { S.gmap.push_back (p + 1) ; n += p + 1 < from + ncols ; }
+            }
+            const int m = (int) (S.gmap.size () - m0) ;
+            if (n == 0) { S.gmap.resize (m0) ; return ; }
+            GatherGroup X ;
+            memset (&X, 0, sizeof (X)) ;
+            X.g = blank_region (fid) ;
+            X.g.a_off = X.g.b_off = f.psx ; X.g.lda = f.nsrow ;
+            if (to_cb) { X.g.c_off = f.cb - f.nscol - (i64) f.nscol * f.ncb ; X.g.ldc = f.ncb ; X.g.c_in_cb = 1 ; }
+            else { X.g.c_off = f.psx ; X.g.ldc = f.nsrow ; }
+            X.g.m = m ; X.g.n = n ; X.g.k = H ; X.g.tri = 1 ;
+            X.g.assign = (to_cb && assign_cb && assign_cb [fid]) ? 1 : 0 ;
+            X.map = (i64) m0 ;
+            done += tri_elems (m, n) ;
+            gav.push_back (X) ;
+        } ;
+        if (x.t1 > x.t0) gathered (H, f.nscol - H, false) ;
+        if (f.ncb > 0)
+        {
+            if (assign_cb && assign_cb [fid])
+            {
+                Launch Lz {K_ZERO, 0, 0, S.zg.size (), 0, 0} ;
+                S.zg.push_back (ZeroGroup {f.cb, (i64) f.ncb, 0, 0}) ;
+                Lz.ng = 1 ; Lz.grid = (f.ncb + ZERO_COLS - 1) / ZERO_COLS ;
+                Lz.bytes = 8.0 * (double) f.ncb * (f.ncb + 1) / 2 ;
+                S.launches.push_back (Lz) ;
+            }
+            gathered (f.nscol, f.ncb, true) ;
+        }
+        gav_skipped += 2.0 * H * std::max (0.0, full - done) ;
+    }
+    void flush_gathered ()
+    {
+        if (gav.empty ()) return ;
+        Launch L {K_UPD_G, 0, 0, S.xg.size (), 0, 0} ;
+        i64 tiles = 0 ;
+        for (GatherGroup &X : gav)
+        {
+            GemmGroup &G = X.g ;
+            const i64 mine = place_region (G, SMALL, true, tiles) ;
+            G.nblk = (i32) mine ;
+            G.tile_start = X.tile_start = (i32) tiles ;
+            tiles += mine ;
+            const double elems = (double) G.n * (G.n + 1) / 2 + (double) (G.m - G.n) * G.n ;
+            L.flops += 2.0 * elems * G.k ;
+            L.aux = std::max (L.aux, (int) G.k) ;
+            L.bytes += (G.assign ? 8.0 : 16.0) * elems + 8.0 * ((double) G.m + G.n) * G.k ;
+            S.xg.push_back (X) ;
+        }
+        L.ng = (int) (S.xg.size () - L.goff) ;
+        L.grid = (int) tiles ;
+        L.half = tiles < w_half_max ? 1 : 0 ;
+        L.skipped = gav_skipped ;
+        S.launches.push_back (L) ;
+        gav.clear () ;
+        gav_skipped = 0 ;
     }
 
     void emit_rs (int q, int c0, int wait_ev)
@@ -503,6 +589,7 @@
             if (ff) pf_done [x.q] = x.t0 ;
             if (!x.wide && is_shared (fid) && x.t1 > c0) { add_chunk_update (x, c0, ff) ; continue ; }
             if (x.wide && is_shared (fid) && !x.cb) { if (x.t1 > c0) add_wide_shared (x, c0, x.t1) ; continue ; }
+            if (x.cb && x.kc == 0 && x.kk == head_of (fid) && heads->gather) { add_head_gathered (x) ; continue ; }
             if (x.cb && windowed (fid)) { if (x.t1 > c0) add_outer_slabs (f, fid, x.kc, x.kk, c0, x.t1) ; }
             else if (x.t1 > c0) add_update (f, fid, c0, x.kc, x.kk, f.nsrow - c0, x.t1 - c0, false, x.wide, ff) ;
             if (x.cb && f.cbd) add_distributed_cb (x) ;
@@ -535,9 +622,8 @@
         {
             const FrontD &f = fr [ids [q]] ;
             if (f.nscol <= i0 || (skip && (*skip) [q])) continue ;
-            int OBq = ob_of (f) ;
-            int o0 = (i0 / OBq) * OBq ;
-            int o1 = std::min (o0 + OBq, (int) f.nscol) ;
+            int o0, o1 ;
+            ob_bounds (q, i0, o0, o1) ;
             if (i0 + W >= o1)
             {
                 step.push_back (Upd {q, o0, o1 - o0, o1, f.nscol, true, true}) ;
@@ -583,9 +669,8 @@
         {
             const FrontD &f = fr [ids [q]] ;
             if (f.nscol <= i0) continue ;
-            int OBq = ob_of (f) ;
-            int o0 = (i0 / OBq) * OBq ;
-            int o1 = std::min (o0 + OBq, (int) f.nscol) ;
+            int o0, o1 ;
+            ob_bounds (q, i0, o0, o1) ;
             int b1 = std::min (i0 + SB, o1) ;
             int w = b1 - i0 ;
             int slot = (int) (S.cg.size () - Lc.goff) ;
@@ -614,9 +699,8 @@
         {
             const FrontD &f = fr [ids [q]] ;
             if (f.nscol <= i0) continue ;
-            int OBq = ob_of (f) ;
-            int o0 = (i0 / OBq) * OBq ;
-            int o1 = std::min (o0 + OBq, (int) f.nscol) ;
+            int o0, o1 ;
+            ob_bounds (q, i0, o0, o1) ;
             int b1 = std::min (i0 + SB, o1) ;
             int w = b1 - i0 ;
             int slot = (int) (S.dg.size () - Ld.goff) ;
@@ -677,9 +761,8 @@
         {
             const FrontD &f = fr [ids [q]] ;
             if (f.nscol < i0 + 2 * NB || is_shared (ids [q])) continue ;
-            int OBq = ob_of (f) ;
-            int o0 = (i0 / OBq) * OBq ;
-            int o1 = std::min (o0 + OBq, (int) f.nscol) ;
+            int o0, o1 ;
+            ob_bounds (q, i0, o0, o1) ;
             if (i0 + 2 * NB > o1) continue ;
             int e = (i0 - o0) / NB + 1 ;
             if ((e & -e) != 1) continue ;
@@ -749,9 +832,9 @@
 
 void schedule_dense (const std::vector<FrontD> &fr, const i32 *ids, int nf,
     Schedule &S, int flags, const i32 *owner, const i32 *grp0, const i32 *grpn, int rank, int world,
-    const char *assign_cb, const i64 *win, const i32 *child, bool allow_half)
+    const char *assign_cb, const i64 *win, const i32 *child, bool allow_half, const HeadInfo *heads)
 {
-    DenseScheduler D (fr, ids, nf, S, flags, owner, grp0, grpn, rank, world, assign_cb, win, child, allow_half) ;
+    DenseScheduler D (fr, ids, nf, S, flags, owner, grp0, grpn, rank, world, assign_cb, win, child, allow_half, heads) ;
     D.run () ;
 }
 
diff --git a/suitesparse_amd/csrc/host/analyze.c b/suitesparse_amd/csrc/host/analyze.c
--- a/suitesparse_amd/csrc/host/analyze.c
+++ b/suitesparse_amd/csrc/host/analyze.c
@@ -705,6 +705,10 @@
     tt [3] = ssamd_now () ;
     if (ok) ok = cholmod_l_super_symbolic2 (for_whom, U, NULL, Parent, L, Common) ;
     tt [4] = ssamd_now () ;
+    int64_t *reach_p = NULL ; int32_t *reach_first = NULL ;
+    const int ahead = ok && for_whom == CHOLMOD_ANALYZE_FOR_CHOLESKY && A->xtype == CHOLMOD_REAL && !Common->hip_lazy_plan ;
+    if (ahead && L->is_super && L->useGPU && Common->useGPU == 1 && Common->hip_world <= 1 && U)
+        ssamd_front_reach_alloc (U, L, &reach_p, &reach_first) ;
     if (timing)
         fprintf (stderr, "cholmod_l_analyze: ordering %.3f s, permute %.3f s, etree+colcounts+postorder(+re-permute) %.3f s, super_symbolic %.3f s\n",
             tt [1] - tt [0], tt [2] - tt [1], tt [3] - tt [2], tt [4] - tt [3]) ;
@@ -716,14 +720,16 @@
     if (Apk) cholmod_l_free_sparse (&Apk, Common) ;
     if (!ok)
     {
+        free (reach_p) ; free (reach_first) ;
         if (Common->status == CHOLMOD_OK) ERROR (CHOLMOD_OUT_OF_MEMORY, "analyze failed") ;
         cholmod_l_free_factor (&L, Common) ;
         return NULL ;
     }
-    if (for_whom == CHOLMOD_ANALYZE_FOR_CHOLESKY && A->xtype == CHOLMOD_REAL && !Common->hip_lazy_plan)
+    if (ahead)
     {
         double tp = ssamd_now () ;
-        ssamd_plan_ahead (L, Common) ;
+        ssamd_plan_ahead (L, Common, reach_p, reach_first) ;
+        free (reach_p) ; free (reach_first) ;
         if (timing) fprintf (stderr, "cholmod_l_analyze: engine plan (schedule, maps, HBM reservation) %.3f s%s\n", ssamd_now () - tp,
             L->hip_plan ? "" : " -- none built") ;
     }
diff --git a/suitesparse_amd/csrc/host/host_internal.h b/suitesparse_amd/csrc/host/host_internal.h
--- a/suitesparse_amd/csrc/host/host_internal.h
+++ b/suitesparse_amd/csrc/host/host_internal.h
@@ -46,7 +46,9 @@
 int ssamd_nested_dissection (Int n, const Int *Ap, const Int *Ai, Int *Perm, cholmod_common *Common) ;
 int ssamd_resolve_use_gpu (cholmod_common *Common) ;
 int ssamd_ensure_plan (cholmod_factor *L, cholmod_common *Common) ;
-void ssamd_plan_ahead (cholmod_factor *L, cholmod_common *Common) ;
+void ssamd_plan_ahead (cholmod_factor *L, cholmod_common *Common, const int64_t *reach_p, const int32_t *reach_first) ;
+int64_t ssamd_front_reach (const cholmod_sparse *U, const cholmod_factor *L, int64_t *reach_p, int32_t *reach_first) ;
+void ssamd_front_reach_alloc (const cholmod_sparse *U, const cholmod_factor *L, int64_t **reach_p, int32_t **reach_first) ;
 
 int ssamd_complex_super_numeric (cholmod_sparse *A, double beta, cholmod_factor *L, cholmod_common *Common) ;
 int ssamd_complex_sync_host (cholmod_factor *L, cholmod_common *Common) ;
diff --git a/suitesparse_amd/csrc/host/numeric.c b/suitesparse_amd/csrc/host/numeric.c
--- a/suitesparse_amd/csrc/host/numeric.c
+++ b/suitesparse_amd/csrc/host/numeric.c
@@ -91,7 +91,10 @@
     return flags ;
 }
 
-int ssamd_ensure_plan (cholmod_factor *L, cholmod_common *Common)
+static int ensure_plan_with (cholmod_factor *L, cholmod_common *Common, const int64_t *reach_p, const int32_t *reach_first) ;
+int ssamd_ensure_plan (cholmod_factor *L, cholmod_common *Common) { return ensure_plan_with (L, Common, NULL, NULL) ; }
+
+static int ensure_plan_with (cholmod_factor *L, cholmod_common *Common, const int64_t *reach_p, const int32_t *reach_first)
 {
     if (!ssamd_factor_has_cholesky_sizes (L))
     { ERROR (CHOLMOD_INVALID, "L was analysed for SPQR (no Cholesky sizes)") ; return FALSE ; }
@@ -106,8 +109,11 @@
     L->hip_plan_ahead = 0 ;
     if (L->hip_plan) return TRUE ;
     const double t_plan = omp_get_wtime () ;
-    cholmod_hip_plan *P = cholmod_hip_plan_create_dist ((int64_t) L->n, (int64_t) L->nsuper,
-        L->super, L->pi, L->px, L->s, flags, world > 1 ? Common->hip_rank : 0, world, &st) ;
+    cholmod_hip_plan *P = (reach_p && world == 1)
+        ? cholmod_hip_plan_create_reach ((int64_t) L->n, (int64_t) L->nsuper, L->super, L->pi, L->px, L->s, flags,
+            reach_p, reach_first, &st)
+        : cholmod_hip_plan_create_dist ((int64_t) L->n, (int64_t) L->nsuper,
+            L->super, L->pi, L->px, L->s, flags, world > 1 ? Common->hip_rank : 0, world, &st) ;
     Common->hip_plan_seconds = omp_get_wtime () - t_plan ;
     if (!P) return map_hip_status (st ? st : CHOLMOD_HIP_GPU_PROBLEM, Common, "HIP plan creation failed") ;
     if (Common->hip_allreduce)
@@ -116,14 +122,100 @@
     return TRUE ;
 }
 
-void ssamd_plan_ahead (cholmod_factor *L, cholmod_common *Common)
+#define REACH_MIN_COLS 512
+int64_t ssamd_front_reach (const cholmod_sparse *U, const cholmod_factor *L, int64_t *reach_p, int32_t *reach_first)
+{
+    const Int nsuper = (Int) L->nsuper, n = (Int) L->n ;
+    const Int *super = L->super, *pi = L->pi, *Ls = L->s ;
+    if (!U || !L->is_super || (Int) U->ncol != n) return -1 ;
+    reach_p [0] = 0 ;
+    for (Int s = 0 ; s < nsuper ; s++)
+    {
+        const Int nscol = super [s + 1] - super [s], nsrow = pi [s + 1] - pi [s] ;
+        reach_p [s + 1] = reach_p [s] + (nscol >= REACH_MIN_COLS ? nsrow : 0) ;
+    }
+    if (!reach_first || reach_p [nsuper] == 0) return reach_p [nsuper] ;
+    Int *smap = malloc ((size_t) (n > 0 ? n : 1) * sizeof (Int)) ;
+    if (!smap) return -1 ;
+    for (Int s = 0 ; s < nsuper ; s++)
+        for (Int k = super [s] ; k < super [s + 1] ; k++) smap [k] = s ;
+    for (int64_t q = 0 ; q < reach_p [nsuper] ; q++) reach_first [q] = INT32_MAX ;
+    for (Int s = 0 ; s < nsuper ; s++)
+        if (reach_p [s + 1] > reach_p [s])
+            for (Int p = 0 ; p < super [s + 1] - super [s] ; p++) reach_first [reach_p [s] + p] = (int32_t) p ;
+    #define ROW_POS(s, i, pos) do { Int lo_ = pi [s], hi_ = pi [s + 1] ; \
+        while (lo_ < hi_) { Int mid_ = (lo_ + hi_) >> 1 ; if (Ls [mid_] < (i)) lo_ = mid_ + 1 ; else hi_ = mid_ ; } \
+        (pos) = (lo_ < pi [s + 1] && Ls [lo_] == (i)) ? lo_ - pi [s] : -1 ; } while (0)
+    const Int *Up = U->p, *Ui = U->i, *Unz = U->nz ;
+    for (Int i = 0 ; i < n ; i++)
+    {
+        const Int pend = U->packed ? Up [i + 1] : Up [i] + Unz [i] ;
+        for (Int q = Up [i] ; q < pend ; q++)
+        {
+            const Int k = Ui [q], s = (k < i) ? smap [k] : -1 ;
+            if (s < 0 || reach_p [s + 1] == reach_p [s]) continue ;
+            Int pos ;
+            ROW_POS (s, i, pos) ;
+            int32_t *fp = reach_first + reach_p [s] + pos ;
+            if (pos >= 0 && *fp > (int32_t) (k - super [s])) *fp = (int32_t) (k - super [s]) ;
+        }
+    }
+    for (Int c = 0 ; c < nsuper ; c++)
+    {
+        const Int nscol = super [c + 1] - super [c], p0 = pi [c] + nscol ;
+        if (p0 >= pi [c + 1]) continue ;
+        const Int s = smap [Ls [p0]] ;
+        if (reach_p [s + 1] == reach_p [s]) continue ;
+        const int32_t f = (int32_t) (Ls [p0] - super [s]) ;
+        Int pos = 0 ;
+        for (Int q = p0 ; q < pi [c + 1] ; q++)
+        {
+            while (pi [s] + pos < pi [s + 1] && Ls [pi [s] + pos] < Ls [q]) pos++ ;
+            if (pi [s] + pos < pi [s + 1] && Ls [pi [s] + pos] == Ls [q] && reach_first [reach_p [s] + pos] > f)
+                reach_first [reach_p [s] + pos] = f ;
+        }
+    }
+    #undef ROW_POS
+    free (smap) ;
+    return reach_p [nsuper] ;
+}
+
+void ssamd_front_reach_alloc (const cholmod_sparse *U, const cholmod_factor *L, int64_t **reach_p, int32_t **reach_first)
+{
+    *reach_p = malloc (((size_t) L->nsuper + 1) * sizeof (int64_t)) ;
+    *reach_first = NULL ;
+    int64_t len = *reach_p ? ssamd_front_reach (U, L, *reach_p, NULL) : -1 ;
+    if (len > 0) *reach_first = malloc ((size_t) len * sizeof (int32_t)) ;
+    if (len > 0 && *reach_first && ssamd_front_reach (U, L, *reach_p, *reach_first) == len) return ;
+    free (*reach_p) ; free (*reach_first) ;
+    *reach_p = NULL ; *reach_first = NULL ;
+}
+
+int64_t cholmod_l_hip_front_reach (cholmod_sparse *A, cholmod_factor *L, int64_t *reach_p, int32_t *reach_first,
+    cholmod_common *Common)
+{
+    if (!A || !L || !reach_p || !L->is_super || !L->Perm || A->stype == 0 || A->nrow != L->n) return -1 ;
+    cholmod_sparse *U = NULL, *Lw = NULL ;
+    if (A->stype < 0) U = cholmod_l_ptranspose (A, 0, L->Perm, NULL, 0, Common) ;
+    else
+    {
+        Lw = cholmod_l_ptranspose (A, 0, L->Perm, NULL, 0, Common) ;
+        if (Lw) U = cholmod_l_ptranspose (Lw, 0, NULL, NULL, 0, Common) ;
+    }
+    const int64_t len = U ? ssamd_front_reach (U, L, reach_p, reach_first) : -1 ;
+    cholmod_l_free_sparse (&U, Common) ;
+    cholmod_l_free_sparse (&Lw, Common) ;
+    return len ;
+}
+
+void ssamd_plan_ahead (cholmod_factor *L, cholmod_common *Common, const int64_t *reach_p, const int32_t *reach_first)
 {
     if (!L || !L->is_super || !L->useGPU || L->hip_plan || Common->useGPU != 1) return ;
     if (Common->hip_world > 1 || Common->hip_allreduce) return ;
     if (!ssamd_factor_has_cholesky_sizes (L) || !cholmod_hip_probe ()) return ;
     const int st = Common->status, tc = Common->try_catch ;
     Common->try_catch = TRUE ;
-    if (ssamd_ensure_plan (L, Common)) L->hip_plan_ahead = plan_flags_of (L, Common) + 1 ;
+    if (ensure_plan_with (L, Common, reach_p, reach_first)) L->hip_plan_ahead = plan_flags_of (L, Common) + 1 ;
     Common->try_catch = tc ; Common->status = st ;
 }
 
```

Result: faster. 64600 GFLOP/s, median of 6 (+5.5%).
